# adamjorr/kbbq-py

Hardware: NVIDIA B200
Metric: bases/sec recalibrated (table build + apply) (higher is better)
Workload: dtype u8 in/out, u32->int64 counts, f64 model

## Files before the change

include/kbbq_b200.h:

```cpp
#ifndef KBBQ_B200_H
#define KBBQ_B200_H

#include <stddef.h>
#include <stdint.h>

#ifdef __cplusplus
extern "C" {
#endif

#define KBBQ_NQ 43
#define KBBQ_NDINUC 16

#define KBBQ_OK 0
#define KBBQ_E_ARG (-1)
#define KBBQ_E_CUDA (-2)
#define KBBQ_E_WORKSPACE (-3)
#define KBBQ_E_DATA (-4)
#define KBBQ_E_IO (-5)
#define KBBQ_E_FORMAT (-6)
#define KBBQ_E_RAGGED (-7)
#define KBBQ_E_NAME_FIELD (-8)
#define KBBQ_E_NAME_RG (-9)
#define KBBQ_E_NAME_MISMATCH (-10)
#define KBBQ_E_PEER (-11)
#define KBBQ_E_UNSUPPORTED (-12)

#define KBBQ_FLAG_QUAL_RANGE 1
#define KBBQ_FLAG_BAD_BASE 2
#define KBBQ_FLAG_RG_RANGE 4
#define KBBQ_FLAG_SEGMENTS 8

int kbbq_abi_version(void);
const char *kbbq_strerror(int code);
const char *kbbq_last_cuda_error(void);

int64_t kbbq_pos_table_elems(int L, int R);
int64_t kbbq_din_table_elems(int R);

int kbbq_workspace_bytes(int64_t N, int L, int R, size_t *bytes);

int kbbq_build(const uint8_t *seq_dev, const uint8_t *qual_dev, const uint8_t *corr_dev,
               const uint16_t *rg_dev, const uint8_t *second_dev, int64_t N, int L, int R,
               int minscore, int64_t *pos_errs_dev, int64_t *pos_total_dev, int64_t *din_errs_dev,
               int64_t *din_total_dev, void *workspace_dev, size_t workspace_bytes,
               int *status_dev, int path, void *stream);

int kbbq_marginals(const int64_t *pos_errs_dev, const int64_t *pos_total_dev, int L, int R,
                   int64_t *q_errs_dev, int64_t *q_total_dev, int64_t *rg_errs_dev,
                   int64_t *rg_total_dev, int64_t *meanq_dev, void *stream);

int kbbq_delta_q(const int64_t *prior_q_dev, const int64_t *numerrs_dev,
                 const int64_t *numtotal_dev, int64_t n, int64_t *delta_dev, void *stream);

int kbbq_posterior_q_real(const double *prior_q_dev, const int64_t *numerrs_dev,
                          const int64_t *numtotal_dev, int64_t n, int64_t *posterior_dev, void *stream);

int kbbq_bam_workspace_bytes(int64_t N, int L, int R, size_t *bytes);
int kbbq_build_bam(const uint8_t *seq_dev, const uint8_t *qual_dev, const uint8_t *err_dev,
                   const uint8_t *skip_dev, const uint16_t *rg_dev, const uint8_t *flags_dev,
                   const uint16_t *aln_start_dev, const uint16_t *aln_end_dev, int64_t N, int L, int R,
                   int minscore, int64_t *pos_errs_dev, int64_t *pos_total_dev, int64_t *din_errs_dev,
                   int64_t *din_total_dev, void *workspace_dev, size_t workspace_bytes, int *status_dev,
                   void *stream);
int kbbq_apply_bam(const uint8_t *seq_dev, const uint8_t *qual_dev, const uint16_t *rg_dev,
                   const uint8_t *flags_dev, int64_t N, int L, int R, int minscore,
                   const int64_t *meanq_dev, const int64_t *rgdq_dev, const int64_t *qdq_dev,
                   const int64_t *posdq_dev, const int64_t *dindq_dev, int nq, int ndin1,
                   uint8_t *out_qual_dev, void *workspace_dev, size_t workspace_bytes, int *status_dev,
                   void *stream);

int kbbq_calibration_counts(const uint8_t *qual_dev, const uint8_t *err_dev, const uint8_t *seq_dev,
                            const uint8_t *corr_dev, const uint8_t *skip_dev, int64_t n,
                            int64_t *total_dev, int64_t *errs_dev, void *stream);

int kbbq_get_delta_qs(const int64_t *meanq_dev, const int64_t *rg_errs_dev,
                      const int64_t *rg_total_dev, const int64_t *q_errs_dev,
                      const int64_t *q_total_dev, const int64_t *pos_errs_dev,
                      const int64_t *pos_total_dev, const int64_t *din_errs_dev,
                      const int64_t *din_total_dev, int R, int nq, int ncyc, int ndin,
                      int64_t *rgdq_dev, int64_t *qdq_dev, int64_t *posdq_dev, int64_t *dindq_dev,
                      void *stream);

int kbbq_apply(const uint8_t *seq_dev, const uint8_t *qual_dev, const uint16_t *rg_dev,
               const uint8_t *second_dev, int64_t N, int L, int R, int minscore,
               const int64_t *meanq_dev, const int64_t *rgdq_dev, const int64_t *qdq_dev,
               const int64_t *posdq_dev, const int64_t *dindq_dev, int nq, int ndin1,
               uint8_t *out_qual_dev, void *workspace_dev, size_t workspace_bytes, int *status_dev,
               int path, void *stream);

int64_t kbbq_segment_rows_bound(int64_t N, int R);
int64_t kbbq_segment_table_elems(int R);
int kbbq_segmented_supported(int L, int R, int minscore);
int kbbq_segment_plan(const uint16_t *rg_dev, const uint8_t *second_dev, int64_t N, int R, uint32_t *seg_dev,
                      uint32_t *dest_dev, int *status_dev, void *stream);
int kbbq_segment_rows(const uint8_t *src_dev, const uint32_t *dest_dev, int64_t N, int L, uint8_t *dst_segmented_dev,
                      void *stream);
int kbbq_segment_pad(const uint32_t *seg_dev, int R, int L, uint8_t *seq_dev, uint8_t *qual_dev, uint8_t *corr_dev,
                     void *stream);
int kbbq_unsegment_rows(const uint8_t *src_segmented_dev, const uint32_t *dest_dev, int64_t N, int L,
                        int64_t rows_bound, uint8_t *dst_dev, void *stream);
int kbbq_build_segmented(const uint8_t *seq_dev, const uint8_t *qual_dev, const uint8_t *corr_dev,
                         const uint32_t *seg_dev, int64_t rows_bound, int L, int R, int minscore,
                         int64_t *pos_errs_dev, int64_t *pos_total_dev, int64_t *din_errs_dev,
                         int64_t *din_total_dev, void *workspace_dev, size_t workspace_bytes, int *status_dev,
                         void *stream);
int kbbq_apply_segmented(const uint8_t *seq_dev, const uint8_t *qual_dev, const uint32_t *seg_dev, int64_t rows_bound,
                         int L, int R, int minscore, const int64_t *meanq_dev, const int64_t *rgdq_dev,
                         const int64_t *qdq_dev, const int64_t *posdq_dev, const int64_t *dindq_dev, int nq,
                         int ndin1, uint8_t *out_qual_dev, void *workspace_dev, size_t workspace_bytes,
                         int *status_dev, void *stream);

int kbbq_recalibrate_host(const uint8_t *seq, const uint8_t *qual, const uint8_t *corr,
                          const uint16_t *rg, const uint8_t *second, int64_t N, int L, int R,
                          int minscore, uint8_t *out_qual, int64_t *tables_host,
                          int64_t *deltas_host, int *status_out, int device);
int kbbq_recalibrate_host_multi(const uint8_t *seq, const uint8_t *qual, const uint8_t *corr,
                                const uint16_t *rg, const uint8_t *second, int64_t N, int L, int R,
                                int minscore, uint8_t *out_qual, int64_t *tables_host,
                                int64_t *deltas_host, int *status_out, const int *devices, int n_dev);

int kbbq_recalibrate_fastq(const char *reads_path, const char *corrected_path, int infer_rg, int minscore, int out_fd,
                           int device, int threads, int64_t *n_reads, int *n_rg, int *status_out);

int kbbq_host_release(int device);
int kbbq_host_last_traffic(int device, int64_t *h2d_bytes, int64_t *d2h_bytes);
int kbbq_host_pack_mode(int host_threads);

typedef struct kbbq_session kbbq_session;
int kbbq_session_create(int device, int L, int R, int minscore, int64_t chunk_reads, int64_t resident_reads_cap,
                        int host_threads, kbbq_session **out);
void kbbq_session_destroy(kbbq_session *s);
int64_t kbbq_session_chunk_reads(const kbbq_session *s);
// ... 88 lines not shown
```

kbbq-py_b200/csrc/apply.cuh:

```cuda
#pragma once
#include "build.cuh"
#include "common.cuh"
#include "stage.cuh"

namespace kbbq {

struct ApplyArgs {
    const uint8_t *seq, *qual;
    uint8_t *out;
    long long total_bytes;
    Geom g;
    TableCfg t;
    StageLayout sl;
    int R, nq;
    int nsub, segmode;
    const entry_t *entries;
    const unsigned int *seg;
    const unsigned int *uni;
    const short *fold_cyc;
    const short *fold_din;
    int *status;
};

static_assert((offsetof(ApplyArgs, t) + offsetof(TableCfg, ohe)) % 16 == 0,
              "ApplyArgs: TableCfg::ohe has to be 16-byte aligned in the kernel parameters (build.cuh); pad Geom");

__host__ __device__ inline int apply_table_bytes(const TableCfg &t) { return t.table_bytes; }

template <int KPS, bool UNI>
__device__ __forceinline__ void apply_consume(const ApplyArgs &a, unsigned char *smem_raw, uint32_t lo, uint32_t hi,
                                              uint32_t uni_flo, uint32_t uni_fhi) {
    const Geom &g = a.g;
    const TableCfg &t = a.t;
    const StageLayout &sl = a.sl;
    const int nconsumers = g.threads;
    const uint32_t bar0 = pin(smem_u32(smem_raw + sl.bar_off));
    const ThreadMap m = make_thread_map(g, t, UNI, true);
    const int lane = threadIdx.x & 31;
    const uint32_t pos_base = smem_addr(smem_raw + t.pos_off);
    const uint32_t din_base = pin(smem_addr(smem_raw + t.din_off) + (lane & (t.drep - 1)) * 4);
    uint32_t aeff[4];
#pragma unroll
    for (int b = 0; b < 4; ++b) aeff[b] = pos_base + m.cell[b];
    uint32_t cur_flag = 1;
    const uint32_t selv = pin(m.selv), seln = pin(m.seln);
    const uint32_t rowsel = m.row >= 0 ? (uint32_t)m.row : 0u;
    const uint32_t lanemask = pin(m.row >= 0 ? 0xFFu : 0u);
    const uint32_t rowmask = pin(m.rowmask);
    const bool live = m.row >= 0;
    const uint32_t kgrp = g.ng * g.gbytes;
    const bool half_lo = m.rowmask == 0x0000FFFFu, half_hi = m.rowmask == 0xFFFF0000u;
    const bool st32 = m.rowmask == 0xFFFFFFFFu, st16 = half_lo || half_hi, st8 = !st32 && !st16 && m.rowmask != 0u;
    const uint32_t wshift = pin(half_hi ? 16u : 0u);
    unsigned long long outp = (unsigned long long)(a.out + m.toff + (half_hi ? 2 : 0));
    asm volatile("" : "+l"(outp));
    const uint32_t data0 = pin(smem_u32(smem_raw + sl.data_off) + m.toff + (UNI ? m.grp * g.gbytes : 0));
    const uint32_t hdr0 = pin(smem_u32(smem_raw + sl.hdr_off) + m.grp * 16);
    const uint32_t stage_bytes = pin(sl.narr * sl.abytes), abytes = pin(sl.abytes), hdr_stride = sl.ngs * 16, krec = g.ng * 16;
    const uint32_t nstages = pin(sl.stages), ngs = pin(sl.ngs);
    const uint32_t revoff = t.revoff, addq = t.addq, gbytes = g.gbytes;
    const uint32_t addnq = (uint32_t)(128 - a.nq) * ONE4;
    const uint32_t one = pin(1u);
    uint32_t stage = 0, phase = 0;
    uint32_t qgood = 0xFFFFFFFFu;

    int cur_rg = -1, cur_sub = -1;
    int hs0 = 0, hs1 = 1;
    if (UNI && !a.segmode) {
        hs0 = (int)((uni_flo & 0xFFu) >> 1);
        hs1 = (int)(((uni_flo >> 8) & 0xFFu) >> 1);
    }
    for (int sub = 0; sub < a.nsub; ++sub) {
        uint32_t s_lo = a.seg[sub], s_hi = a.seg[sub + 1];
        if (s_hi <= lo) continue;
        if (s_lo >= hi) break;
        if (s_lo < lo) s_lo = lo;
        if (s_hi > hi) s_hi = hi;
        if (s_lo >= s_hi) continue;
        const int rg = a.segmode ? sub >> 1 : sub;

        if (rg != cur_rg || (a.segmode && sub != cur_sub)) {
            cur_rg = rg;
            cur_sub = sub;
            if (a.segmode) hs0 = hs1 = sub & 1;
            consumer_sync(nconsumers);
            for (int i = threadIdx.x; i < apply_table_bytes(t) / 4; i += nconsumers)
                reinterpret_cast<int *>(smem_raw)[i] = i * 4 < t.din_off && (i * 4) % t.revoff < t.rs ? g.minscore - 1 : 0;
            consumer_sync(nconsumers);
            const int L = g.L, L2 = 2 * g.L;
            const short *fc = a.fold_cyc + (size_t)rg * NQ * L2;
            for (int i = threadIdx.x; i < 2 * (t.nrows - 1) * L; i += nconsumers) {
                const int slot = i >= (t.nrows - 1) * L, j = i - slot * (t.nrows - 1) * L;
                const int r = j / L + 1, c = j - (r - 1) * L;
                const int half = slot ? hs1 : hs0;
                int *p = reinterpret_cast<int *>(smem_raw + t.pos_off + slot * t.revoff + r * t.rs) + ((c & 3) * t.sj + (c >> 2));
                *p = fc[(size_t)(r + g.minscore - 1) * L2 + (half ? L2 - 1 - c : c)];
            }
            const short *fd = a.fold_din + (size_t)rg * NQ * DIN_SLOTS;
            for (int i = threadIdx.x; i < (t.nrows - 1) * DIN_SLOTS * t.drep; i += nconsumers) {
                const int cell = i / t.drep, r = cell / DIN_SLOTS + 1, s = cell & (DIN_SLOTS - 1);
                int *p = reinterpret_cast<int *>(smem_raw + t.din_off + r * t.dq + s * (t.drep * 4)) + (i & (t.drep - 1));
                *p = fd[(r + g.minscore - 1) * DIN_SLOTS + s];
            }
            consumer_sync(nconsumers);
        }

        for (uint32_t first = s_lo; first < s_hi; first += ngs) {
            mbar_wait(bar0 + stage * 8, phase);
            const uint32_t shdr = pin(hdr0 + stage * hdr_stride);
            uint32_t sdata = data0 + stage * stage_bytes;
            uint32_t nlive = sl.ngs;
            if (UNI) {
                sdata += (uint32_t)((unsigned long long)first * g.gbytes) & 15u;
                nlive = s_hi - first;
            }
            sdata = pin(sdata);
            auto apply_word = [&](const uint32_t wa, const uint32_t hgrp) {
                uint32_t sw, qw, pb;
                asm volatile("ld.shared.u32 %0, [%1];" : "=r"(sw) : "r"(wa));
                asm volatile("ld.shared.u32 %0, [%1];" : "=r"(qw) : "r"(wa + abytes));
                asm volatile("ld.shared.u8 %0, [%1];" : "=r"(pb) : "r"(wa - 1));

                const uint32_t nu = ~add_fma(qw, one, addnq);
                const uint32_t w5 = add_fma(qw, one, addq);
                qgood &= nu & ~qw;
                const uint32_t vraw = w5 & nu & ~qw;
                const uint32_t vm8 = prmt(vraw, 0u, selv);
                const uint32_t qrow4 = w5 & vm8 & 0x3F3F3F3Fu;
                const uint32_t pw = prmt(pb, sw, 0x6540u);
                const uint32_t d4 = (pw & 0x06060606u) * 4u + (sw & 0x06060606u);
                const uint32_t nm8 = prmt((sw | pw) * 16u, 0xFFFFFFFFu, seln);
                const uint32_t qd = qrow4 & ~nm8;
                const uint32_t x01 = prmt(d4, qd, 0x5140u), x23 = prmt(d4, qd, 0x7362u);

                uint32_t v[4];
#pragma unroll
                for (int b = 0; b < 4; ++b) {
                    const uint32_t pa = (b & 2) ? __dp2a_hi(t.cyc16[b & 1], qrow4, aeff[b]) : __dp2a_lo(t.cyc16[b & 1], qrow4, aeff[b]);
                    const uint32_t xb = (b & 2) ? x23 : x01;
                    const uint32_t da = (b & 1) ? __dp2a_hi(t.din16, xb, din_base) : __dp2a_lo(t.din16, xb, din_base);
                    uint32_t x, y;
                    asm volatile("ld.shared.u32 %0, [%1];" : "=r"(x) : "r"(pa));
                    asm volatile("ld.shared.u32 %0, [%1];" : "=r"(y) : "r"(da));
                    v[b] = x + y;
                }
                const uint32_t sum4 = __byte_perm(__byte_perm(v[0], v[1], 0x0040), __byte_perm(v[2], v[3], 0x0040), 0x5410);
                const uint32_t res = (sum4 & vm8) | (qw & ~vm8);
                const unsigned long long dst = outp + (unsigned long long)hgrp * gbytes;
                if (UNI) {
                    if (st32) asm volatile("st.global.u32 [%0], %1;" ::"l"(dst), "r"(res) : "memory");
                    return;
                }
                if (st32) asm volatile("st.global.u32 [%0], %1;" ::"l"(dst), "r"(res) : "memory");
                if (st16) asm volatile("st.global.u16 [%0], %1;" ::"l"(dst), "h"((unsigned short)(res >> wshift)) : "memory");
                if (st8) {
#pragma unroll
                    for (int b = 0; b < 4; ++b)
                        if ((rowmask >> (8 * b)) & 1u)
                            asm volatile("st.global.u8 [%0], %1;" ::"l"(dst + b), "r"(res >> (8 * b)) : "memory");
                }
            };
            if (UNI && nlive >= sl.ngs) {
#pragma unroll
                for (int k = 0; k < KPS; ++k) apply_word(sdata + k * kgrp, first + m.grp + k * g.ng);
            } else {
#pragma unroll
                for (int k = 0; k < KPS; ++k) {
                    uint32_t soff, hgrp;
                    if (UNI) {
                        if (!live || (uint32_t)(m.grp + k * g.ng) >= nlive) continue;
                        soff = k * kgrp;
                        hgrp = first + m.grp + k * g.ng;
                    } else {
                        uint32_t flo, fhi;
                        if (g.contig) {
                            const uint32_t e = first + (uint32_t)m.grp + (uint32_t)(k * g.ng);
                            const uint4 rec = e < s_hi ? __ldg(a.entries + e) : make_uint4(0u, 0u, 0u, 0u);
                            soff = rec.x; hgrp = rec.y; flo = rec.z; fhi = rec.w;
                        } else {
                            asm volatile("ld.shared.v4.u32 {%0, %1, %2, %3}, [%4];"
                                         : "=r"(soff), "=r"(hgrp), "=r"(flo), "=r"(fhi)
                                         : "r"(shdr + k * krec));
                        }
                        const uint32_t flag = prmt(flo, fhi, rowsel) & lanemask;
                        if (flag != cur_flag) {
                            if (!flag) continue;
                            const uint32_t delta = ((flag >> 1) - (cur_flag >> 1)) * revoff;
#pragma unroll
                            for (int b = 0; b < 4; ++b) aeff[b] += delta;
                            cur_flag = flag;
                        }
                    }
                    apply_word(sdata + soff, hgrp);
                }
            }
            __syncwarp();
            if (lane == 0) mbar_arrive(bar0 + (nstages + stage) * 8);
            if (++stage == nstages) { stage = 0; phase ^= 1; }
        }
    }
    if (~qgood & rowmask & H4) atomicOr(a.status, KBBQ_FLAG_QUAL_RANGE);
}


template <int KPS>
__global__ void __launch_bounds__(MAX_THREADS, 1) apply_smem_kernel(const __grid_constant__ ApplyArgs a) {
    extern __shared__ __align__(128) unsigned char smem_raw[];
    const Geom &g = a.g;
    const StageLayout &sl = a.sl;
    const int nconsumers = g.threads;

    const unsigned long long E = a.seg[a.nsub];
    const uint32_t lo = (uint32_t)(E * blockIdx.x / gridDim.x), hi = (uint32_t)(E * (blockIdx.x + 1) / gridDim.x);
    const bool contig = a.R == 1 || a.segmode;
    const bool uniform = contig && a.uni[0] == 0u;

    const uint32_t bar0 = smem_u32(smem_raw + sl.bar_off);
    if (threadIdx.x == 0) {
        for (int s = 0; s < sl.stages; ++s) {
            mbar_init(bar0 + s * 8, 1);
            mbar_init(bar0 + (sl.stages + s) * 8, nconsumers / 32);
        }
        mbar_fence_init();
    }
    __syncthreads();

    if ((int)threadIdx.x >= nconsumers) {
        ProducerArgs p;
        p.arr[0] = a.seq; p.arr[1] = a.qual; p.arr[2] = nullptr;
        p.entries = a.entries; p.seg = a.seg; p.nsub = a.nsub; p.contig = contig; p.lo = lo; p.hi = hi;
        p.gbytes = g.gbytes; p.ng = sl.ngs; p.total_bytes = a.total_bytes;
        p.pw = ((int)threadIdx.x - nconsumers) >> 5; p.nprod = g.nprod;
        p.uniform = uniform;
        producer_loop(p, sl, smem_raw);
        return;
    }

    if (uniform) apply_consume<KPS, true>(a, smem_raw, lo, hi, a.uni[1], a.uni[2]);
    else apply_consume<KPS, false>(a, smem_raw, lo, hi, 0u, 0u);
}

struct ApplyGenericArgs {
    const uint8_t *seq, *qual;
    const uint16_t *rg;
    const uint8_t *second;
    uint8_t *out;
    long long N;
    int L, R, minscore, nq;
    const short *fold_cyc, *fold_din;
    int *status;
};

__global__ void apply_generic_kernel(ApplyGenericArgs a) {
    const long long total = a.N * a.L;
    for (long long i = (long long)blockIdx.x * blockDim.x + threadIdx.x; i < total;
         i += (long long)gridDim.x * blockDim.x) {
        const long long r = i / a.L;
        const int c = (int)(i - r * a.L);
        const unsigned int q = a.qual[i];
        if ((int)q < a.minscore) { a.out[i] = (uint8_t)q; continue; }
        if ((int)q >= a.nq) { atomicOr(a.status, KBBQ_FLAG_QUAL_RANGE); a.out[i] = (uint8_t)q; continue; }
        const unsigned int g = a.rg ? a.rg[r] : 0;
        if (g >= (unsigned int)a.R) { atomicOr(a.status, KBBQ_FLAG_RG_RANGE); a.out[i] = (uint8_t)q; continue; }
        const int c2 = (a.second && a.second[r]) ? 2 * a.L - 1 - c : c;
        const size_t gq = (size_t)g * NQ + q;
        int v = a.fold_cyc[gq * (2 * a.L) + c2];
        if (c > 0) {
            const uint8_t s = a.seq[i], ps = a.seq[i - 1];
            if (s != 'N' && ps != 'N') v += a.fold_din[gq * DIN_SLOTS + ((((ps >> 1) & 3) << 2) | ((s >> 1) & 3))];
        }
        a.out[i] = (uint8_t)v;
    }
}

}
```

kbbq-py_b200/csrc/build.cuh:

```cuda
#pragma once
#include <cstddef>
#include "common.cuh"
#include "prepare.cuh"
#include "stage.cuh"

namespace kbbq {

constexpr uint32_t ERR_UNIT = 65025u;
constexpr int DIN_SLOTS = 16;
constexpr int DIN_REP = 32;
constexpr int MAX_WARPS = MAX_THREADS / 32;

struct TableCfg {
    int nrows;
    int rs;
    int sj;
    int revoff;
    int dq;
    int drep;
    int pos_off, din_off;
    int table_bytes;
    int flush_pos;
    int fold_din;
    uint32_t addq;
    uint32_t cyc16[2];
    uint32_t din16;
    uint32_t ohe[4];
    uint32_t val16[2];
};

inline int cycle_table_wavefronts(const Geom &g, int sj, int rs_words, int shift, bool word_owner) {
    const int nwords = g.gbytes >> 2;
    int total = 0;
    for (int warp = 0; warp < g.threads / 32; ++warp)
        for (int b = 0; b < 4; ++b) {
            int cnt[32] = {0}, worst = 0;
            for (int lane = 0; lane < 32; ++lane) {
                const int tid = warp * 32 + lane, grp = tid / g.lps, t = tid - grp * g.lps;
                int cell = (lane + 32 * b) % rs_words;
                if (grp < g.ng && word_owner) {
                    if (t < nwords) {
                        const int j = 4 * t + b, k = j / g.L, c = j - k * g.L;
                        cell = (c & 3) * sj + (c >> 2) + (k & 1) * shift;
                    }
                } else if (grp < g.ng) {
                    for (int k = 0; k < g.G; ++k)
                        if (t >= g.wstart[k] && t < g.wstart[k + 1]) {
                            const int c = 4 * (t - g.wstart[k]) + b - ((k * g.L) & 3);
                            cell = c >= 0 && c < g.L ? (c & 3) * sj + (c >> 2) + (k & 1) * shift : 0;
                        }
                }
                worst = std::max(worst, ++cnt[cell & 31]);
            }
            total += worst;
        }
    return total;
}

inline bool make_table_cfg(const Geom &g, int kps, int drep, bool word_owner, TableCfg *t) {
    if (g.minscore < 1) return false;
    if (drep != 32 && drep != 16 && drep != 8) return false;
    t->nrows = NQ + 1 - g.minscore;
    t->sj = (g.L + 3) / 4;
    t->rs = (16 * t->sj + 127) / 128 * 128;
    if (t->rs > 1152) return false;
    int shift = 0;
    if (const char *e = getenv("KBBQ_SLOT_SHIFT")) shift = std::max(0, std::min(31, atoi(e)));
    else {
        int best = cycle_table_wavefronts(g, t->sj, t->rs / 4, 0, word_owner);
        for (int d = 1; d < 32; ++d) {
            const int w = cycle_table_wavefronts(g, t->sj, t->rs / 4, d, word_owner);
            if (w < best) { best = w; shift = d; }
        }
    }
    t->revoff = t->nrows * t->rs + 4 * shift;
    t->drep = drep;
    t->dq = DIN_SLOTS * drep * 4;
    t->pos_off = 0;
    t->din_off = (t->revoff + t->nrows * t->rs + 127) / 128 * 128;
    t->table_bytes = t->din_off + t->nrows * t->dq;
    t->flush_pos = std::max(1, (int)((ERR_UNIT - 1) / (uint32_t)(kps * g.ng * g.G)));
    t->fold_din = std::max(1, (int)((ERR_UNIT - 1) / (uint32_t)(kps * 4 * ((g.threads + drep - 1) / drep))));
    t->addq = (uint32_t)(0x81 - g.minscore) * ONE4;
    t->cyc16[0] = (uint32_t)t->rs;
    t->cyc16[1] = (uint32_t)t->rs << 16;
    t->din16 = (uint32_t)(drep * 2) | ((uint32_t)t->dq << 16);
    for (int b = 0; b < 4; ++b) t->ohe[b] = 255u << (8 * b);
    t->val16[0] = 1u | (16u << 16);
    t->val16[1] = 256u | (4096u << 16);
    return true;
}

struct BuildArgs {
    const uint8_t *seq, *qual, *corr;
    long long total_bytes;
    Geom g;
    TableCfg t;
    StageLayout sl;
    int R;
    int nsub;
    int segmode;
    const entry_t *entries;
    const unsigned int *seg;
    const unsigned int *uni;
    unsigned long long *pos_errs, *pos_total, *din_errs, *din_total;
    int *status;
};

static_assert((offsetof(BuildArgs, t) + offsetof(TableCfg, ohe)) % 16 == 0,
              "BuildArgs: TableCfg::ohe has to be 16-byte aligned in the kernel parameters; pad Geom");

__device__ __forceinline__ void red_shared_add(uint32_t saddr, uint32_t v) {
    asm volatile("red.shared.add.u32 [%0], %1;" ::"r"(saddr), "r"(v) : "memory");
}
__device__ __forceinline__ uint32_t smem_addr(const void *p) {
    return (uint32_t)__cvta_generic_to_shared(p);
}
__device__ __forceinline__ uint32_t prmt(uint32_t a, uint32_t b, uint32_t sel) {
    uint32_t d;
    asm("prmt.b32 %0, %1, %2, %3;" : "=r"(d) : "r"(a), "r"(b), "r"(sel));
    return d;
}
__device__ __forceinline__ uint32_t pin(uint32_t v) {
    asm volatile("" : "+r"(v));
    return v;
}

__device__ __forceinline__ uint32_t add_fma(uint32_t a, uint32_t one, uint32_t c) {
    uint32_t d;
    asm("mad.lo.u32 %0, %1, %2, %3;" : "=r"(d) : "r"(a), "r"(one), "r"(c));
    return d;
}

struct ThreadMap {
    int grp;
    int row;
    int toff;
    uint32_t rowmask;
    uint32_t selv;
    uint32_t seln;
    uint32_t cell[4];
    int cyc[4];
};

__device__ __forceinline__ ThreadMap make_thread_map(const Geom &g, const TableCfg &tc, bool by_parity, bool word_owner) {
    ThreadMap m;
    const int tid = threadIdx.x;
    m.grp = tid / g.lps;
    const int t = tid - m.grp * g.lps;
    m.row = -1;
    int w = 0;
#pragma unroll
    for (int k = 0; k < MAX_G; ++k)
        if (k < g.G && t >= g.wstart[k] && t < g.wstart[k + 1]) { m.row = k; w = t - g.wstart[k]; }
    if (m.grp >= g.ng) m.row = -1;
    m.rowmask = 0; m.toff = 0; m.selv = 0x4444u; m.seln = 0x4444u;
#pragma unroll
    for (int b = 0; b < 4; ++b) { m.cell[b] = 0; m.cyc[b] = -1; }
    if (by_parity && word_owner) {
        const int nwords = g.gbytes >> 2;
        m.row = (t < nwords && m.grp < g.ng) ? (4 * t) / g.L : -1;
        if (m.row >= 0) {
            m.toff = 4 * t;
            m.rowmask = 0xFFFFFFFFu;
            m.selv = 0xBA98u;
            m.seln = 0xBA98u;
#pragma unroll
            for (int b = 0; b < 4; ++b) {
                const int j = 4 * t + b, k = j / g.L, c = j - k * g.L;
                m.cyc[b] = c;
                if (c == 0) m.seln = (m.seln & ~(0xFu << (4 * b))) | (0x4u << (4 * b));
                m.cell[b] = 4u * (uint32_t)((c & 3) * tc.sj + (c >> 2)) + (uint32_t)((k & 1) * tc.revoff);
            }
        }
    } else if (m.row >= 0) {
        const int a = (m.row * g.L) & 3;
        m.toff = m.row * g.L - a + 4 * w;
#pragma unroll
        for (int b = 0; b < 4; ++b) {
            const int c = 4 * w + b - a;
            if (c >= 0 && c < g.L) {
                m.cyc[b] = c;
                m.rowmask |= 0xFFu << (8 * b);
                m.selv = (m.selv & ~(0xFu << (4 * b))) | ((8u | b) << (4 * b));
                if (c != 0) m.seln = (m.seln & ~(0xFu << (4 * b))) | ((8u | b) << (4 * b));
                m.cell[b] = 4u * (uint32_t)((c & 3) * tc.sj + (c >> 2)) + (by_parity ? (uint32_t)((m.row & 1) * tc.revoff) : 0u);
            }
// ... 12 lines not shown
    const int lane = threadIdx.x & 31, warp = threadIdx.x >> 5, nwarps = nconsumers >> 5;
    unsigned long long *gde = a.din_errs + (size_t)rg * NQ * 16, *gdt = a.din_total + (size_t)rg * NQ * 16;
    for (int cell = DIN_SLOTS + warp; cell < t.nrows * DIN_SLOTS; cell += nwarps) {
        const int r = cell / DIN_SLOTS, dn = cell - r * DIN_SLOTS;
        unsigned int *p = reinterpret_cast<unsigned int *>(smem_raw + t.din_off + r * t.dq + dn * (t.drep * 4)) + lane;
        const unsigned int v = lane < t.drep ? *p : 0u;
        if (__any_sync(0xFFFFFFFFu, v != 0)) {
            if (lane < t.drep) *p = 0;
            unsigned int tot = v % ERR_UNIT, er = v / ERR_UNIT;
#pragma unroll
            for (int o = 16; o; o >>= 1) {
                tot += __shfl_xor_sync(0xFFFFFFFFu, tot, o);
                er += __shfl_xor_sync(0xFFFFFFFFu, er, o);
            }
            if (lane == 0) {
                const int dref = nat_to_ref(dn >> 2) * 4 + nat_to_ref(dn & 3);
                const size_t o = (size_t)(r + a.g.minscore - 1) * 16 + dref;
                atomicAdd(gdt + o, (unsigned long long)tot);
                if (er) atomicAdd(gde + o, (unsigned long long)er);
            }
        }
    }
}

__device__ __forceinline__ void flush_pos_table(const BuildArgs &a, unsigned char *smem_raw, int rg, int nconsumers, int hs0, int hs1) {
    const Geom &g = a.g;
    const TableCfg &t = a.t;
    const int L = g.L, L2 = 2 * g.L;
    unsigned long long *gpe = a.pos_errs + (size_t)rg * NQ * L2, *gpt = a.pos_total + (size_t)rg * NQ * L2;
    const int per_slot = (t.nrows - 1) * L;
    for (int i = threadIdx.x; i < 2 * per_slot; i += nconsumers) {
        const int slot = i >= per_slot, j = i - slot * per_slot;
        const int r = j / L + 1, c = j - (r - 1) * L;
        unsigned int *p = reinterpret_cast<unsigned int *>(smem_raw + t.pos_off + slot * t.revoff + r * t.rs) +
                          ((c & 3) * t.sj + (c >> 2));
        const unsigned int v = *p;
        if (v) {
            *p = 0;
            const unsigned int tot = v % ERR_UNIT, er = v / ERR_UNIT;
            const int half = slot ? hs1 : hs0;
            const size_t o = (size_t)(r + g.minscore - 1) * L2 + (half ? L2 - 1 - c : c);
            atomicAdd(gpt + o, (unsigned long long)tot);
            if (er) atomicAdd(gpe + o, (unsigned long long)er);
        }
    }
}

template <int KPS, bool VALIDATE, bool UNI>
__device__ __forceinline__ void build_consume(const BuildArgs &a, unsigned char *smem_raw, uint32_t lo, uint32_t hi,
                                              uint32_t uni_flo, uint32_t uni_fhi) {
    const Geom &g = a.g;
    const TableCfg &t = a.t;
    const StageLayout &sl = a.sl;
    const int nconsumers = g.threads;
    const uint32_t bar0 = pin(smem_u32(smem_raw + sl.bar_off));
    const ThreadMap m = make_thread_map(g, t, UNI, false);
    const int lane = threadIdx.x & 31;
    const uint32_t pos_base = smem_addr(smem_raw + t.pos_off);
    const uint32_t din_base = pin(smem_addr(smem_raw + t.din_off) + (lane & (t.drep - 1)) * 4);
    uint32_t aeff[4];
#pragma unroll
    for (int b = 0; b < 4; ++b) aeff[b] = pos_base + m.cell[b];
    uint32_t cur_flag = 1;
    const uint32_t selv = pin(m.selv), seln = pin(m.seln);
    const uint32_t rowsel = m.row >= 0 ? (uint32_t)m.row : 0u;
    const uint32_t lanemask = pin(m.row >= 0 ? 0xFFu : 0u);
    const uint32_t rowmask = pin(m.rowmask);
    const bool live = m.row >= 0;
    const uint32_t data0 = pin(smem_u32(smem_raw + sl.data_off) + m.toff + (UNI ? m.grp * g.gbytes : 0));
    const uint32_t hdr0 = pin(smem_u32(smem_raw + sl.hdr_off) + m.grp * 16);
    const uint32_t kgrp = g.ng * g.gbytes;
    const uint32_t stage_bytes = pin(sl.narr * sl.abytes), abytes = pin(sl.abytes), abytes2 = pin(2 * sl.abytes), hdr_stride = sl.ngs * 16, krec = g.ng * 16;
    const uint32_t nstages = pin(sl.stages), ngs = pin(sl.ngs);
    const uint32_t revoff = t.revoff, addq = t.addq;
    const uint32_t one = pin(1u), minus1 = pin(0xFFFFFFFFu), lut_lo = pin(0x43014101u), lut_hi = pin(0x474E0154u);
    uint32_t stage = 0, phase = 0;
    uint32_t qgood = 0xFFFFFFFFu, bbad = 0;

    for (int i = threadIdx.x; i < t.table_bytes / 4; i += nconsumers) reinterpret_cast<unsigned int *>(smem_raw)[i] = 0;
    consumer_sync(nconsumers);
    int cur_rg = -1, cur_sub = -1;
    int hs0 = 0, hs1 = 1;
    uint32_t since_pos = 0, since_din = 0;
    auto flush_all = [&](int rg) {
        consumer_sync(nconsumers);
        flush_pos_table(a, smem_raw, rg, nconsumers, hs0, hs1);
        fold_din_replicas(a, smem_raw, rg, nconsumers);
        consumer_sync(nconsumers);
        since_pos = since_din = 0;
    };
    if (UNI && !a.segmode) {
        hs0 = (int)((uni_flo & 0xFFu) >> 1);
        hs1 = (int)(((uni_flo >> 8) & 0xFFu) >> 1);
    }

    for (int sub = 0; sub < a.nsub; ++sub) {
        uint32_t s_lo = a.seg[sub], s_hi = a.seg[sub + 1];
        if (s_hi <= lo) continue;
        if (s_lo >= hi) break;
        if (s_lo < lo) s_lo = lo;
        if (s_hi > hi) s_hi = hi;
        if (s_lo >= s_hi) continue;
        const int rg = a.segmode ? sub >> 1 : sub;
        if (cur_rg >= 0 && (rg != cur_rg || (a.segmode && sub != cur_sub))) flush_all(cur_rg);
        cur_rg = rg;
        cur_sub = sub;
        if (a.segmode) hs0 = hs1 = sub & 1;

        for (uint32_t first = s_lo; first < s_hi;) {
            if (since_pos >= (uint32_t)t.flush_pos || since_din >= (uint32_t)t.fold_din) {
                consumer_sync(nconsumers);
                if (since_pos >= (uint32_t)t.flush_pos) { flush_pos_table(a, smem_raw, rg, nconsumers, hs0, hs1); since_pos = 0; }
                if (since_din >= (uint32_t)t.fold_din) { fold_din_replicas(a, smem_raw, rg, nconsumers); since_din = 0; }
                consumer_sync(nconsumers);
            }
            const uint32_t room = min((uint32_t)t.flush_pos - since_pos, (uint32_t)t.fold_din - since_din);
            const uint32_t chunk_end = (uint32_t)min((unsigned long long)s_hi, (unsigned long long)first + (unsigned long long)room * sl.ngs);
            const uint32_t iters = (chunk_end - first + ngs - 1) / ngs;
            since_pos += iters;
            since_din += iters;
            for (; first < chunk_end; first += ngs) {
                mbar_wait(bar0 + stage * 8, phase);
                const uint32_t shdr = pin(hdr0 + stage * hdr_stride);
                uint32_t sdata = data0 + stage * stage_bytes;
                uint32_t nlive = sl.ngs;
                if (UNI) {
                    sdata += (uint32_t)((unsigned long long)first * g.gbytes) & 15u;
                    nlive = s_hi - first;
                }
                sdata = pin(sdata);
                auto tally_word = [&](const uint32_t wa) {
                    uint32_t sw, qw, cw, pb;
                    asm volatile("ld.shared.u32 %0, [%1];" : "=r"(sw) : "r"(wa));
                    asm volatile("ld.shared.u32 %0, [%1];" : "=r"(qw) : "r"(wa + abytes));
                    asm volatile("ld.shared.u32 %0, [%1];" : "=r"(cw) : "r"(wa + abytes2));
                    asm volatile("ld.shared.u8 %0, [%1];" : "=r"(pb) : "r"(wa - 1));

                    const uint32_t nu = add_fma(qw, minus1, 0xAAAAAAAAu);
                    const uint32_t w5 = qw + addq;
                    qgood &= nu & ~qw;
                    const uint32_t vraw = w5 & nu & ~qw;
                    const uint32_t vm8 = prmt(vraw, 0u, selv);
                    const uint32_t qrow4 = w5 & vm8 & 0x3F3F3F3Fu;

                    const uint32_t pw = prmt(pb, sw, 0x6540u);
                    const uint32_t d4 = (pw & 0x06060606u) * 4u + (sw & 0x06060606u);
                    const uint32_t nm8 = prmt((sw | pw) * 16u, 0xFFFFFFFFu, seln);
                    const uint32_t qd = qrow4 & ~nm8;
                    const uint32_t x01 = prmt(d4, qd, 0x5140u), x23 = prmt(d4, qd, 0x7362u);

                    const uint32_t e8 = prmt(add_fma(sw ^ cw, one, 0x7F7F7F7Fu), 0u, 0xBA98u);

                    if (VALIDATE) {
                        const uint32_t code3 = sw & 0x07070707u;
                        const uint32_t sel = __dp2a_hi(t.val16[1], code3, __dp2a_lo(t.val16[0], code3, 0u));
                        const uint32_t recon = prmt(lut_lo, lut_hi, sel);
                        bbad |= recon ^ sw;
                    }

#pragma unroll
                    for (int b = 0; b < 4; ++b) {
                        const uint32_t inc = __dp4a(e8, t.ohe[b], one);
                        const uint32_t pa = (b & 2) ? __dp2a_hi(t.cyc16[b & 1], qrow4, aeff[b]) : __dp2a_lo(t.cyc16[b & 1], qrow4, aeff[b]);
                        const uint32_t xb = (b & 2) ? x23 : x01;
                        const uint32_t da = (b & 1) ? __dp2a_hi(t.din16, xb, din_base) : __dp2a_lo(t.din16, xb, din_base);
                        red_shared_add(pa, inc);
                        red_shared_add(da, inc);
                    }
                };
                if (UNI && nlive >= sl.ngs) {
#pragma unroll
                    for (int k = 0; k < KPS; ++k) tally_word(sdata + k * kgrp);
                } else {
#pragma unroll
                    for (int k = 0; k < KPS; ++k) {
                        uint32_t soff;
                        if (UNI) {
                            if (!live || (uint32_t)(m.grp + k * g.ng) >= nlive) continue;
                            soff = k * kgrp;
                        } else {
                            uint32_t hgrp, flo, fhi;
                            if (g.contig) {
                                const uint32_t e = first + (uint32_t)m.grp + (uint32_t)(k * g.ng);
                                const uint4 rec = e < s_hi ? __ldg(a.entries + e) : make_uint4(0u, 0u, 0u, 0u);
                                soff = rec.x; hgrp = rec.y; flo = rec.z; fhi = rec.w;
                            } else {
                                asm volatile("ld.shared.v4.u32 {%0, %1, %2, %3}, [%4];"
                                             : "=r"(soff), "=r"(hgrp), "=r"(flo), "=r"(fhi)
                                             : "r"(shdr + k * krec));
                            }
                            const uint32_t flag = prmt(flo, fhi, rowsel) & lanemask;
                            if (flag != cur_flag) {
                                if (!flag) continue;
                                const uint32_t delta = ((flag >> 1) - (cur_flag >> 1)) * revoff;
#pragma unroll
                                for (int b = 0; b < 4; ++b) aeff[b] += delta;
                                cur_flag = flag;
                            }
                        }
                        tally_word(sdata + soff);
                    }
                }
                __syncwarp();
                if (lane == 0) mbar_arrive(bar0 + (nstages + stage) * 8);
                if (++stage == nstages) { stage = 0; phase ^= 1; }
            }
        }
    }
    if (cur_rg >= 0) flush_all(cur_rg);
    if (~qgood & rowmask & H4) atomicOr(a.status, KBBQ_FLAG_QUAL_RANGE);
    if (VALIDATE && (bbad & rowmask)) atomicOr(a.status, KBBQ_FLAG_BAD_BASE);
}


template <int KPS, bool VALIDATE>
__global__ void __launch_bounds__(MAX_THREADS, 1) build_smem_kernel(const __grid_constant__ BuildArgs a) {
    extern __shared__ __align__(128) unsigned char smem_raw[];
    const Geom &g = a.g;
    const StageLayout &sl = a.sl;
    const int nconsumers = g.threads;

    const unsigned long long E = a.seg[a.nsub];
    const uint32_t lo = (uint32_t)(E * blockIdx.x / gridDim.x), hi = (uint32_t)(E * (blockIdx.x + 1) / gridDim.x);
    const bool contig = a.R == 1 || a.segmode;
    const bool uniform = contig && a.uni[0] == 0u;

    const uint32_t bar0 = smem_u32(smem_raw + sl.bar_off);
    if (threadIdx.x == 0) {
        for (int s = 0; s < sl.stages; ++s) {
            mbar_init(bar0 + s * 8, 1);
            mbar_init(bar0 + (sl.stages + s) * 8, nconsumers / 32);
        }
        mbar_fence_init();
    }
    __syncthreads();

    if ((int)threadIdx.x >= nconsumers) {
        ProducerArgs p;
        p.arr[0] = a.seq; p.arr[1] = a.qual; p.arr[2] = a.corr;
        p.entries = a.entries; p.seg = a.seg; p.nsub = a.nsub; p.contig = contig; p.lo = lo; p.hi = hi;
        p.gbytes = g.gbytes; p.ng = sl.ngs; p.total_bytes = a.total_bytes;
        p.pw = ((int)threadIdx.x - nconsumers) >> 5; p.nprod = g.nprod;
        p.uniform = uniform;
        producer_loop(p, sl, smem_raw);
        return;
    }

    if (uniform) build_consume<KPS, VALIDATE, true>(a, smem_raw, lo, hi, a.uni[1], a.uni[2]);
    else build_consume<KPS, VALIDATE, false>(a, smem_raw, lo, hi, 0u, 0u);
}

struct BuildGenericArgs {
    const uint8_t *seq, *qual, *corr;
    const uint16_t *rg;
    const uint8_t *second;
    long long N;
    int L, R, minscore;
    unsigned long long *pos_errs, *pos_total, *din_errs, *din_total;
    int *status;
};

__device__ __forceinline__ int base_code_ref(uint8_t b) {
    return b == 'A' ? 0 : b == 'T' ? 1 : b == 'G' ? 2 : b == 'C' ? 3 : b == 'N' ? 4 : 5;
}

__global__ void build_generic_kernel(BuildGenericArgs a) {
    const long long total = a.N * a.L;
    for (long long i = (long long)blockIdx.x * blockDim.x + threadIdx.x; i < total;
         i += (long long)gridDim.x * blockDim.x) {
        const long long r = i / a.L;
        const int c = (int)(i - r * a.L);
        const unsigned int q = a.qual[i];
        const uint8_t s = a.seq[i];
        const int code = base_code_ref(s);
        if (code == 5) atomicOr(a.status, KBBQ_FLAG_BAD_BASE);
        if (q > NQ - 1) { atomicOr(a.status, KBBQ_FLAG_QUAL_RANGE); continue; }
        const unsigned int g = a.rg ? a.rg[r] : 0;
        if (g >= (unsigned int)a.R) { atomicOr(a.status, KBBQ_FLAG_RG_RANGE); continue; }
        if ((int)q < a.minscore) continue;
        const bool err = s != a.corr[i];
        const int c2 = (a.second && a.second[r]) ? 2 * a.L - 1 - c : c;
        const size_t po = ((size_t)g * NQ + q) * (2 * a.L) + c2;
        atomicAdd(a.pos_total + po, 1ull);
        if (err) atomicAdd(a.pos_errs + po, 1ull);
        if (c > 0) {
            const int pcode = base_code_ref(a.seq[i - 1]);
            if (code < 4 && pcode < 4) {
                const size_t d = ((size_t)g * NQ + q) * 16 + pcode * 4 + code;
                atomicAdd(a.din_total + d, 1ull);
                if (err) atomicAdd(a.din_errs + d, 1ull);
            }
        }
    }
}

}
```

kbbq-py_b200/csrc/host_api.cu:

```cuda
#include <algorithm>
#include <atomic>
#include <chrono>
#include <condition_variable>
#include <memory>
#include <mutex>
#include <sched.h>
#include <stdlib.h>
#include <string.h>
#include <sys/mman.h>
#include <sys/stat.h>
#include <fcntl.h>
#include <thread>
#include <unistd.h>
#include <vector>

#include "common.cuh"

using namespace kbbq;

namespace {

#define KBBQ_TRY(x) do { int rc_ = (x); if (rc_) return rc_; } while (0)

constexpr int MAX_DEVICES = 16;
// ... 258 lines not shown
    return p;
}

bool chunk_args_ok(const kbbq_session *S, int64_t k, int64_t n, bool keep) {
    return n > 0 && n <= S->C && (!keep || k < (int64_t)S->res.size());
}

int build_chunk_upload(kbbq_session *S, int64_t k, const uint8_t *seq, const uint8_t *qual, const uint16_t *rg,
                       const uint8_t *second, int64_t n, bool keep) {
    if (!chunk_args_ok(S, k, n, keep) || !seq || !qual) return KBBQ_E_ARG;
    const ChunkPlace p = chunk_place(S, k, keep, rg != nullptr, second != nullptr);
    KBBQ_CUDA(cudaStreamWaitEvent(S->s_up, p.u->consumed, 0));
    return upload_reads(S, S->pack == PACK_NIBBLES ? nullptr : seq, qual, rg, second, n, p.d_seq, p.d_qual, p.d_rg, p.d_sec);
}

int build_chunk_finish(kbbq_session *S, int64_t k, const uint8_t *seq, const uint8_t *corr, bool has_rg, bool has_second,
                       int64_t n, bool keep) {
    if (!chunk_args_ok(S, k, n, keep) || !seq || !corr) return KBBQ_E_ARG;
    const ChunkPlace p = chunk_place(S, k, keep, has_rg, has_second);
    UpSlot &u = *p.u;
    Resident *r = p.r;
    const int L = S->L, R = S->R;
    const size_t nb = (size_t)n * L;
    if (r) r->n = n;
    if (S->pack) {
        KBBQ_CUDA(cudaEventSynchronize(u.uploaded));
        size_t bb;
        if (S->pack == PACK_NIBBLES) {
            int bad = 0;
            KBBQ_TRY(kbbq_host_pack_nibbles(seq, corr, (int64_t)nb, (uint8_t *)u.h_bits, S->host_threads, &bad));
            if (bad) S->host_status |= KBBQ_FLAG_BAD_BASE;
            bb = (nb + 1) / 2;
        } else {
            KBBQ_TRY(kbbq_host_mismatch_bits(seq, corr, (int64_t)nb, u.h_bits, S->host_threads));
            bb = ((nb + 31) / 32) * 4;
        }
        KBBQ_CUDA(cudaMemcpyAsync(u.bits, u.h_bits, bb, cudaMemcpyHostToDevice, S->s_up));
        S->h2d_bytes += (int64_t)bb;
    } else {
        KBBQ_CUDA(cudaMemcpyAsync(u.corr, corr, nb, cudaMemcpyHostToDevice, S->s_up));
        S->h2d_bytes += (int64_t)nb;
    }
    KBBQ_CUDA(cudaEventRecord(u.uploaded, S->s_up));
    KBBQ_CUDA(cudaStreamWaitEvent(S->s_comp, u.uploaded, 0));
    if (S->pack == PACK_NIBBLES) KBBQ_TRY(kbbq_expand_nibbles((const uint8_t *)u.bits, (int64_t)nb, p.d_seq, u.corr, S->s_comp));
    else if (S->pack == PACK_BITS) KBBQ_TRY(kbbq_expand_mismatch_bits(p.d_seq, u.bits, (int64_t)nb, u.corr, S->s_comp));
    const size_t npos = (size_t)R * NQ * 2 * L, ndin = (size_t)R * NQ * 16;
    int64_t *pe = S->d_tab, *pt = pe + npos, *de = pt + npos, *dt = de + ndin;
    if (S->segmode) {
        uint32_t *seg = keep ? r->seg : u.seg, *dest = keep ? r->dest : u.dest;
        uint8_t *sseq = keep ? r->seq : u.sseq, *squal = keep ? r->qual : u.squal;
        KBBQ_TRY(kbbq_segment_plan(p.d_rg, p.d_sec, n, R, seg, dest, S->d_status, S->s_comp));
        KBBQ_TRY(kbbq_segment_rows(p.d_seq, dest, n, L, sseq, S->s_comp));
        KBBQ_TRY(kbbq_segment_rows(p.d_qual, dest, n, L, squal, S->s_comp));
        KBBQ_TRY(kbbq_segment_rows(u.corr, dest, n, L, u.scorr, S->s_comp));
        KBBQ_TRY(kbbq_segment_pad(seg, R, L, sseq, squal, u.scorr, S->s_comp));
        KBBQ_TRY(kbbq_build_segmented(sseq, squal, u.scorr, seg, S->rowsC, L, R, S->minscore, pe, pt, de, dt, S->d_ws,
                                      S->ws_bytes, S->d_status, S->s_comp));
    } else {
        KBBQ_TRY(kbbq_build(p.d_seq, p.d_qual, u.corr, p.d_rg, p.d_sec, n, L, R, S->minscore, pe, pt, de, dt, S->d_ws, S->ws_bytes,
                            S->d_status, 0, S->s_comp));
    }
    KBBQ_CUDA(cudaEventRecord(u.consumed, S->s_comp));
    return KBBQ_OK;
}

int build_chunk_async(kbbq_session *S, const uint8_t *seq, const uint8_t *qual, const uint8_t *corr, const uint16_t *rg,
                      const uint8_t *second, int64_t n, bool keep) {
    if (n < 0 || n > S->C) return KBBQ_E_ARG;
    if (n == 0) return KBBQ_OK;
    if (!seq || !qual || !corr) return KBBQ_E_ARG;
    const int64_t k = S->built;
    if (keep && k >= (int64_t)S->res.size()) return KBBQ_E_ARG;
    S->built++;
    KBBQ_TRY(build_chunk_upload(S, k, seq, qual, rg, second, n, keep));
    return build_chunk_finish(S, k, seq, corr, rg != nullptr, second != nullptr, n, keep);
}

int model_async(kbbq_session *S) {
    const int L = S->L, R = S->R;
    const size_t npos = (size_t)R * NQ * 2 * L, ndin = (size_t)R * NQ * 16;
    int64_t *pe = S->summed ? S->d_sum : S->d_tab, *pt = pe + npos, *de = pt + npos, *dt = de + ndin;
    const ModelPtrs &mp = S->mp;
    KBBQ_TRY(kbbq_marginals(pe, pt, L, R, mp.q_errs, mp.q_total, mp.rg_errs, mp.rg_total, mp.meanq, S->s_comp));
    KBBQ_TRY(kbbq_get_delta_qs(mp.meanq, mp.rg_errs, mp.rg_total, mp.q_errs, mp.q_total, pe, pt, de, dt, R, NQ, 2 * L, 16,
                               mp.rgdq, mp.qdq, mp.posdq, mp.dindq, S->s_comp));
    return KBBQ_OK;
}

int apply_and_download(kbbq_session *S, const uint8_t *d_seq, const uint8_t *d_qual, const uint16_t *d_rg,
                       const uint8_t *d_sec, const uint32_t *seg, const uint32_t *dest, int64_t n, uint8_t *out_host) {
    const int L = S->L, R = S->R;
    OutSlot &o = S->down[S->applied++ & 1];
    const ModelPtrs &mp = S->mp;
    KBBQ_CUDA(cudaStreamWaitEvent(S->s_comp, o.drained, 0));
    if (S->segmode) {
        KBBQ_TRY(kbbq_apply_segmented(d_seq, d_qual, seg, S->rowsC, L, R, S->minscore, mp.meanq, mp.rgdq, mp.qdq, mp.posdq,
                                      mp.dindq, NQ, 17, o.out_seg, S->d_ws, S->ws_bytes, S->d_status, S->s_comp));
        KBBQ_TRY(kbbq_unsegment_rows(o.out_seg, dest, n, L, S->rowsC, o.out, S->s_comp));
    } else {
        KBBQ_TRY(kbbq_apply(d_seq, d_qual, d_rg, d_sec, n, L, R, S->minscore, mp.meanq, mp.rgdq, mp.qdq, mp.posdq, mp.dindq,
                            NQ, 17, o.out, S->d_ws, S->ws_bytes, S->d_status, 0, S->s_comp));
    }
    KBBQ_CUDA(cudaEventRecord(o.applied, S->s_comp));
    KBBQ_CUDA(cudaStreamWaitEvent(S->s_down, o.applied, 0));
    KBBQ_CUDA(cudaMemcpyAsync(out_host, o.out, (size_t)n * L, cudaMemcpyDeviceToHost, S->s_down));
    S->d2h_bytes += n * L;
    KBBQ_CUDA(cudaEventRecord(o.drained, S->s_down));
    return KBBQ_OK;
}

int apply_resident_async(kbbq_session *S, int64_t k, uint8_t *out_host) {
    if (k < 0 || k >= (int64_t)S->res.size() || !out_host) return KBBQ_E_ARG;
    const Resident &r = S->res[(size_t)k];
    if (r.n == 0) return KBBQ_OK;
    return apply_and_download(S, r.seq, r.qual, r.rg, r.sec, r.seg, r.dest, r.n, out_host);
}

int apply_chunk_async(kbbq_session *S, const uint8_t *seq, const uint8_t *qual, const uint16_t *rg, const uint8_t *second,
                      int64_t n, uint8_t *out_host) {
    if (n < 0 || n > S->C || !S->up[0].seq) return KBBQ_E_ARG;
    if (n == 0) return KBBQ_OK;
    if (!seq || !qual || !out_host) return KBBQ_E_ARG;
    UpSlot &u = S->up[S->applied & 1];
    const int L = S->L, R = S->R;
    uint16_t *d_rg = rg ? u.rg : nullptr;
    uint8_t *d_sec = second ? u.sec : nullptr;
    KBBQ_CUDA(cudaStreamWaitEvent(S->s_up, u.consumed, 0));
    KBBQ_TRY(upload_reads(S, seq, qual, rg, second, n, u.seq, u.qual, d_rg, d_sec));
    KBBQ_CUDA(cudaEventRecord(u.uploaded, S->s_up));
    KBBQ_CUDA(cudaStreamWaitEvent(S->s_comp, u.uploaded, 0));
    const uint8_t *a_seq = u.seq, *a_qual = u.qual;
    if (S->segmode) {
        uint8_t *sseq = u.sseq ? u.sseq : nullptr, *squal = u.squal;
        if (!sseq) return KBBQ_E_ARG;
        KBBQ_TRY(kbbq_segment_plan(d_rg, d_sec, n, R, u.seg, u.dest, S->d_status, S->s_comp));
        KBBQ_TRY(kbbq_segment_rows(u.seq, u.dest, n, L, sseq, S->s_comp));
        KBBQ_TRY(kbbq_segment_rows(u.qual, u.dest, n, L, squal, S->s_comp));
        KBBQ_TRY(kbbq_segment_pad(u.seg, R, L, sseq, squal, nullptr, S->s_comp));
        a_seq = sseq; a_qual = squal;
    }
    KBBQ_TRY(apply_and_download(S, a_seq, a_qual, d_rg, d_sec, u.seg, u.dest, n, out_host));
    KBBQ_CUDA(cudaEventRecord(u.consumed, S->s_comp));
    return KBBQ_OK;
}

int session_sync(kbbq_session *S, int *status_out) {
    int st = 0;
    KBBQ_CUDA(cudaStreamSynchronize(S->s_up));
    KBBQ_CUDA(cudaStreamSynchronize(S->s_comp));
    KBBQ_CUDA(cudaStreamSynchronize(S->s_down));
    KBBQ_CUDA(cudaMemcpy(&st, S->d_status, sizeof(int), cudaMemcpyDeviceToHost));
    st |= S->host_status;
    if (status_out) *status_out = st;
    return st ? KBBQ_E_DATA : KBBQ_OK;
}

struct CacheSlot {
    std::mutex mu;
    std::unique_ptr<kbbq_session> s;
};
CacheSlot g_cache[MAX_DEVICES];

int cached_session(int slot, int device, int L, int R, int minscore, int64_t C, int64_t M, int host_threads, int pack,
                   kbbq_session **out) {
    CacheSlot &c = g_cache[slot];
    kbbq_session *s = c.s.get();
    const int64_t C16 = (C + 15) / 16 * 16;
    const int64_t nres = M ? (M + C16 - 1) / C16 : 0;
    if (s && s->device == device && s->L == L && s->R == R && s->minscore == minscore && s->C == C16 &&
// ... 597 lines not shown
```

kbbq-py_b200/csrc/kbbq_b200.cu:

```cuda
#include <algorithm>
#include <mutex>
#include <stdlib.h>
#include <string.h>
#include <vector>

#include "apply.cuh"
#include "bam.cuh"
#include "build.cuh"
#include "calib.cuh"
#include "common.cuh"
#include "model.cuh"
#include "prepare.cuh"
#include "segment.cuh"
#include "synth.cuh"

namespace kbbq {

std::atomic<long long> g_launches{0};
char g_last_cuda_error[256] = "";

static std::mutex g_const_mu;
static bool g_const_done[64];

static int upload_constants(int device) {
// ... 133 lines not shown
    case KBBQ_E_DATA: return "input data error (see status flags)";
    case KBBQ_E_IO: return "FASTQ file could not be opened, read or written";
    case KBBQ_E_FORMAT: return "malformed FASTQ (4-line records expected)";
    case KBBQ_E_RAGGED: return "reads of unequal length";
    case KBBQ_E_NAME_FIELD: return "read name has no read-group field";
    case KBBQ_E_NAME_RG: return "read-group field does not start with RG";
    case KBBQ_E_NAME_MISMATCH: return "corrected read name does not start with the read name";
    case KBBQ_E_PEER: return "multi-GPU: peer access between the devices is not available";
    case KBBQ_E_UNSUPPORTED: return "not handled by this entry point (use the chunked driver)";
    default: return "unknown error";
    }
}

const char *kbbq_last_cuda_error(void) { return g_last_cuda_error; }

int64_t kbbq_pos_table_elems(int L, int R) { return (int64_t)R * NQ * 2 * L; }
int64_t kbbq_din_table_elems(int R) { return (int64_t)R * NQ * 16; }
int64_t kbbq_launch_count(void) { return g_launches.load(); }

int kbbq_plan_info(int L, int R, int minscore, int arrays, int max_smem, int *out) {
    if (!out || L < 1 || R < 1 || (arrays != 2 && arrays != 3)) return KBBQ_E_ARG;
    Geom g;
    TableCfg tc;
    StageLayout sl;
    if (!plan_kernel(L, R, minscore, arrays, max_smem > 0 ? max_smem : 232448, &g, &tc, &sl))
        return KBBQ_E_ARG;
    const int v[10] = {g.G, g.lanes, g.ng, g.threads, g.nprod, sl.kps, sl.stages, tc.drep, sl.total, tc.table_bytes};
    for (int i = 0; i < 10; ++i) out[i] = v[i];
    return KBBQ_OK;
}

int kbbq_workspace_bytes(int64_t N, int L, int R, size_t *bytes) {
    if (N < 0 || L < 1 || R < 1 || R > 65535 || !bytes) return KBBQ_E_ARG;
    *bytes = carve_workspace(nullptr, N, L, R).bytes;
    return KBBQ_OK;
}

static int build_impl(const uint8_t *seq, const uint8_t *qual, const uint8_t *corr, const uint16_t *rg,
                      const uint8_t *second, int64_t N, int L, int R, int minscore, int64_t *pos_errs,
                      int64_t *pos_total, int64_t *din_errs, int64_t *din_total, void *workspace,
                      size_t workspace_bytes, int *status, int path, void *stream, const unsigned int *seg_rows) {
    if (N < 0 || L < 1 || R < 1 || R > 65535 || minscore < 0 || minscore >= NQ) return KBBQ_E_ARG;
    if (!pos_errs || !pos_total || !din_errs || !din_total || !status) return KBBQ_E_ARG;
    if (N == 0) return KBBQ_OK;
    if (!seq || !qual || !corr) return KBBQ_E_ARG;
    const bool segmode = seg_rows != nullptr;
    cudaStream_t st = (cudaStream_t)stream;
    int device, sms, max_smem;
    int rc = current_device_info(&device, &sms, &max_smem);
    if (rc) return rc;

    Geom g;
    TableCfg tc;
    StageLayout sl;
    const bool smem_ok = path != 2 && !misaligned(seq, 16) && !misaligned(qual, 16) && !misaligned(corr, 16) &&
                         plan_kernel(L, R, minscore, 3, max_smem, &g, &tc, &sl, segmode) &&
                         (uint64_t)((N + g.G - 1) / g.G) < 0xFFFFFFFFull;
    if (!smem_ok) {
        if (path == 1 || segmode) return KBBQ_E_ARG;
        BuildGenericArgs a = {seq, qual, corr, rg, second, N, L, R, minscore,
                              (unsigned long long *)pos_errs, (unsigned long long *)pos_total,
                              (unsigned long long *)din_errs, (unsigned long long *)din_total, status};
        build_generic_kernel<<<sms * 8, 256, 0, st>>>(a);
        KBBQ_LAUNCHED();
        return KBBQ_OK;
    }
    Workspace w = carve_workspace(workspace, N, L, R);
    if (!workspace || workspace_bytes < w.bytes) return KBBQ_E_WORKSPACE;
    if (segmode) {
        seg_prepare_kernel<<<1, 256, 0, st>>>(seg_rows, 2 * R, g.G, (unsigned long long)N, w.seg, w.uni, status);
        KBBQ_LAUNCHED();
    } else {
        const int64_t tail = (R == 1 && N > g.G) ? N % g.G : 0;
        if (tail) {
            const int64_t n0 = N - tail;
            BuildGenericArgs ga = {seq + n0 * L, qual + n0 * L, corr + n0 * L, rg ? rg + n0 : nullptr,
                                   second ? second + n0 : nullptr, tail, L, R, minscore,
                                   (unsigned long long *)pos_errs, (unsigned long long *)pos_total,
                                   (unsigned long long *)din_errs, (unsigned long long *)din_total, status};
            build_generic_kernel<<<1, 256, 0, st>>>(ga);
            KBBQ_LAUNCHED();
            N = n0;
        }
        rc = run_prepare(rg, second, N, g.G, R, w, status, sms, sl.ngs, g.gbytes, sl.slot, st);
        if (rc) return rc;
    }

    BuildArgs a;
    a.seq = seq; a.qual = qual; a.corr = corr; a.total_bytes = N * L; a.g = g; a.t = tc; a.R = R;
    a.nsub = segmode ? 2 * R : R; a.segmode = segmode ? 1 : 0;
    a.sl = sl;
    a.entries = w.entries; a.seg = w.seg; a.uni = w.uni;
    a.pos_errs = (unsigned long long *)pos_errs; a.pos_total = (unsigned long long *)pos_total;
    a.din_errs = (unsigned long long *)din_errs; a.din_total = (unsigned long long *)din_total;
    a.status = status;
    return launch_build_smem(a, sms, a.sl.total, st);
}

int kbbq_build(const uint8_t *seq, const uint8_t *qual, const uint8_t *corr, const uint16_t *rg,
               const uint8_t *second, int64_t N, int L, int R, int minscore, int64_t *pos_errs,
               int64_t *pos_total, int64_t *din_errs, int64_t *din_total, void *workspace,
               size_t workspace_bytes, int *status, int path, void *stream) {
    return build_impl(seq, qual, corr, rg, second, N, L, R, minscore, pos_errs, pos_total, din_errs, din_total,
                      workspace, workspace_bytes, status, path, stream, nullptr);
}

int kbbq_build_segmented(const uint8_t *seq, const uint8_t *qual, const uint8_t *corr, const uint32_t *seg,
                         int64_t rows_bound, int L, int R, int minscore, int64_t *pos_errs, int64_t *pos_total,
                         int64_t *din_errs, int64_t *din_total, void *workspace, size_t workspace_bytes, int *status,
                         void *stream) {
    if (!seg || rows_bound % SEG_ALIGN) return KBBQ_E_ARG;
    return build_impl(seq, qual, corr, nullptr, nullptr, rows_bound, L, R, minscore, pos_errs, pos_total, din_errs,
                      din_total, workspace, workspace_bytes, status, 1, stream, seg);
}

int kbbq_marginals(const int64_t *pos_errs, const int64_t *pos_total, int L, int R, int64_t *q_errs,
                   int64_t *q_total, int64_t *rg_errs, int64_t *rg_total, int64_t *meanq, void *stream) {
    if (L < 1 || R < 1 || !pos_errs || !pos_total || !q_errs || !q_total || !rg_errs || !rg_total || !meanq)
        return KBBQ_E_ARG;
    cudaStream_t st = (cudaStream_t)stream;
    int device;
    KBBQ_CUDA(cudaGetDevice(&device));
    int rc = upload_constants(device);
    if (rc) return rc;
    marginals_q_kernel<<<dim3(NQ, R), 128, 0, st>>>((const long long *)pos_errs, (const long long *)pos_total,
                                                   2 * L, (long long *)q_errs, (long long *)q_total);
    KBBQ_LAUNCHED();
    marginals_rg_kernel<<<R, 64, 0, st>>>((const long long *)q_errs, (const long long *)q_total, R,
                                                      (long long *)rg_errs, (long long *)rg_total, (long long *)meanq);
    KBBQ_LAUNCHED();
    return KBBQ_OK;
}

int kbbq_delta_q(const int64_t *prior_q, const int64_t *numerrs, const int64_t *numtotal, int64_t n,
                 int64_t *delta, void *stream) {
    if (n < 0 || (n > 0 && (!prior_q || !numerrs || !numtotal || !delta))) return KBBQ_E_ARG;
    if (n == 0) return KBBQ_OK;
    int device;
    KBBQ_CUDA(cudaGetDevice(&device));
    int rc = upload_constants(device);
    if (rc) return rc;
    delta_q_kernel<<<(unsigned)((n + 127) / 128), 128, 0, (cudaStream_t)stream>>>(
        (const long long *)prior_q, (const long long *)numerrs, (const long long *)numtotal, n, (long long *)delta);
    KBBQ_LAUNCHED();
    return KBBQ_OK;
}

int kbbq_posterior_q_real(const double *prior_q, const int64_t *numerrs, const int64_t *numtotal, int64_t n,
                          int64_t *posterior, void *stream) {
    if (n < 0 || (n > 0 && (!prior_q || !numerrs || !numtotal || !posterior))) return KBBQ_E_ARG;
    if (n == 0) return KBBQ_OK;
    int device;
    KBBQ_CUDA(cudaGetDevice(&device));
    int rc = upload_constants(device);
    if (rc) return rc;
    posterior_q_real_kernel<<<(unsigned)((n + 127) / 128), 128, 0, (cudaStream_t)stream>>>(
        prior_q, (const long long *)numerrs, (const long long *)numtotal, n, (long long *)posterior);
    KBBQ_LAUNCHED();
    return KBBQ_OK;
}

struct BamWorkspace {
    uint8_t *cseq, *cqual, *cthird, *csecond;
    void *inner;
    size_t inner_bytes, bytes;
};
static BamWorkspace carve_bam_workspace(void *base, long long N, int L, int R) {
    BamWorkspace w = {};
    char *p = (char *)base;
    size_t off = 0;
    const size_t nb = align_up((size_t)N * L + 16, 256);
    w.cseq = (uint8_t *)(p + off); off += nb;
    w.cqual = (uint8_t *)(p + off); off += nb;
    w.cthird = (uint8_t *)(p + off); off += nb;
    w.csecond = (uint8_t *)(p + off); off += align_up((size_t)N + 16, 256);
    w.inner = p + off;
    w.inner_bytes = carve_workspace(nullptr, N, L, R).bytes;
    w.bytes = off + w.inner_bytes;
    return w;
}

static int launch_bam_canon(const BamCanonArgs &c, cudaStream_t st) {
    const unsigned int wmax = (unsigned int)((3 + c.L + 3) >> 2);
    const long long per = std::max<long long>(1, (long long)(0x7FFFFFFFu / wmax) / 256 * 256);
    for (long long r0 = 0; r0 < c.N; r0 += per) {
        const long long n = std::min<long long>(per, c.N - r0);
        bam_canon_kernel<<<(unsigned)((n * wmax + BAM_WARPS * 32 - 1) / (BAM_WARPS * 32)), BAM_WARPS * 32, 0, st>>>(c, r0, wmax);
        KBBQ_LAUNCHED();
    }
    return KBBQ_OK;
}

int kbbq_bam_workspace_bytes(int64_t N, int L, int R, size_t *bytes) {
    if (N < 0 || L < 1 || R < 1 || R > 65535 || !bytes) return KBBQ_E_ARG;
    *bytes = carve_bam_workspace(nullptr, N, L, R).bytes;
    return KBBQ_OK;
}

int kbbq_build_bam(const uint8_t *seq, const uint8_t *qual, const uint8_t *err, const uint8_t *skip, const uint16_t *rg,
                   const uint8_t *flags, const uint16_t *aln_start, const uint16_t *aln_end, int64_t N, int L, int R,
                   int minscore, int64_t *pos_errs, int64_t *pos_total, int64_t *din_errs, int64_t *din_total,
                   void *workspace, size_t workspace_bytes, int *status, void *stream) {
    if (N < 0 || L < 1 || L > 32767 || R < 1 || R > 65535 || minscore < 0 || minscore > NQ) return KBBQ_E_ARG;
    if (!pos_errs || !pos_total || !din_errs || !din_total || !status) return KBBQ_E_ARG;
    if (N == 0) return KBBQ_OK;
    if (!seq || !qual || !err) return KBBQ_E_ARG;
    int device, sms = KBBQ_SM_COUNT_FALLBACK;
    KBBQ_CUDA(cudaGetDevice(&device));
    cudaDeviceGetAttribute(&sms, cudaDevAttrMultiProcessorCount, device);
    cudaStream_t st = (cudaStream_t)stream;
    const long long blocks = std::min<long long>(((long long)N * L + 255) / 256, (long long)sms * 16);
    if (workspace && minscore >= 1) {
        BamWorkspace w = carve_bam_workspace(workspace, N, L, R);
        if (workspace_bytes < w.bytes) return KBBQ_E_WORKSPACE;
        BamCanonArgs c = {seq, qual, err, skip, rg, flags, aln_start, aln_end, N, L, R, minscore, true,
                          w.cseq, w.cqual, w.cthird, w.csecond,
                          (unsigned long long *)pos_errs, (unsigned long long *)pos_total,
                          (unsigned long long *)din_errs, (unsigned long long *)din_total, status};
        { const int rc_ = launch_bam_canon(c, st); if (rc_) return rc_; }
        return kbbq_build(w.cseq, w.cqual, w.cthird, rg, w.csecond, N, L, R, minscore, pos_errs, pos_total, din_errs,
                          din_total, w.inner, w.inner_bytes, status, 0, stream);
    }
    BuildBamArgs a = {seq, qual, err, skip, rg, flags, aln_start, aln_end, N, L, R, minscore,
                      (unsigned long long *)pos_errs, (unsigned long long *)pos_total,
                      (unsigned long long *)din_errs, (unsigned long long *)din_total, status};
    build_bam_kernel<<<(unsigned)blocks, 256, 0, st>>>(a);
    KBBQ_LAUNCHED();
    return KBBQ_OK;
}

int kbbq_apply_bam(const uint8_t *seq, const uint8_t *qual, const uint16_t *rg, const uint8_t *flags, int64_t N, int L,
                   int R, int minscore, const int64_t *meanq, const int64_t *rgdq, const int64_t *qdq,
                   const int64_t *posdq, const int64_t *dindq, int nq, int ndin1, uint8_t *out_qual, void *workspace,
                   size_t workspace_bytes, int *status, void *stream) {
    if (N < 0 || L < 1 || L > 32767 || R < 1 || R > 65535 || nq < 1 || nq > 256 || ndin1 != 17) return KBBQ_E_ARG;
    if (!meanq || !rgdq || !qdq || !posdq || !dindq || !status) return KBBQ_E_ARG;
    if (N == 0) return KBBQ_OK;
    if (!seq || !qual || !out_qual) return KBBQ_E_ARG;
    int device, sms = KBBQ_SM_COUNT_FALLBACK;
    KBBQ_CUDA(cudaGetDevice(&device));
    cudaDeviceGetAttribute(&sms, cudaDevAttrMultiProcessorCount, device);
    cudaStream_t st = (cudaStream_t)stream;
    const long long blocks = std::min<long long>(((long long)N * L + 255) / 256, (long long)sms * 16);
    if (workspace && minscore >= 1 && nq <= NQ) {
        BamWorkspace w = carve_bam_workspace(workspace, N, L, R);
        if (workspace_bytes < w.bytes) return KBBQ_E_WORKSPACE;
        BamCanonArgs c = {seq, qual, nullptr, nullptr, rg, flags, nullptr, nullptr, N, L, R, minscore, false,
                          w.cseq, w.cqual, nullptr, w.csecond, nullptr, nullptr, nullptr, nullptr, status};
        { const int rc_ = launch_bam_canon(c, st); if (rc_) return rc_; }
        int rc = kbbq_apply(w.cseq, w.cqual, rg, w.csecond, N, L, R, minscore, meanq, rgdq, qdq, posdq, dindq, nq, ndin1,
                            w.cthird, w.inner, w.inner_bytes, status, 0, stream);
        if (rc) return rc;
        {
            const unsigned int wmax = (unsigned int)((3 + L + 3) >> 2);
            const long long per = std::max<long long>(1, (long long)(0x7FFFFFFFu / wmax) / 256 * 256);
            for (long long r0 = 0; r0 < N; r0 += per) {
                const long long n = std::min<long long>(per, N - r0);
                bam_uncanon_kernel<<<(unsigned)((n * wmax + BAM_WARPS * 32 - 1) / (BAM_WARPS * 32)), BAM_WARPS * 32, 0, st>>>(
                    w.cthird, flags, N, L, out_qual, r0, wmax);
                KBBQ_LAUNCHED();
            }
        }
        return KBBQ_OK;
    }
    ApplyBamArgs a = {seq, qual, rg, flags, out_qual, N, L, R, minscore, nq, ndin1, (const long long *)meanq,
                      (const long long *)rgdq, (const long long *)qdq, (const long long *)posdq,
                      (const long long *)dindq, status};
    apply_bam_kernel<<<(unsigned)blocks, 256, 0, st>>>(a);
    KBBQ_LAUNCHED();
    return KBBQ_OK;
}

int kbbq_calibration_counts(const uint8_t *qual, const uint8_t *err, const uint8_t *seq, const uint8_t *corr,
                            const uint8_t *skip, int64_t n, int64_t *total, int64_t *errs, void *stream) {
    if (n < 0 || !total || !errs) return KBBQ_E_ARG;
    if (n == 0) return KBBQ_OK;
    if (!qual || (!err && (!seq || !corr))) return KBBQ_E_ARG;
    cudaStream_t st = (cudaStream_t)stream;
    int device, sms = KBBQ_SM_COUNT_FALLBACK;
    KBBQ_CUDA(cudaGetDevice(&device));
    cudaDeviceGetAttribute(&sms, cudaDevAttrMultiProcessorCount, device);
    auto misaligned = [](const void *p) { return p && ((uintptr_t)p & 15u); };
    CalibArgs a = {qual, err, seq, corr, skip, n, (unsigned long long *)total, (unsigned long long *)errs};
    if (misaligned(qual) || misaligned(err) || misaligned(skip) || (!err && (misaligned(seq) || misaligned(corr)))) {
        const long long chunk = 1ll << 31;
        for (long long o = 0; o < n; o += chunk) {
            CalibArgs c = a;
            c.qual += o; if (err) c.err += o; else { c.seq += o; c.corr += o; } if (skip) c.skip += o;
            c.n = std::min<long long>(chunk, n - o);
            calibration_scalar_kernel<<<sms * 8, CAL_THREADS, 0, st>>>(c);
            KBBQ_LAUNCHED();
        }
        return KBBQ_OK;
    }
    const int grid = sms * 3;
    const long long chunk = (long long)grid * CAL_THREADS * CAL_MAX_ITERS * 32;
    auto kern = err ? (skip ? calibration_kernel<true, true> : calibration_kernel<true, false>)
                    : (skip ? calibration_kernel<false, true> : calibration_kernel<false, false>);
    KBBQ_CUDA(cudaFuncSetAttribute(kern, cudaFuncAttributeMaxDynamicSharedMemorySize, CAL_SMEM));
    for (long long o = 0; o < n; o += chunk) {
        CalibArgs c = a;
        c.qual += o; if (err) c.err += o; else { c.seq += o; c.corr += o; } if (skip) c.skip += o;
        c.n = std::min<long long>(chunk, n - o);
        kern<<<grid, CAL_THREADS, CAL_SMEM, st>>>(c);
        KBBQ_LAUNCHED();
    }
    return KBBQ_OK;
}

int kbbq_get_delta_qs(const int64_t *meanq, const int64_t *rg_errs, const int64_t *rg_total,
                      const int64_t *q_errs, const int64_t *q_total, const int64_t *pos_errs,
                      const int64_t *pos_total, const int64_t *din_errs, const int64_t *din_total, int R,
                      int nq, int ncyc, int ndin, int64_t *rgdq, int64_t *qdq, int64_t *posdq,
                      int64_t *dindq, void *stream) {
    if (R < 1 || nq < 1 || ncyc < 0 || ndin < 0) return KBBQ_E_ARG;
    if (!meanq || !rg_errs || !rg_total || !q_errs || !q_total || !rgdq || !qdq) return KBBQ_E_ARG;
    if ((ncyc && (!pos_errs || !pos_total || !posdq)) || !dindq || (ndin && (!din_errs || !din_total)))
        return KBBQ_E_ARG;
    int device;
    KBBQ_CUDA(cudaGetDevice(&device));
    int rc = upload_constants(device);
    if (rc) return rc;
    cudaStream_t st = (cudaStream_t)stream;
    DeltaArgs a = {(const long long *)meanq, (const long long *)rg_errs, (const long long *)rg_total,
                   (const long long *)q_errs, (const long long *)q_total, (const long long *)pos_errs,
                   (const long long *)pos_total, (const long long *)din_errs, (const long long *)din_total,
                   R, nq, ncyc, ndin, (long long *)rgdq, (long long *)qdq, (long long *)posdq, (long long *)dindq};
    delta_levels12_kernel<<<R, 64, 0, st>>>(a);
    KBBQ_LAUNCHED();
    const long long cells = (long long)R * nq * (ncyc + ndin + 1);
    delta_level3_kernel<<<(unsigned)((cells + 127) / 128), 128, 0, st>>>(a);
    KBBQ_LAUNCHED();
    return KBBQ_OK;
}

static int apply_impl(const uint8_t *seq, const uint8_t *qual, const uint16_t *rg, const uint8_t *second, int64_t N,
                      int L, int R, int minscore, const int64_t *meanq, const int64_t *rgdq, const int64_t *qdq,
                      const int64_t *posdq, const int64_t *dindq, int nq, int ndin1, uint8_t *out_qual,
                      void *workspace, size_t workspace_bytes, int *status, int path, void *stream,
                      const unsigned int *seg_rows) {
    const bool segmode = seg_rows != nullptr;
    if (N < 0 || L < 1 || R < 1 || R > 65535 || minscore < 0 || minscore >= NQ) return KBBQ_E_ARG;
    if (nq < 1 || nq > NQ || ndin1 < 16 || ndin1 > 64) return KBBQ_E_ARG;
    if (!meanq || !rgdq || !qdq || !posdq || !dindq || !status) return KBBQ_E_ARG;
    if (N == 0) return KBBQ_OK;
    if (!seq || !qual || !out_qual) return KBBQ_E_ARG;
    cudaStream_t st = (cudaStream_t)stream;
    int device, sms, max_smem;
    int rc = current_device_info(&device, &sms, &max_smem);
    if (rc) return rc;
    Workspace w = carve_workspace(workspace, N, L, R);
    if (!workspace || workspace_bytes < w.bytes) return KBBQ_E_WORKSPACE;

    const long long fold_cells = (long long)R * NQ * (2 * L + 16);
    fold_kernel<<<(unsigned)((fold_cells + 255) / 256), 256, 0, st>>>(
        (const long long *)meanq, (const long long *)rgdq, (const long long *)qdq, (const long long *)posdq,
        (const long long *)dindq, R, nq, 2 * L, ndin1, w.fold_cyc, w.fold_din);
    KBBQ_LAUNCHED();

    Geom g;
    TableCfg tc;
    StageLayout sl;
    const bool smem_ok = path != 2 && !misaligned(seq, 16) && !misaligned(qual, 16) && !misaligned(out_qual, 4) &&
                         plan_kernel(L, R, minscore, 2, max_smem, &g, &tc, &sl, segmode) &&
                         (uint64_t)((N + g.G - 1) / g.G) < 0xFFFFFFFFull;
    if (!smem_ok) {
        if (path == 1 || segmode) return KBBQ_E_ARG;
        ApplyGenericArgs a = {seq, qual, rg, second, out_qual, N, L, R, minscore, nq, w.fold_cyc, w.fold_din, status};
        apply_generic_kernel<<<sms * 8, 256, 0, st>>>(a);
        KBBQ_LAUNCHED();
        return KBBQ_OK;
    }
    const int64_t tail = (!segmode && R == 1 && N > g.G) ? N % g.G : 0;
    if (tail) {
        const int64_t n0 = N - tail;
        ApplyGenericArgs ga = {seq + n0 * L, qual + n0 * L, rg ? rg + n0 : nullptr, second ? second + n0 : nullptr,
                               out_qual + n0 * L, tail, L, R, minscore, nq, w.fold_cyc, w.fold_din, status};
        apply_generic_kernel<<<1, 256, 0, st>>>(ga);
        KBBQ_LAUNCHED();
        N = n0;
    }
    if (segmode) {
        seg_prepare_kernel<<<1, 256, 0, st>>>(seg_rows, 2 * R, g.G, (unsigned long long)N, w.seg, w.uni, status);
        KBBQ_LAUNCHED();
    } else {
        rc = run_prepare(rg, second, N, g.G, R, w, status, sms, sl.ngs, g.gbytes, sl.slot, st);
        if (rc) return rc;
    }
    ApplyArgs a;
    a.nsub = segmode ? 2 * R : R; a.segmode = segmode ? 1 : 0;
    a.seq = seq; a.qual = qual; a.out = out_qual; a.total_bytes = N * L; a.g = g; a.t = tc; a.R = R; a.nq = nq;
    a.sl = sl;
    a.entries = w.entries; a.seg = w.seg; a.uni = w.uni; a.fold_cyc = w.fold_cyc; a.fold_din = w.fold_din; a.status = status;
    return launch_apply_smem(a, sms, a.sl.total, st);
}

int kbbq_apply(const uint8_t *seq, const uint8_t *qual, const uint16_t *rg, const uint8_t *second, int64_t N,
               int L, int R, int minscore, const int64_t *meanq, const int64_t *rgdq, const int64_t *qdq,
               const int64_t *posdq, const int64_t *dindq, int nq, int ndin1, uint8_t *out_qual,
               void *workspace, size_t workspace_bytes, int *status, int path, void *stream) {
    return apply_impl(seq, qual, rg, second, N, L, R, minscore, meanq, rgdq, qdq, posdq, dindq, nq, ndin1, out_qual,
                      workspace, workspace_bytes, status, path, stream, nullptr);
}

int kbbq_apply_segmented(const uint8_t *seq, const uint8_t *qual, const uint32_t *seg, int64_t rows_bound, int L, int R,
                         int minscore, const int64_t *meanq, const int64_t *rgdq, const int64_t *qdq,
                         const int64_t *posdq, const int64_t *dindq, int nq, int ndin1, uint8_t *out_qual,
                         void *workspace, size_t workspace_bytes, int *status, void *stream) {
    if (!seg || rows_bound % SEG_ALIGN) return KBBQ_E_ARG;
    return apply_impl(seq, qual, nullptr, nullptr, rows_bound, L, R, minscore, meanq, rgdq, qdq, posdq, dindq, nq, ndin1,
                      out_qual, workspace, workspace_bytes, status, 1, stream, seg);
}


int64_t kbbq_segment_rows_bound(int64_t N, int R) {
    if (N < 0 || R < 1) return -1;
    return (N + SEG_ALIGN - 1) / SEG_ALIGN * SEG_ALIGN + (int64_t)2 * R * SEG_ALIGN;
}

int64_t kbbq_segment_table_elems(int R) { return R < 1 ? -1 : (int64_t)6 * R + 1; }

int kbbq_segmented_supported(int L, int R, int minscore) {
    if (L < 1 || R < 1 || R > 65535) return 0;
    Geom g;
    TableCfg tc;
    StageLayout sl;
    return plan_kernel(L, R, minscore, 3, 232448, &g, &tc, &sl, true) && plan_kernel(L, R, minscore, 2, 232448, &g, &tc, &sl, true);
}

int kbbq_segment_plan(const uint16_t *rg, const uint8_t *second, int64_t N, int R, uint32_t *seg, uint32_t *dest,
                      int *status, void *stream) {
    if (N < 0 || R < 1 || R > 65535 || !seg || !status || (N > 0 && !dest)) return KBBQ_E_ARG;
    if (kbbq_segment_rows_bound(N, R) >= 0xFFFFFFFFll) return KBBQ_E_ARG;
    cudaStream_t st = (cudaStream_t)stream;
    const int nkeys = 2 * R;
    SegPlanArgs a = {rg, second, N, R, seg, seg + 2 * nkeys + 1, dest, status};
    KBBQ_CUDA(cudaMemsetAsync(a.cursor, 0, sizeof(unsigned int) * nkeys, st));
    const int per_thread = 8;
    const long long per_block = (long long)SEG_THREADS * per_thread;
    const unsigned int blocks = (unsigned int)((N + per_block - 1) / per_block);
    const size_t smem = nkeys <= SEG_SMEM_KEYS ? sizeof(unsigned int) * nkeys : 0;
    if (blocks) {
        seg_bucket_kernel<0><<<blocks, SEG_THREADS, smem, st>>>(a, per_thread);
        KBBQ_LAUNCHED();
    }
    seg_scan_kernel<<<1, 1024, 0, st>>>(a);
    KBBQ_LAUNCHED();
    if (blocks) {
        seg_bucket_kernel<1><<<blocks, SEG_THREADS, smem, st>>>(a, per_thread);
        KBBQ_LAUNCHED();
    }
    return KBBQ_OK;
}

static int move_rows(const uint8_t *src, const uint32_t *dest, int64_t N, int L, uint8_t *dst, int64_t src_rows, bool scatter,
                     cudaStream_t st) {
    if (N < 0 || L < 1 || src_rows < 0) return KBBQ_E_ARG;
    if (N == 0) return KBBQ_OK;
    if (!src || !dest || !dst) return KBBQ_E_ARG;
    int device, sms, max_smem;
    int rc = current_device_info(&device, &sms, &max_smem);
    if (rc) return rc;
    const long long warps_per_block = SEG_THREADS / 32;
    const unsigned int blocks = (unsigned int)std::min<long long>((N + warps_per_block - 1) / warps_per_block, (long long)sms * 32);
    if (scatter) seg_move_rows_kernel<true><<<blocks, SEG_THREADS, 0, st>>>(src, dst, dest, N, L, src_rows);
    else seg_move_rows_kernel<false><<<blocks, SEG_THREADS, 0, st>>>(src, dst, dest, N, L, src_rows);
    KBBQ_LAUNCHED();
    return KBBQ_OK;
}

int kbbq_segment_rows(const uint8_t *src, const uint32_t *dest, int64_t N, int L, uint8_t *dst_segmented, void *stream) {
    return move_rows(src, dest, N, L, dst_segmented, N, true, (cudaStream_t)stream);
}

int kbbq_unsegment_rows(const uint8_t *src_segmented, const uint32_t *dest, int64_t N, int L, int64_t rows_bound,
                        uint8_t *dst, void *stream) {
// ... 403 lines not shown
```

kbbq-py_b200/csrc/model.cuh:

```cuda
#pragma once
#include "common.cuh"

namespace kbbq {

__constant__ double c_lnp[NQ];
__constant__ double c_ln1mp[NQ];
__constant__ double c_prior[NQ];
__constant__ double c_p[NQ];
__constant__ double c_bound_hi[NQ];
__constant__ double c_bound_lo[NQ];

struct dd { double hi, lo; };
__device__ __forceinline__ dd two_sum(double a, double b) {
    double s = __dadd_rn(a, b), bb = __dsub_rn(s, a);
    double e = __dadd_rn(__dsub_rn(a, __dsub_rn(s, bb)), __dsub_rn(b, bb));
    return {s, e};
}
__device__ __forceinline__ dd two_prod(double a, double b) {
    double p = __dmul_rn(a, b);
    return {p, __fma_rn(a, b, -p)};
}
__device__ __forceinline__ dd dd_add(dd a, dd b) {
    dd s = two_sum(a.hi, b.hi);
    double lo = __dadd_rn(s.lo, __dadd_rn(a.lo, b.lo));
    return two_sum(s.hi, lo);
}
__device__ __forceinline__ dd dd_div_d(dd a, double b) {
    double q1 = __ddiv_rn(a.hi, b);
    dd p = two_prod(q1, b);
    double r = __dadd_rn(__dsub_rn(__dsub_rn(a.hi, p.hi), p.lo), a.lo);
    double q2 = __ddiv_rn(r, b);
    return two_sum(q1, q2);
}
__device__ __forceinline__ bool dd_le(dd a, double bh, double bl) {
    return a.hi < bh || (a.hi == bh && a.lo <= bl);
}

__global__ void marginals_q_kernel(const long long *pos_errs, const long long *pos_total, int L2,
                                   long long *q_errs, long long *q_total) {
    const int q = blockIdx.x, rg = blockIdx.y;
    const size_t base = ((size_t)rg * NQ + q) * L2;
    long long e = 0, t = 0;
    for (int c = threadIdx.x; c < L2; c += blockDim.x) { e += pos_errs[base + c]; t += pos_total[base + c]; }
    __shared__ long long se[32], st[32];
    for (int o = 16; o; o >>= 1) { e += __shfl_down_sync(0xFFFFFFFFu, e, o); t += __shfl_down_sync(0xFFFFFFFFu, t, o); }
    if ((threadIdx.x & 31) == 0) { se[threadIdx.x >> 5] = e; st[threadIdx.x >> 5] = t; }
    __syncthreads();
    if (threadIdx.x == 0) {
        e = 0; t = 0;
        for (int w = 0; w < (blockDim.x + 31) / 32; ++w) { e += se[w]; t += st[w]; }
        q_errs[rg * NQ + q] = e;
        q_total[rg * NQ + q] = t;
    }
}

__global__ void marginals_rg_kernel(const long long *q_errs, const long long *q_total, int R,
                                    long long *rg_errs, long long *rg_total, long long *meanq) {
    const int rg = blockIdx.x;
    __shared__ long long s_e[NQ], s_t[NQ];
    if (threadIdx.x < NQ) {
        s_e[threadIdx.x] = q_errs[rg * NQ + threadIdx.x];
        s_t[threadIdx.x] = q_total[rg * NQ + threadIdx.x];
    }
    __syncthreads();
    if (threadIdx.x != 0) return;
    long long e = 0, t = 0;
    dd acc = {0.0, 0.0};
    for (int q = 0; q < NQ; ++q) {
        const long long tq = s_t[q];
        e += s_e[q];
        t += tq;
        if (tq) acc = dd_add(acc, two_prod((double)tq, c_p[q]));
    }
    rg_errs[rg] = e;
    rg_total[rg] = t;
    long long mq = 0;
    if (t > 0) {
        if (acc.hi == 0.0) mq = NQ - 1;
        else {
            const dd p = dd_div_d(acc, (double)t);
            for (int m = 1; m < NQ; ++m) mq += dd_le(p, c_bound_hi[m], c_bound_lo[m]) ? 1 : 0;
        }
    }
    meanq[rg] = mq;
}

__device__ __forceinline__ dd round_to_x87(dd s) {
    if (s.lo == 0.0 || isinf(s.hi) || isnan(s.hi)) return s;
    int e;
    frexp(s.hi, &e);
    int eh = e - 1;
    if (fabs(s.hi) == ldexp(1.0, eh) && ((s.hi > 0.0) != (s.lo > 0.0))) eh -= 1;
    const int qe = eh - 63;
    const double lo_r = ldexp(rint(ldexp(s.lo, -qe)), qe);
    const double h = __dadd_rn(s.hi, lo_r);
    return {h, __dadd_rn(__dsub_rn(s.hi, h), lo_r)};
}

template <typename PRIOR>
__device__ __forceinline__ int posterior_q_cell(PRIOR prior, long long errs, long long tot) {
    const double k = (double)(errs + 1), mm = (double)((tot + 2) - (errs + 1));
    int best = 0;
    double bh = 0.0, bl = 0.0;
    bool have = false;
    for (int c = 0; c < NQ; ++c) {
        int d = (int)((PRIOR)c - prior);
        d = d < 0 ? -d : d;
        const double pr = d < NQ ? c_prior[d] : -KBBQ_INF;
        const double a = __dmul_rn(k, c_lnp[c]);
        const double b = (mm == 0.0) ? 0.0 : __dmul_rn(mm, c_ln1mp[c]);
        const double ll = __dadd_rn(a, b);
        double h, l;
        if (isinf(pr) || isinf(ll)) { h = -KBBQ_INF; l = 0.0; }
        else { dd s = round_to_x87(two_sum(pr, ll)); h = s.hi; l = s.lo; }
        if (!have || h > bh || (h == bh && l > bl)) { best = c; bh = h; bl = l; have = true; }
    }
    return best;
}
__device__ __forceinline__ int delta_q_cell(int prior, long long errs, long long tot) {
    return posterior_q_cell<int>(prior, errs, tot) - prior;
}

__global__ void delta_q_kernel(const long long *prior, const long long *errs, const long long *tot,
                               long long n, long long *out) {
    long long i = (long long)blockIdx.x * blockDim.x + threadIdx.x;
    if (i < n) out[i] = delta_q_cell((int)prior[i], errs[i], tot[i]);
}

__global__ void posterior_q_real_kernel(const double *prior, const long long *errs, const long long *tot,
                                        long long n, long long *out) {
    long long i = (long long)blockIdx.x * blockDim.x + threadIdx.x;
    if (i < n) out[i] = posterior_q_cell<double>(prior[i], errs[i], tot[i]);
}

struct DeltaArgs {
    const long long *meanq, *rg_errs, *rg_total, *q_errs, *q_total, *pos_errs, *pos_total, *din_errs, *din_total;
    int R, nq, ncyc, ndin;
    long long *rgdq, *qdq, *posdq, *dindq;
};

__global__ void delta_levels12_kernel(DeltaArgs a) {
    const int rg = blockIdx.x;
    __shared__ int s_prior1;
    if (threadIdx.x == 0) {
        const int mq = (int)a.meanq[rg];
        const int d = delta_q_cell(mq, a.rg_errs[rg], a.rg_total[rg]);
        a.rgdq[rg] = d;
        s_prior1 = mq + d;
    }
    __syncthreads();
    for (int q = threadIdx.x; q < a.nq; q += blockDim.x)
        a.qdq[rg * a.nq + q] = delta_q_cell(s_prior1, a.q_errs[rg * a.nq + q], a.q_total[rg * a.nq + q]);
}

__global__ void delta_level3_kernel(DeltaArgs a) {
    const long long ncell_pos = (long long)a.R * a.nq * a.ncyc;
    const long long ncell_din = (long long)a.R * a.nq * (a.ndin + 1);
    long long i = (long long)blockIdx.x * blockDim.x + threadIdx.x;
    if (i < ncell_pos) {
        const long long gq = i / a.ncyc;
        const int rg = (int)(gq / a.nq);
        const int prior2 = (int)(a.meanq[rg] + a.rgdq[rg] + a.qdq[gq]);
        a.posdq[i] = delta_q_cell(prior2, a.pos_errs[i], a.pos_total[i]);
    } else if (i < ncell_pos + ncell_din) {
        i -= ncell_pos;
        const long long gq = i / (a.ndin + 1);
        const int d = (int)(i - gq * (a.ndin + 1));
        if (d == a.ndin) { a.dindq[i] = 0; return; }
        const int rg = (int)(gq / a.nq);
        const int prior2 = (int)(a.meanq[rg] + a.rgdq[rg] + a.qdq[gq]);
        a.dindq[i] = delta_q_cell(prior2, a.din_errs[gq * a.ndin + d], a.din_total[gq * a.ndin + d]);
    }
}

__global__ void fold_kernel(const long long *meanq, const long long *rgdq, const long long *qdq,
                            const long long *posdq, const long long *dindq, int R, int nq, int L2,
                            int ndin1, short *fold_cyc, short *fold_din) {
    const long long ncyc = (long long)R * NQ * L2, ndin = (long long)R * NQ * 16;
    long long i = (long long)blockIdx.x * blockDim.x + threadIdx.x;
    if (i < ncyc) {
        const long long gq = i / L2;
        const int c2 = (int)(i - gq * L2);
        const int rg = (int)(gq / NQ), q = (int)(gq - (long long)rg * NQ);
        long long v = 0;
        if (q < nq)
            v = meanq[rg] + rgdq[rg] + qdq[rg * nq + q] + posdq[((size_t)rg * nq + q) * L2 + c2] +
                dindq[((size_t)rg * nq + q) * ndin1 + ndin1 - 1];
        fold_cyc[i] = (short)v;
    } else if (i < ncyc + ndin) {
        i -= ncyc;
        const long long gq = i >> 4;
        const int n = (int)(i & 15);
        const int rg = (int)(gq / NQ), q = (int)(gq - (long long)rg * NQ);
        long long v = 0;
        if (q < nq) {
            const size_t row = ((size_t)rg * nq + q) * ndin1;
            v = dindq[row + nat_to_ref(n >> 2) * 4 + nat_to_ref(n & 3)] - dindq[row + ndin1 - 1];
        }
        fold_din[i] = (short)v;
    }
}

}
```

kbbq-py_b200/csrc/prepare.cuh:

```cuda
#pragma once
#include "common.cuh"

namespace kbbq {

constexpr int PREP_THREADS = 256;
constexpr int PREP_SMEM_RG = 8192;

struct PrepArgs {
    const uint16_t *rg;
    const uint8_t *second;
    long long N;
    long long ngroups;
    int G;
    int R;
    unsigned int *seg;
    unsigned int *cursor;
    entry_t *entries;
    unsigned int *uni;
    int *status;
    int grid;
    int ng;
    unsigned int gbytes;
    unsigned int slot;
};

__device__ __forceinline__ entry_t make_entry(unsigned int soff, long long grp, unsigned int match, unsigned int sec) {
    unsigned int f[2] = {0u, 0u};
#pragma unroll
    for (int k = 0; k < MAX_G; ++k) {
        const unsigned int live = (match >> k) & 1u, s2 = (sec >> k) & 1u;
        f[k >> 2] |= (live | ((live & s2) << 1)) << (8 * (k & 3));
    }
    return make_uint4(soff, (unsigned int)grp, f[0], f[1]);
}

__device__ __forceinline__ unsigned long long slice_lo(unsigned long long E, unsigned long long b, int grid) {
    return E * b / (unsigned long long)grid;
}
__device__ __forceinline__ unsigned long long slice_of(unsigned long long E, unsigned long long i, int grid) {
    return ((i + 1) * (unsigned long long)grid + E - 1) / E - 1;
}

__device__ __forceinline__ void load_rows(const PrepArgs &a, long long grp, unsigned int rgv[MAX_G],
                                          unsigned int &sec, unsigned int &exist) {
    sec = 0;
    exist = 0;
#pragma unroll
    for (int k = 0; k < MAX_G; ++k) {
        rgv[k] = 0xFFFFFFFFu;
        if (k < a.G) {
            const long long r = grp * a.G + k;
            if (r < a.N) {
                rgv[k] = a.rg ? a.rg[r] : 0u;
                exist |= 1u << k;
                if (a.second && a.second[r]) sec |= 1u << k;
            }
        }
    }
}

__device__ __forceinline__ void identity_rows(const PrepArgs &a, long long grp, unsigned int &exist, unsigned int &sec,
                                              bool report) {
    unsigned int rgv[MAX_G];
    load_rows(a, grp, rgv, sec, exist);
    if (a.rg) {
        unsigned int ok = 0;
#pragma unroll
        for (int k = 0; k < MAX_G; ++k)
            if ((exist >> k) & 1) {
                if (rgv[k] == 0) ok |= 1u << k;
                else if (report) atomicOr(a.status, KBBQ_FLAG_RG_RANGE);
            }
        exist = ok;
    }
}

__global__ void prep_uniform_kernel(PrepArgs a) {
    const long long t0 = (long long)blockIdx.x * blockDim.x + threadIdx.x;
    const long long stride = (long long)gridDim.x * blockDim.x;
    if (t0 == 0) {
        a.seg[0] = 0;
        a.seg[1] = (unsigned int)a.ngroups;
    }
    unsigned int exist0, sec0;
    identity_rows(a, 0, exist0, sec0, false);
    bool differs = exist0 != (1u << a.G) - 1u;
    for (int k = 2; k < a.G; ++k) differs |= ((sec0 >> k) & 1u) != ((sec0 >> (k & 1)) & 1u);
    const bool wide = (a.G & (a.G - 1)) == 0 && a.G <= 16 && (!a.second || ((uintptr_t)a.second & 15u) == 0) &&
                      (!a.rg || ((uintptr_t)a.rg & 15u) == 0);
    long long done_groups = 0;
    if (wide) {
        const long long chunks = a.N / 16;
        uint4 pat;
        {
            unsigned int v[4];
            for (int j = 0; j < 4; ++j) {
                v[j] = 0;
                for (int k = 0; k < 4; ++k) v[j] |= ((sec0 >> ((4 * j + k) % a.G)) & 1u) << (8 * k);
            }
            pat = make_uint4(v[0], v[1], v[2], v[3]);
        }
        for (long long c = t0; c < chunks; c += stride) {
            if (a.second) {
                const uint4 s = reinterpret_cast<const uint4 *>(a.second)[c];
                auto norm = [](unsigned int x) { return ((x | ((x | 0x80808080u) - 0x01010101u)) >> 7) & 0x01010101u; };
                differs |= norm(s.x) != pat.x || norm(s.y) != pat.y || norm(s.z) != pat.z || norm(s.w) != pat.w;
            } else {
                differs |= sec0 != 0;
            }
            if (a.rg) {
                const uint4 r0 = reinterpret_cast<const uint4 *>(a.rg)[2 * c], r1 = reinterpret_cast<const uint4 *>(a.rg)[2 * c + 1];
                if (r0.x | r0.y | r0.z | r0.w | r1.x | r1.y | r1.z | r1.w) { differs = true; atomicOr(a.status, KBBQ_FLAG_RG_RANGE); }
            }
        }
        done_groups = chunks * 16 / a.G;
    }
    for (long long grp = done_groups + t0; grp < a.ngroups; grp += stride) {
        unsigned int exist, sec;
        identity_rows(a, grp, exist, sec, true);
        differs |= exist != exist0 || sec != sec0;
    }
    if (differs) a.uni[0] = 1u;
    if (t0 == 0) {
        const entry_t p0 = make_entry(0u, 0, exist0, sec0);
        a.uni[1] = p0.z;
        a.uni[2] = p0.w;
    }
}

__global__ void prep_identity_kernel(PrepArgs a) {
    if (a.uni[0] == 0u) return;
    const unsigned long long E = (unsigned long long)a.ngroups;
    for (long long grp = (long long)blockIdx.x * blockDim.x + threadIdx.x; grp < a.ngroups;
         grp += (long long)gridDim.x * blockDim.x) {
        unsigned int exist, sec;
        identity_rows(a, grp, exist, sec, false);
        const unsigned long long lo = slice_lo(E, slice_of(E, (unsigned long long)grp, a.grid), a.grid);
        const unsigned int j = (unsigned int)(((unsigned long long)grp - lo) % (unsigned int)a.ng);
        const unsigned int mis0 = (unsigned int)((((unsigned long long)grp - j) * a.gbytes) & 15ull);
        a.entries[grp] = make_entry(mis0 + j * a.gbytes, grp, exist, sec);
    }
}

template <int MODE>
__global__ void __launch_bounds__(PREP_THREADS) prep_bucket_kernel(PrepArgs a) {
    extern __shared__ unsigned int s_cnt[];
    const bool use_smem = a.R <= PREP_SMEM_RG;
    if (use_smem) {
        for (int i = threadIdx.x; i < a.R; i += blockDim.x) s_cnt[i] = 0;
        __syncthreads();
    }
    const long long grp = (long long)blockIdx.x * blockDim.x + threadIdx.x;
    unsigned int rgv[MAX_G], exist = 0, sec = 0;
    unsigned int slot[MAX_G], mask[MAX_G];
    if (grp < a.ngroups) load_rows(a, grp, rgv, sec, exist);
#pragma unroll
    for (int k = 0; k < MAX_G; ++k) {
        mask[k] = 0;
        slot[k] = 0;
        if (!((exist >> k) & 1)) continue;
        const unsigned int v = rgv[k];
        if (v >= (unsigned int)a.R) {
            atomicOr(a.status, KBBQ_FLAG_RG_RANGE);
            continue;
        }
        bool first = true;
        unsigned int m = 0;
#pragma unroll
        for (int k2 = 0; k2 < MAX_G; ++k2) {
            if (((exist >> k2) & 1) && rgv[k2] == v) {
                if (k2 < k) first = false;
                m |= 1u << k2;
            }
        }
        if (!first) continue;
        mask[k] = m;
        if (use_smem) slot[k] = atomicAdd(&s_cnt[v], 1u);
        else slot[k] = atomicAdd(&a.cursor[v], 1u);
    }
    if (use_smem) {
        __syncthreads();
        for (int i = threadIdx.x; i < a.R; i += blockDim.x) {
            const unsigned int c = s_cnt[i];
            if (c) s_cnt[i] = atomicAdd(&a.cursor[i], c);
        }
        if (MODE == 0) return;
        __syncthreads();
    }
    if (MODE == 1) {
        const unsigned long long E = a.seg[a.R];
#pragma unroll
        for (int k = 0; k < MAX_G; ++k) {
            if (!mask[k]) continue;
            const unsigned int pos = slot[k] + (use_smem ? s_cnt[rgv[k]] : 0u);
            const unsigned long long lo = slice_lo(E, slice_of(E, pos, a.grid), a.grid);
            const unsigned long long start = max((unsigned long long)a.seg[rgv[k]], lo);
            const unsigned int j = (unsigned int)((pos - start) % (unsigned int)a.ng);
            const unsigned int mis = (unsigned int)(((unsigned long long)grp * a.gbytes) & 15ull);
            a.entries[pos] = make_entry(j * a.slot + mis, grp, mask[k], sec);
        }
    }
}

__global__ void prep_scan_kernel(PrepArgs a) {
    __shared__ unsigned int s_part[1024];
    const int T = blockDim.x;
    const int per = (a.R + T - 1) / T;
    const int lo = threadIdx.x * per, hi = min(a.R, lo + per);
    unsigned int sum = 0;
    for (int i = lo; i < hi; ++i) sum += a.cursor[i];
    s_part[threadIdx.x] = sum;
    __syncthreads();
    if (threadIdx.x == 0) {
        unsigned int run = 0;
        for (int t = 0; t < T; ++t) {
            const unsigned int v = s_part[t];
            s_part[t] = run;
            run += v;
        }
        a.seg[a.R] = run;
    }
    __syncthreads();
    unsigned int run = s_part[threadIdx.x];
    for (int i = lo; i < hi; ++i) {
        const unsigned int v = a.cursor[i];
        a.seg[i] = run;
        a.cursor[i] = run;
        run += v;
    }
}

struct Workspace {
    unsigned int *seg;
    unsigned int *cursor;
    unsigned int *uni;
    entry_t *entries;
    short *fold_cyc;
    short *fold_din;
    size_t bytes;
};

inline size_t align_up(size_t v, size_t a) { return (v + a - 1) / a * a; }

inline Workspace carve_workspace(void *base, long long N, int L, int R) {
    Workspace w = {};
    size_t off = 0;
    char *p = (char *)base;
    const size_t max_entries = (size_t)N + MAX_G;
    w.seg = (unsigned int *)(p + off);      off = align_up(off + sizeof(unsigned int) * (2 * (size_t)R + 2), 256);
    w.cursor = (unsigned int *)(p + off);   off = align_up(off + sizeof(unsigned int) * (size_t)R, 256);
    w.uni = (unsigned int *)(p + off);      off = align_up(off + sizeof(unsigned int) * 4, 256);
    w.entries = (entry_t *)(p + off);       off = align_up(off + sizeof(entry_t) * max_entries, 256);
    w.fold_cyc = (short *)(p + off);        off = align_up(off + sizeof(short) * (size_t)R * NQ * 2 * L, 256);
    w.fold_din = (short *)(p + off);        off = align_up(off + sizeof(short) * (size_t)R * NQ * 16, 256);
    w.bytes = off;
    return w;
}

inline int run_prepare(const uint16_t *rg, const uint8_t *second, long long N, int G, int R,
                       const Workspace &w, int *status, int grid, int ng, unsigned int gbytes,
                       unsigned int slot, cudaStream_t st) {
    PrepArgs a;
    a.rg = rg; a.second = second; a.N = N; a.G = G;
    a.ngroups = (N + G - 1) / G; a.R = R;
    a.seg = w.seg; a.cursor = w.cursor; a.entries = w.entries; a.uni = w.uni; a.status = status;
    a.grid = grid; a.ng = ng; a.gbytes = gbytes; a.slot = slot;
    KBBQ_CUDA(cudaMemsetAsync(w.uni, (R == 1 && a.ngroups > 0) ? 0 : 0xFF, sizeof(unsigned int) * 4, st));
    if (a.ngroups == 0) {
        KBBQ_CUDA(cudaMemsetAsync(w.seg, 0, sizeof(unsigned int) * ((size_t)R + 1), st));
        return KBBQ_OK;
    }
    const unsigned int blocks = (unsigned int)((a.ngroups + PREP_THREADS - 1) / PREP_THREADS);
    if (R == 1) {
        const unsigned int few = std::min<unsigned int>(blocks, (unsigned int)std::max(grid, 1) * 8u);
        prep_uniform_kernel<<<few, PREP_THREADS, 0, st>>>(a);
        KBBQ_LAUNCHED();
        prep_identity_kernel<<<few, PREP_THREADS, 0, st>>>(a);
        KBBQ_LAUNCHED();
        return KBBQ_OK;
    }
    const size_t smem = R <= PREP_SMEM_RG ? sizeof(unsigned int) * (size_t)R : 0;
    KBBQ_CUDA(cudaMemsetAsync(w.cursor, 0, sizeof(unsigned int) * (size_t)R, st));
    prep_bucket_kernel<0><<<blocks, PREP_THREADS, smem, st>>>(a);
    KBBQ_LAUNCHED();
    prep_scan_kernel<<<1, 1024, 0, st>>>(a);
    KBBQ_LAUNCHED();
    prep_bucket_kernel<1><<<blocks, PREP_THREADS, smem, st>>>(a);
    KBBQ_LAUNCHED();
    return KBBQ_OK;
}

}
```

kbbq-py_b200/csrc/stage.cuh:

```cuda
#pragma once
#include "common.cuh"
#include "prepare.cuh"

namespace kbbq {

constexpr int MAX_STAGES = 8;

struct StageLayout {
    int stages;
    int kps;
    int ngs;
    int narr;
    int abytes;
    int slot;
    int data_off;
    int hdr_off;
    int bar_off;
    int total;
};

inline StageLayout make_stage_layout(const Geom &g, int narr, int stages, int kps, size_t table_bytes) {
    StageLayout s;
    s.stages = stages;
    s.kps = kps;
    s.ngs = g.ng * kps;
    s.narr = narr;
    s.slot = (g.gbytes + 15 + 15) / 16 * 16;
    s.abytes = g.contig ? (s.ngs * g.gbytes + 32 + 15) / 16 * 16 : (s.ngs * s.slot + 127) / 128 * 128;
    s.data_off = (int)((table_bytes + 127) / 128 * 128);
    s.hdr_off = s.data_off + stages * narr * s.abytes;
    s.bar_off = (s.hdr_off + (g.contig ? 0 : stages * s.ngs * 16) + 15) / 16 * 16;
    s.total = s.bar_off + 2 * stages * 8;
    return s;
}

__device__ __forceinline__ uint32_t smem_u32(const void *p) { return (uint32_t)__cvta_generic_to_shared(p); }

__device__ __forceinline__ void mbar_init(uint32_t bar, uint32_t count) {
    asm volatile("mbarrier.init.shared::cta.b64 [%0], %1;" ::"r"(bar), "r"(count) : "memory");
}
__device__ __forceinline__ void mbar_fence_init() { asm volatile("fence.mbarrier_init.release.cluster;" ::: "memory"); }
__device__ __forceinline__ void mbar_arrive(uint32_t bar) {
    asm volatile("mbarrier.arrive.shared::cta.b64 _, [%0];" ::"r"(bar) : "memory");
}
__device__ __forceinline__ void mbar_arrive_expect_tx(uint32_t bar, uint32_t bytes) {
    asm volatile("mbarrier.arrive.expect_tx.shared::cta.b64 _, [%0], %1;" ::"r"(bar), "r"(bytes) : "memory");
}
__device__ __forceinline__ void mbar_wait(uint32_t bar, uint32_t parity) {
    uint32_t ok;
    do {
        asm volatile(
            "{\n .reg .pred p;\n mbarrier.try_wait.parity.shared::cta.b64 p, [%1], %2;\n selp.u32 %0, 1, 0, p;\n}"
            : "=r"(ok)
            : "r"(bar), "r"(parity)
            : "memory");
    } while (!ok);
}
__device__ __forceinline__ void bulk_g2s(uint32_t dst, const void *src, uint32_t bytes, uint32_t bar) {
    asm volatile("cp.async.bulk.shared::cluster.global.mbarrier::complete_tx::bytes [%0], [%1], %2, [%3];" ::"r"(dst),
                 "l"(src), "r"(bytes), "r"(bar)
                 : "memory");
}
__device__ __forceinline__ void consumer_sync(int nthreads) {
    asm volatile("bar.sync 1, %0;" ::"r"(nthreads) : "memory");
}

struct ProducerArgs {
    const uint8_t *arr[3];
    const entry_t *entries;
    const unsigned int *seg;
    int nsub;
    bool contig;
    uint32_t lo, hi;
    uint32_t gbytes;
    int ng;
    long long total_bytes;
    int pw, nprod;
    bool uniform;
};

__device__ __forceinline__ void mbar_expect_tx(uint32_t bar, uint32_t bytes) {
    asm volatile("mbarrier.expect_tx.relaxed.cta.shared::cta.b64 [%0], %1;" ::"r"(bar), "r"(bytes) : "memory");
}

__device__ __forceinline__ void producer_loop(const ProducerArgs &p, const StageLayout &sl, unsigned char *smem_base) {
    const int lane = threadIdx.x & 31;
    const uint32_t data0 = smem_u32(smem_base + sl.data_off);
    const uint32_t hdr0 = smem_u32(smem_base + sl.hdr_off);
    const uint32_t bar0 = smem_u32(smem_base + sl.bar_off);
    uint32_t stage = 0, phase = 0;
    const unsigned long long end16 = ((unsigned long long)p.total_bytes + 15ull) & ~15ull;

    if (p.contig) {
        if (lane != 0 || p.pw != 0) return;
        for (int sub = 0; sub < p.nsub; ++sub) {
            uint32_t s_lo = p.seg[sub], s_hi = p.seg[sub + 1];
            if (s_hi <= p.lo) continue;
            if (s_lo >= p.hi) break;
            if (s_lo < p.lo) s_lo = p.lo;
            if (s_hi > p.hi) s_hi = p.hi;
            for (uint32_t first = s_lo; first < s_hi; first += p.ng) {
                const uint32_t n = min((uint32_t)p.ng, s_hi - first);
                const uint32_t full = bar0 + stage * 8, empty = bar0 + (sl.stages + stage) * 8;
                const unsigned long long start = (unsigned long long)first * p.gbytes;
                const uint32_t mis = (uint32_t)start & 15u;
                const unsigned long long src = start - mis;
                uint32_t bytes = (mis + n * p.gbytes + 15u) & ~15u;
                bytes = src >= end16 ? 0u : (uint32_t)min((unsigned long long)bytes, end16 - src);
                mbar_wait(empty, phase ^ 1);
                mbar_arrive_expect_tx(full, bytes * sl.narr);
                const uint32_t dst = data0 + stage * sl.narr * sl.abytes;
                if (bytes) {
#pragma unroll
                    for (int k = 0; k < 3; ++k)
                        if (k < sl.narr) bulk_g2s(dst + k * sl.abytes, p.arr[k] + src, bytes, full);
                }
                if (++stage == (uint32_t)sl.stages) { stage = 0; phase ^= 1; }
            }
        }
        return;
    }

    uint32_t it = 0;
    for (int rg = 0; rg < p.nsub; ++rg) {
        uint32_t s_lo = p.seg[rg], s_hi = p.seg[rg + 1];
        if (s_hi <= p.lo) continue;
        if (s_lo >= p.hi) break;
        if (s_lo < p.lo) s_lo = p.lo;
        if (s_hi > p.hi) s_hi = p.hi;
        const uint32_t iters = (s_hi - s_lo + p.ng - 1) / p.ng;
        uint32_t i = (uint32_t)((p.pw + p.nprod - (int)(it % p.nprod)) % p.nprod);
        auto fetch = [&](uint32_t iter) -> uint32_t {
            const unsigned long long e = (unsigned long long)s_lo + (unsigned long long)iter * p.ng + lane;
            return (iter < iters && lane < p.ng && e < s_hi) ? __ldg(&p.entries[e].y) : 0u;
        };
        uint32_t nxt = fetch(i);
        for (; i < iters; i += p.nprod) {
            const uint32_t first = s_lo + i * p.ng;
            const uint32_t grp = nxt;
            nxt = fetch(i + p.nprod);
            const uint32_t g_it = it + i;
            stage = g_it % (uint32_t)sl.stages;
            phase = (g_it / (uint32_t)sl.stages) & 1u;
            const uint32_t n = min((uint32_t)p.ng, s_hi - first);
            const uint32_t full = bar0 + stage * 8, empty = bar0 + (sl.stages + stage) * 8;
            const unsigned long long start = (unsigned long long)grp * p.gbytes;
            const uint32_t mis = (uint32_t)start & 15u;
            const unsigned long long src = start - mis;
            uint32_t bytes = 0;
            if ((uint32_t)lane < n) {
                bytes = (mis + p.gbytes + 15u) & ~15u;
                bytes = src >= end16 ? 0u : (uint32_t)min((unsigned long long)bytes, end16 - src);
            }
            if (lane == 0) mbar_wait(empty, phase ^ 1);
            __syncwarp();
            if (bytes) {
                mbar_expect_tx(full, bytes * sl.narr);
                const uint32_t dst = data0 + stage * sl.narr * sl.abytes + lane * sl.slot;
#pragma unroll
                for (int k = 0; k < 3; ++k)
                    if (k < sl.narr) bulk_g2s(dst + k * sl.abytes, p.arr[k] + src, bytes, full);
            }
            if ((uint32_t)lane >= n && lane < p.ng)
                asm volatile("st.shared.v4.u32 [%0], {%1, %1, %1, %1};" ::"r"(hdr0 + (stage * p.ng + lane) * 16u), "r"(0u) : "memory");
            if (lane == 0) {
                mbar_expect_tx(full, n * 16u);
                bulk_g2s(hdr0 + stage * p.ng * 16u, p.entries + first, n * 16u, full);
            }
            __syncwarp();
            if (lane == 0) mbar_arrive(full);
        }
        it += iters;
    }
}

}
```

kbbq-py_b200/kbbq/_native.py:

```python
import ctypes as C
import os

import numpy as np

HERE = os.path.dirname(os.path.abspath(__file__))
LIB_PATH = os.path.join(HERE, "libkbbq_b200.so")

NQ = 43
FLAG_QUAL_RANGE, FLAG_BAD_BASE, FLAG_RG_RANGE, FLAG_SEGMENTS = 1, 2, 4, 8
E_DATA = -4
E_UNSUPPORTED = -12

_lib = None

_vp, _i, _i64, _sz = C.c_void_p, C.c_int, C.c_int64, C.c_size_t
SIGNATURES = {
    "kbbq_abi_version": (_i, []),
    "kbbq_strerror": (C.c_char_p, [_i]),
    "kbbq_last_cuda_error": (C.c_char_p, []),
    "kbbq_pos_table_elems": (_i64, [_i, _i]),
    "kbbq_din_table_elems": (_i64, [_i]),
    "kbbq_workspace_bytes": (_i, [_i64, _i, _i, C.POINTER(_sz)]),
    "kbbq_build": (_i, [_vp] * 5 + [_i64, _i, _i, _i] + [_vp] * 4 + [_vp, _sz, _vp, _i, _vp]),
    "kbbq_marginals": (_i, [_vp, _vp, _i, _i] + [_vp] * 5 + [_vp]),
    "kbbq_delta_q": (_i, [_vp, _vp, _vp, _i64, _vp, _vp]),
    "kbbq_get_delta_qs": (_i, [_vp] * 9 + [_i, _i, _i, _i] + [_vp] * 4 + [_vp]),
    "kbbq_apply": (_i, [_vp] * 4 + [_i64, _i, _i, _i] + [_vp] * 5 + [_i, _i, _vp, _vp, _sz, _vp, _i, _vp]),
    "kbbq_recalibrate_host": (_i, [_vp] * 5 + [_i64, _i, _i, _i] + [_vp] * 3 + [C.POINTER(_i), _i]),
    "kbbq_recalibrate_host_multi": (_i, [_vp] * 5 + [_i64, _i, _i, _i] + [_vp] * 3 + [C.POINTER(_i), C.POINTER(_i), _i]),
    "kbbq_recalibrate_fastq": (_i, [C.c_char_p, C.c_char_p, _i, _i, _i, _i, _i, C.POINTER(_i64), C.POINTER(_i), C.POINTER(_i)]),
    "kbbq_host_release": (_i, [_i]),
    "kbbq_session_create": (_i, [_i, _i, _i, _i, _i64, _i64, _i, C.POINTER(_vp)]),
    "kbbq_session_destroy": (None, [_vp]),
    "kbbq_session_chunk_reads": (_i64, [_vp]),
    "kbbq_session_reset": (_i, [_vp]),
    "kbbq_session_build_chunk": (_i, [_vp] * 6 + [_i64, _i]),
    "kbbq_session_build_range": (_i, [_vp] * 6 + [_i64]),
    "kbbq_session_tables": (_i, [_vp, _vp]),
    "kbbq_session_set_tables": (_i, [_vp, _vp]),
    "kbbq_session_tables_dev": (_i, [_vp, C.POINTER(_vp), C.POINTER(_i64), C.POINTER(_vp)]),
    "kbbq_session_model": (_i, [_vp, _vp]),
    "kbbq_session_apply_resident": (_i, [_vp, _i64, _vp]),
    "kbbq_session_apply_chunk": (_i, [_vp] * 5 + [_i64, _vp]),
    "kbbq_session_flush": (_i, [_vp]),
    "kbbq_session_sync": (_i, [_vp, C.POINTER(_i)]),
    "kbbq_session_traffic": (_i, [_vp, C.POINTER(_i64), C.POINTER(_i64)]),
    "kbbq_build_host": (_i, [_vp] * 5 + [_i64, _i, _i, _i] + [_vp] * 4 + [C.POINTER(_i), _i]),
    "kbbq_apply_host": (_i, [_vp] * 4 + [_i64, _i, _i, _i] + [_vp] * 5 + [_i, _i, _vp, C.POINTER(_i), _i]),
    "kbbq_get_delta_qs_host": (_i, [_vp] * 9 + [_i, _i, _i, _i] + [_vp] * 4 + [_i]),
    "kbbq_delta_q_host": (_i, [_vp, _vp, _vp, _i64, _vp, _i]),
    "kbbq_posterior_q_real": (_i, [_vp, _vp, _vp, _i64, _vp, _vp]),
    "kbbq_posterior_q_real_host": (_i, [_vp, _vp, _vp, _i64, _vp, _i]),
    "kbbq_calibration_counts": (_i, [_vp] * 5 + [_i64, _vp, _vp, _vp]),
    "kbbq_calibration_counts_host": (_i, [_vp] * 5 + [_i64, _vp, _vp, _i]),
    "kbbq_bam_workspace_bytes": (_i, [_i64, _i, _i, C.POINTER(_sz)]),
    "kbbq_build_bam": (_i, [_vp] * 8 + [_i64, _i, _i, _i] + [_vp] * 4 + [_vp, _sz, _vp, _vp]),
    "kbbq_apply_bam": (_i, [_vp] * 4 + [_i64, _i, _i, _i] + [_vp] * 5 + [_i, _i, _vp, _vp, _sz, _vp, _vp]),
    "kbbq_build_bam_host": (_i, [_vp] * 8 + [_i64, _i, _i, _i] + [_vp] * 4 + [_vp, _i]),
    "kbbq_apply_bam_host": (_i, [_vp] * 4 + [_i64, _i, _i, _i] + [_vp] * 5 + [_i, _i, _vp, _vp, _i]),
    "kbbq_marginals_host": (_i, [_vp, _vp, _i, _i] + [_vp] * 5 + [_i]),
    "kbbq_synth_reads": (_i, [C.c_uint64, _i64, _i64, _i, _i] + [_vp] * 5 + [_vp]),
    "kbbq_launch_count": (_i64, []),
    "kbbq_fastq_open": (_i, [C.c_char_p, _i, C.POINTER(_vp)]),
    "kbbq_fastq_open_mem": (_i, [_vp, _sz, _i, C.POINTER(_vp)]),
    "kbbq_fastq_close": (None, [_vp]),
    "kbbq_fastq_num_reads": (_i64, [_vp]),
    "kbbq_fastq_read_len": (_i, [_vp]),
    "kbbq_fastq_pack": (_i, [_vp, _i64, _i64, _vp, _vp, _i]),
    "kbbq_fastq_name": (_i, [_vp, _i64, C.POINTER(C.c_char_p), C.POINTER(_i)]),
    "kbbq_fastq_infer": (_i, [_vp, _i, _vp, _vp, C.POINTER(_i), _i]),
    "kbbq_fastq_rg_key": (_i, [_vp, _i, C.POINTER(C.c_char_p), C.POINTER(_i)]),
    "kbbq_fastq_check_names": (_i, [_vp, _vp, _i64, _i, C.POINTER(_i64)]),
    "kbbq_fastq_write": (_i, [_i, _vp, _i64, _i64, _vp, _i]),
    "kbbq_fastq_format_size": (_i, [_vp, _i64, _i64, _i, C.POINTER(_i64)]),
    "kbbq_fastq_format": (_i, [_vp, _i64, _i64, _vp, _vp, _i64, _i]),
    "kbbq_host_mismatch_bits": (_i, [_vp, _vp, _i64, _vp, _i]),
    "kbbq_expand_mismatch_bits": (_i, [_vp, _vp, _i64, _vp, _vp]),
    "kbbq_host_last_traffic": (_i, [_i, C.POINTER(_i64), C.POINTER(_i64)]),
    "kbbq_host_pack_mode": (_i, [_i]),
    "kbbq_host_pack_nibbles": (_i, [_vp, _vp, _i64, _vp, _i, _vp]),
    "kbbq_expand_nibbles": (_i, [_vp, _i64, _vp, _vp, _vp]),
    "kbbq_plan_info": (_i, [_i, _i, _i, _i, _i, C.POINTER(_i)]),
    "kbbq_segment_rows_bound": (_i64, [_i64, _i]),
    "kbbq_segment_table_elems": (_i64, [_i]),
    "kbbq_segmented_supported": (_i, [_i, _i, _i]),
    "kbbq_segment_plan": (_i, [_vp, _vp, _i64, _i, _vp, _vp, _vp, _vp]),
    "kbbq_segment_rows": (_i, [_vp, _vp, _i64, _i, _vp, _vp]),
    "kbbq_segment_pad": (_i, [_vp, _i, _i, _vp, _vp, _vp, _vp]),
    "kbbq_unsegment_rows": (_i, [_vp, _vp, _i64, _i, _i64, _vp, _vp]),
    "kbbq_build_segmented": (_i, [_vp] * 4 + [_i64, _i, _i, _i] + [_vp] * 4 + [_vp, _sz, _vp, _vp]),
    "kbbq_apply_segmented": (_i, [_vp] * 3 + [_i64, _i, _i, _i] + [_vp] * 5 + [_i, _i, _vp, _vp, _sz, _vp, _vp]),
}


class KbbqNativeError(RuntimeError):
    """The CUDA library is missing, or a CUDA / argument error came back from it."""


def lib():
    global _lib
    if _lib is None:
        if not os.path.exists(LIB_PATH):
            raise KbbqNativeError(
                "%s not found: build it with `python -c 'import __graft_entry__ as g; g.build()'` "
                "(or make -C kbbq-py_b200/csrc). kbbq_b200 has no CPU fallback." % LIB_PATH)
        handle = C.CDLL(LIB_PATH)
        for name, (res, args) in SIGNATURES.items():
# ... 326 lines not shown
```

kbbq-py_b200/kbbq/device.py:

```python
import ctypes as C

import torch

from . import _native
from . import parallel

NQ = _native.NQ


def _p(t):
    return None if t is None else C.c_void_p(t.data_ptr())


def _on_device(fn):
    import functools

    @functools.wraps(fn)
    def wrapper(self, *args, **kwargs):
        with torch.cuda.device(self.device):
            return fn(self, *args, **kwargs)
    return wrapper


class SegmentedBatch:
# ... 33 lines not shown
        self.ws_reads = -1
        self._ensure_workspace(max_reads)

    @_on_device
    def _ensure_workspace(self, n_reads):
        if n_reads <= self.ws_reads:
            return
        nbytes = C.c_size_t(0)
        _native.check(self.lib.kbbq_workspace_bytes(n_reads, self.L, self.R, C.byref(nbytes)))
        self.workspace = torch.empty(max(nbytes.value, 256), dtype=torch.uint8, device=self.device)
        self.ws_bytes = nbytes.value
        self.ws_reads = n_reads

    def _stream(self):
        return C.c_void_p(torch.cuda.current_stream(self.device).cuda_stream)

    def reset(self):
        self.tables.zero_()
        self.status.zero_()

    @_on_device
    def build(self, seq, qual, corr, rg=None, second=None, path=0):
        N = seq.numel() // self.L
        self._ensure_workspace(N)
        rc = self.lib.kbbq_build(_p(seq), _p(qual), _p(corr), _p(rg), _p(second), N, self.L, self.R, self.minscore,
                                 _p(self.pos_errs), _p(self.pos_total), _p(self.din_errs), _p(self.din_total),
                                 _p(self.workspace), self.ws_bytes, _p(self.status), path, self._stream())
        _native.check(rc)

    @_on_device
    def build_from_bits(self, seq, qual, bits, corr_scratch, rg=None, second=None):
        _native.check(self.lib.kbbq_expand_mismatch_bits(_p(seq), _p(bits), seq.numel(), _p(corr_scratch), self._stream()))
        self.build(seq, qual, corr_scratch, rg, second)

    @_on_device
    def segment(self, seq, qual, corr=None, rg=None, second=None):
        N, L, R = seq.numel() // self.L, self.L, self.R
        if not self.lib.kbbq_segmented_supported(L, R, self.minscore):
            raise _native.KbbqNativeError("no shared-memory plan for L=%d, R=%d: use build() / apply()" % (L, R))
        rows = int(self.lib.kbbq_segment_rows_bound(N, R))
        dev, st = self.device, self._stream()
        seg = torch.empty(int(self.lib.kbbq_segment_table_elems(R)), dtype=torch.int32, device=dev)
        dest = torch.empty(max(N, 1), dtype=torch.int32, device=dev)
        _native.check(self.lib.kbbq_segment_plan(_p(rg), _p(second), N, R, _p(seg), _p(dest), _p(self.status), st))
        outs = []
        for src in (seq, qual, corr):
            if src is None:
                outs.append(None)
                continue
            dst = torch.empty(rows * L + 16, dtype=torch.uint8, device=dev)
            _native.check(self.lib.kbbq_segment_rows(_p(src), _p(dest), N, L, _p(dst), st))
            outs.append(dst)
        _native.check(self.lib.kbbq_segment_pad(_p(seg), R, L, _p(outs[0]), _p(outs[1]), _p(outs[2]), st))
        return SegmentedBatch(outs[0], outs[1], outs[2], seg, dest, N, rows)

    @_on_device
    def build_segmented(self, sb):
        self._ensure_workspace(sb.rows_bound)
        rc = self.lib.kbbq_build_segmented(_p(sb.seq), _p(sb.qual), _p(sb.corr), _p(sb.seg), sb.rows_bound, self.L, self.R,
                                           self.minscore, _p(self.pos_errs), _p(self.pos_total), _p(self.din_errs),
                                           _p(self.din_total), _p(self.workspace), self.ws_bytes, _p(self.status),
                                           self._stream())
        _native.check(rc)

    @_on_device
    def apply_segmented(self, sb, out_seg):
        self._ensure_workspace(sb.rows_bound)
        rc = self.lib.kbbq_apply_segmented(_p(sb.seq), _p(sb.qual), _p(sb.seg), sb.rows_bound, self.L, self.R, self.minscore,
                                           _p(self.meanq), _p(self.rgdq), _p(self.qdq), _p(self.posdq), _p(self.dindq),
                                           NQ, 17, _p(out_seg), _p(self.workspace), self.ws_bytes, _p(self.status),
                                           self._stream())
        _native.check(rc)

    @_on_device
    def unsegment(self, sb, out_seg, out):
        _native.check(self.lib.kbbq_unsegment_rows(_p(out_seg), _p(sb.dest), sb.N, self.L, sb.rows_bound, _p(out),
                                                   self._stream()))

    def allreduce(self):
        parallel.allreduce_tables(self.tables, self.pg)

    @_on_device
    def model(self):
        L, R = self.L, self.R
        _native.check(self.lib.kbbq_marginals(_p(self.pos_errs), _p(self.pos_total), L, R, _p(self.q_errs),
                                              _p(self.q_total), _p(self.rg_errs), _p(self.rg_total),
                                              _p(self.meanq), self._stream()))
        _native.check(self.lib.kbbq_get_delta_qs(_p(self.meanq), _p(self.rg_errs), _p(self.rg_total),
                                                 _p(self.q_errs), _p(self.q_total), _p(self.pos_errs),
                                                 _p(self.pos_total), _p(self.din_errs), _p(self.din_total),
                                                 R, NQ, 2 * L, 16, _p(self.rgdq), _p(self.qdq), _p(self.posdq),
                                                 _p(self.dindq), self._stream()))

    @_on_device
    def apply(self, seq, qual, out, rg=None, second=None, path=0):
        N = seq.numel() // self.L
        self._ensure_workspace(N)
        rc = self.lib.kbbq_apply(_p(seq), _p(qual), _p(rg), _p(second), N, self.L, self.R, self.minscore,
                                 _p(self.meanq), _p(self.rgdq), _p(self.qdq), _p(self.posdq), _p(self.dindq),
                                 NQ, 17, _p(out), _p(self.workspace), self.ws_bytes, _p(self.status), path,
                                 self._stream())
        _native.check(rc)

    @_on_device
    def build_bam(self, seq, qual, err, skip=None, rg=None, flags=None, aln_start=None, aln_end=None, fast=True):
        N = seq.numel() // self.L
        ws = self._bam_workspace(N) if fast else None
        rc = self.lib.kbbq_build_bam(_p(seq), _p(qual), _p(err), _p(skip), _p(rg), _p(flags), _p(aln_start),
                                     _p(aln_end), N, self.L, self.R, self.minscore, _p(self.pos_errs),
                                     _p(self.pos_total), _p(self.din_errs), _p(self.din_total), _p(ws),
                                     0 if ws is None else ws.numel(), _p(self.status), self._stream())
        _native.check(rc)

    @_on_device
    def _bam_workspace(self, n_reads):
        if n_reads > getattr(self, "bam_ws_reads", -1):
            nbytes = C.c_size_t(0)
            _native.check(self.lib.kbbq_bam_workspace_bytes(n_reads, self.L, self.R, C.byref(nbytes)))
            self.bam_ws = torch.empty(max(nbytes.value, 256), dtype=torch.uint8, device=self.device)
            self.bam_ws_reads = n_reads
        return self.bam_ws

    @_on_device
    def apply_bam(self, seq, qual, out, rg=None, flags=None, fast=True):
        N = seq.numel() // self.L
        ws = self._bam_workspace(N) if fast else None
        rc = self.lib.kbbq_apply_bam(_p(seq), _p(qual), _p(rg), _p(flags), N, self.L, self.R, self.minscore,
                                     _p(self.meanq), _p(self.rgdq), _p(self.qdq), _p(self.posdq), _p(self.dindq),
                                     NQ, 17, _p(out), _p(ws), 0 if ws is None else ws.numel(), _p(self.status),
                                     self._stream())
        _native.check(rc)

    @_on_device
    def check_status(self):
        st = int(self.status.item())
        if st:
            _native.raise_for_status(st)

    def covariate_arrays(self):
        self.model()
        return tuple(t.cpu().numpy().copy() for t in (self.meanq, self.rg_errs, self.rg_total, self.q_errs,
                                                      self.q_total, self.pos_errs, self.pos_total,
                                                      self.din_errs, self.din_total))

    def delta_qs(self):
        return tuple(t.cpu().numpy().copy() for t in (self.rgdq, self.qdq, self.posdq, self.dindq))


def calibration_counts(qual, err=None, seq=None, corr=None, skip=None, total=None, errs=None):
    lib = _native.lib()
    dev = qual.device
    torch.cuda.set_device(dev)
    if total is None:
        total = torch.zeros(256, dtype=torch.int64, device=dev)
    if errs is None:
        errs = torch.zeros(256, dtype=torch.int64, device=dev)
    rc = lib.kbbq_calibration_counts(_p(qual), _p(err), _p(seq), _p(corr), _p(skip), qual.numel(), _p(total),
                                     _p(errs), C.c_void_p(torch.cuda.current_stream(dev).cuda_stream))
    _native.check(rc)
    return total, errs


def synth_reads(seed, first_read, n, L, R, device=None, want_corr=True):
    lib = _native.lib()
    dev = torch.device("cuda", torch.cuda.current_device()) if device is None else torch.device(device)
    torch.cuda.set_device(dev)
    seq = torch.empty(n, L, dtype=torch.uint8, device=dev)
    qual = torch.empty(n, L, dtype=torch.uint8, device=dev)
    corr = torch.empty(n, L, dtype=torch.uint8, device=dev)
    rg = torch.empty(n, dtype=torch.int16, device=dev)
    second = torch.empty(n, dtype=torch.uint8, device=dev)
    rc = lib.kbbq_synth_reads(seed, first_read, n, L, R, _p(seq), _p(qual), _p(corr), _p(rg), _p(second),
                              C.c_void_p(torch.cuda.current_stream(dev).cuda_stream))
    _native.check(rc)
    return seq, qual, corr, rg, second
# ... 1 lines not shown
```

Baseline: 870.7 billion.

## Fuse model into one kernel and drop R==1 prep and fold tables

Combines the marginals and delta-q steps into a single model kernel with several CTAs per read group. For the single-read-group case it skips the prepare kernels: entry records are computed inline from rg/second, and uniformity is checked per slice inside the main kernels. The apply path now reads delta tables directly instead of going through materialised fold_cyc/fold_din buffers. Uniform slices also get a separate, less frequent position-flush interval. The goal is fewer launches and less global traffic, at the cost of extra per-block scanning and more complex index math.

```diff
diff --git a/include/kbbq_b200.h b/include/kbbq_b200.h
--- a/include/kbbq_b200.h
+++ b/include/kbbq_b200.h
@@ -48,6 +48,11 @@
 int kbbq_marginals(const int64_t *pos_errs_dev, const int64_t *pos_total_dev, int L, int R,
                    int64_t *q_errs_dev, int64_t *q_total_dev, int64_t *rg_errs_dev,
                    int64_t *rg_total_dev, int64_t *meanq_dev, void *stream);
+
+int kbbq_model(const int64_t *pos_errs_dev, const int64_t *pos_total_dev, const int64_t *din_errs_dev,
+               const int64_t *din_total_dev, int L, int R, int64_t *q_errs_dev, int64_t *q_total_dev,
+               int64_t *rg_errs_dev, int64_t *rg_total_dev, int64_t *meanq_dev, int64_t *rgdq_dev,
+               int64_t *qdq_dev, int64_t *posdq_dev, int64_t *dindq_dev, void *stream);
 
 int kbbq_delta_q(const int64_t *prior_q_dev, const int64_t *numerrs_dev,
                  const int64_t *numtotal_dev, int64_t n, int64_t *delta_dev, void *stream);
diff --git a/kbbq-py_b200/csrc/apply.cuh b/kbbq-py_b200/csrc/apply.cuh
--- a/kbbq-py_b200/csrc/apply.cuh
+++ b/kbbq-py_b200/csrc/apply.cuh
@@ -17,10 +17,25 @@
     const entry_t *entries;
     const unsigned int *seg;
     const unsigned int *uni;
-    const short *fold_cyc;
-    const short *fold_din;
+    uint32_t E1;
+    const uint16_t *rg;
+    const uint8_t *second;
+    long long nrows;
+    int ndin1;
+    const long long *meanq, *rgdq, *qdq, *posdq, *dindq;
     int *status;
 };
+
+__device__ __forceinline__ int fold_cyc_cell(const long long *meanq, const long long *rgdq, const long long *qdq,
+                                             const long long *posdq, const long long *dindq, int rg, int nq, int q,
+                                             int L2, int ndin1, int c2) {
+    const size_t gq = (size_t)rg * nq + q;
+    return (short)(meanq[rg] + rgdq[rg] + qdq[gq] + posdq[gq * L2 + c2] + dindq[gq * ndin1 + ndin1 - 1]);
+}
+__device__ __forceinline__ int fold_din_cell(const long long *dindq, int rg, int nq, int q, int ndin1, int n) {
+    const long long *row = dindq + ((size_t)rg * nq + q) * ndin1;
+    return (short)(row[nat_to_ref(n >> 2) * 4 + nat_to_ref(n & 3)] - row[ndin1 - 1]);
+}
 
 static_assert((offsetof(ApplyArgs, t) + offsetof(TableCfg, ohe)) % 16 == 0,
               "ApplyArgs: TableCfg::ohe has to be 16-byte aligned in the kernel parameters (build.cuh); pad Geom");
@@ -71,7 +86,7 @@
         hs1 = (int)(((uni_flo >> 8) & 0xFFu) >> 1);
     }
     for (int sub = 0; sub < a.nsub; ++sub) {
-        uint32_t s_lo = a.seg[sub], s_hi = a.seg[sub + 1];
+        uint32_t s_lo = a.seg ? a.seg[sub] : 0u, s_hi = a.seg ? a.seg[sub + 1] : a.E1;
         if (s_hi <= lo) continue;
         if (s_lo >= hi) break;
         if (s_lo < lo) s_lo = lo;
@@ -88,19 +103,19 @@
                 reinterpret_cast<int *>(smem_raw)[i] = i * 4 < t.din_off && (i * 4) % t.revoff < t.rs ? g.minscore - 1 : 0;
             consumer_sync(nconsumers);
             const int L = g.L, L2 = 2 * g.L;
-            const short *fc = a.fold_cyc + (size_t)rg * NQ * L2;
             for (int i = threadIdx.x; i < 2 * (t.nrows - 1) * L; i += nconsumers) {
                 const int slot = i >= (t.nrows - 1) * L, j = i - slot * (t.nrows - 1) * L;
-                const int r = j / L + 1, c = j - (r - 1) * L;
+                const int r = j / L + 1, c = j - (r - 1) * L, q = r + g.minscore - 1;
                 const int half = slot ? hs1 : hs0;
                 int *p = reinterpret_cast<int *>(smem_raw + t.pos_off + slot * t.revoff + r * t.rs) + ((c & 3) * t.sj + (c >> 2));
-                *p = fc[(size_t)(r + g.minscore - 1) * L2 + (half ? L2 - 1 - c : c)];
-            }
-            const short *fd = a.fold_din + (size_t)rg * NQ * DIN_SLOTS;
+                *p = q < a.nq ? fold_cyc_cell(a.meanq, a.rgdq, a.qdq, a.posdq, a.dindq, rg, a.nq, q, L2, a.ndin1,
+                                              half ? L2 - 1 - c : c)
+                              : 0;
+            }
             for (int i = threadIdx.x; i < (t.nrows - 1) * DIN_SLOTS * t.drep; i += nconsumers) {
-                const int cell = i / t.drep, r = cell / DIN_SLOTS + 1, s = cell & (DIN_SLOTS - 1);
+                const int cell = i / t.drep, r = cell / DIN_SLOTS + 1, s = cell & (DIN_SLOTS - 1), q = r + g.minscore - 1;
                 int *p = reinterpret_cast<int *>(smem_raw + t.din_off + r * t.dq + s * (t.drep * 4)) + (i & (t.drep - 1));
-                *p = fd[(r + g.minscore - 1) * DIN_SLOTS + s];
+                *p = q < a.nq ? fold_din_cell(a.dindq, rg, a.nq, q, a.ndin1, s) : 0;
             }
             consumer_sync(nconsumers);
         }
@@ -175,7 +190,8 @@
                         uint32_t flo, fhi;
                         if (g.contig) {
                             const uint32_t e = first + (uint32_t)m.grp + (uint32_t)(k * g.ng);
-                            const uint4 rec = e < s_hi ? __ldg(a.entries + e) : make_uint4(0u, 0u, 0u, 0u);
+                            const uint4 rec = e < s_hi ? identity_record(a.rg, a.second, a.nrows, g.G, g.gbytes, first, e)
+                                                       : make_uint4(0u, 0u, 0u, 0u);
                             soff = rec.x; hgrp = rec.y; flo = rec.z; fhi = rec.w;
                         } else {
                             asm volatile("ld.shared.v4.u32 {%0, %1, %2, %3}, [%4];"
@@ -210,10 +226,9 @@
     const StageLayout &sl = a.sl;
     const int nconsumers = g.threads;
 
-    const unsigned long long E = a.seg[a.nsub];
+    const unsigned long long E = a.seg ? a.seg[a.nsub] : a.E1;
     const uint32_t lo = (uint32_t)(E * blockIdx.x / gridDim.x), hi = (uint32_t)(E * (blockIdx.x + 1) / gridDim.x);
     const bool contig = a.R == 1 || a.segmode;
-    const bool uniform = contig && a.uni[0] == 0u;
 
     const uint32_t bar0 = smem_u32(smem_raw + sl.bar_off);
     if (threadIdx.x == 0) {
@@ -231,12 +246,13 @@
         p.entries = a.entries; p.seg = a.seg; p.nsub = a.nsub; p.contig = contig; p.lo = lo; p.hi = hi;
         p.gbytes = g.gbytes; p.ng = sl.ngs; p.total_bytes = a.total_bytes;
         p.pw = ((int)threadIdx.x - nconsumers) >> 5; p.nprod = g.nprod;
-        p.uniform = uniform;
+        p.E1 = a.E1;
         producer_loop(p, sl, smem_raw);
         return;
     }
 
-    if (uniform) apply_consume<KPS, true>(a, smem_raw, lo, hi, a.uni[1], a.uni[2]);
+    uint32_t flo = 0, fhi = 0;
+    if (uniform_walk(a, lo, hi, nconsumers, flo, fhi)) apply_consume<KPS, true>(a, smem_raw, lo, hi, flo, fhi);
     else apply_consume<KPS, false>(a, smem_raw, lo, hi, 0u, 0u);
 }
 
@@ -246,8 +262,8 @@
     const uint8_t *second;
     uint8_t *out;
     long long N;
-    int L, R, minscore, nq;
-    const short *fold_cyc, *fold_din;
+    int L, R, minscore, nq, ndin1;
+    const long long *meanq, *rgdq, *qdq, *posdq, *dindq;
     int *status;
 };
 
@@ -263,11 +279,10 @@
         const unsigned int g = a.rg ? a.rg[r] : 0;
         if (g >= (unsigned int)a.R) { atomicOr(a.status, KBBQ_FLAG_RG_RANGE); a.out[i] = (uint8_t)q; continue; }
         const int c2 = (a.second && a.second[r]) ? 2 * a.L - 1 - c : c;
-        const size_t gq = (size_t)g * NQ + q;
-        int v = a.fold_cyc[gq * (2 * a.L) + c2];
+        int v = fold_cyc_cell(a.meanq, a.rgdq, a.qdq, a.posdq, a.dindq, (int)g, a.nq, (int)q, 2 * a.L, a.ndin1, c2);
         if (c > 0) {
             const uint8_t s = a.seq[i], ps = a.seq[i - 1];
-            if (s != 'N' && ps != 'N') v += a.fold_din[gq * DIN_SLOTS + ((((ps >> 1) & 3) << 2) | ((s >> 1) & 3))];
+            if (s != 'N' && ps != 'N') v += fold_din_cell(a.dindq, (int)g, a.nq, (int)q, a.ndin1, (((ps >> 1) & 3) << 2) | ((s >> 1) & 3));
         }
         a.out[i] = (uint8_t)v;
     }
diff --git a/kbbq-py_b200/csrc/build.cuh b/kbbq-py_b200/csrc/build.cuh
--- a/kbbq-py_b200/csrc/build.cuh
+++ b/kbbq-py_b200/csrc/build.cuh
@@ -27,6 +27,7 @@
     uint32_t din16;
     uint32_t ohe[4];
     uint32_t val16[2];
+    int flush_pos_par;
 };
 
 inline int cycle_table_wavefronts(const Geom &g, int sj, int rs_words, int shift, bool word_owner) {
@@ -80,6 +81,7 @@
     t->din_off = (t->revoff + t->nrows * t->rs + 127) / 128 * 128;
     t->table_bytes = t->din_off + t->nrows * t->dq;
     t->flush_pos = std::max(1, (int)((ERR_UNIT - 1) / (uint32_t)(kps * g.ng * g.G)));
+    t->flush_pos_par = std::max(1, (int)((ERR_UNIT - 1) / (uint32_t)(kps * g.ng * ((g.G + 1) / 2))));
     t->fold_din = std::max(1, (int)((ERR_UNIT - 1) / (uint32_t)(kps * 4 * ((g.threads + drep - 1) / drep))));
     t->addq = (uint32_t)(0x81 - g.minscore) * ONE4;
     t->cyc16[0] = (uint32_t)t->rs;
@@ -103,6 +105,10 @@
     const entry_t *entries;
     const unsigned int *seg;
     const unsigned int *uni;
+    uint32_t E1;
+    const uint16_t *rg;
+    const uint8_t *second;
+    long long nrows;
     unsigned long long *pos_errs, *pos_total, *din_errs, *din_total;
     int *status;
 };
@@ -281,6 +287,7 @@
     int cur_rg = -1, cur_sub = -1;
     int hs0 = 0, hs1 = 1;
     uint32_t since_pos = 0, since_din = 0;
+    const uint32_t flush_every = (uint32_t)(UNI ? t.flush_pos_par : t.flush_pos);
     auto flush_all = [&](int rg) {
         consumer_sync(nconsumers);
         flush_pos_table(a, smem_raw, rg, nconsumers, hs0, hs1);
@@ -294,7 +301,7 @@
     }
 
     for (int sub = 0; sub < a.nsub; ++sub) {
-        uint32_t s_lo = a.seg[sub], s_hi = a.seg[sub + 1];
+        uint32_t s_lo = a.seg ? a.seg[sub] : 0u, s_hi = a.seg ? a.seg[sub + 1] : a.E1;
         if (s_hi <= lo) continue;
         if (s_lo >= hi) break;
         if (s_lo < lo) s_lo = lo;
@@ -307,13 +314,13 @@
         if (a.segmode) hs0 = hs1 = sub & 1;
 
         for (uint32_t first = s_lo; first < s_hi;) {
-            if (since_pos >= (uint32_t)t.flush_pos || since_din >= (uint32_t)t.fold_din) {
+            if (since_pos >= flush_every || since_din >= (uint32_t)t.fold_din) {
                 consumer_sync(nconsumers);
-                if (since_pos >= (uint32_t)t.flush_pos) { flush_pos_table(a, smem_raw, rg, nconsumers, hs0, hs1); since_pos = 0; }
+                if (since_pos >= flush_every) { flush_pos_table(a, smem_raw, rg, nconsumers, hs0, hs1); since_pos = 0; }
                 if (since_din >= (uint32_t)t.fold_din) { fold_din_replicas(a, smem_raw, rg, nconsumers); since_din = 0; }
                 consumer_sync(nconsumers);
             }
-            const uint32_t room = min((uint32_t)t.flush_pos - since_pos, (uint32_t)t.fold_din - since_din);
+            const uint32_t room = min(flush_every - since_pos, (uint32_t)t.fold_din - since_din);
             const uint32_t chunk_end = (uint32_t)min((unsigned long long)s_hi, (unsigned long long)first + (unsigned long long)room * sl.ngs);
             const uint32_t iters = (chunk_end - first + ngs - 1) / ngs;
             since_pos += iters;
@@ -381,7 +388,8 @@
                             uint32_t hgrp, flo, fhi;
                             if (g.contig) {
                                 const uint32_t e = first + (uint32_t)m.grp + (uint32_t)(k * g.ng);
-                                const uint4 rec = e < s_hi ? __ldg(a.entries + e) : make_uint4(0u, 0u, 0u, 0u);
+                                const uint4 rec = e < s_hi ? identity_record(a.rg, a.second, a.nrows, g.G, g.gbytes, first, e)
+                                                           : make_uint4(0u, 0u, 0u, 0u);
                                 soff = rec.x; hgrp = rec.y; flo = rec.z; fhi = rec.w;
                             } else {
                                 asm volatile("ld.shared.v4.u32 {%0, %1, %2, %3}, [%4];"
@@ -412,6 +420,18 @@
 }
 
 
+template <class ARGS>
+__device__ __forceinline__ bool uniform_walk(const ARGS &a, uint32_t lo, uint32_t hi, int nconsumers, uint32_t &flo,
+                                             uint32_t &fhi) {
+    if (a.segmode) {
+        flo = a.uni[1];
+        fhi = a.uni[2];
+        return a.uni[0] == 0u;
+    }
+    if (a.R != 1) return false;
+    return slice_uniform(a.rg, a.second, a.nrows, a.g.G, lo, hi, nconsumers, a.status, flo, fhi);
+}
+
 template <int KPS, bool VALIDATE>
 __global__ void __launch_bounds__(MAX_THREADS, 1) build_smem_kernel(const __grid_constant__ BuildArgs a) {
     extern __shared__ __align__(128) unsigned char smem_raw[];
@@ -419,10 +439,9 @@
     const StageLayout &sl = a.sl;
     const int nconsumers = g.threads;
 
-    const unsigned long long E = a.seg[a.nsub];
+    const unsigned long long E = a.seg ? a.seg[a.nsub] : a.E1;
     const uint32_t lo = (uint32_t)(E * blockIdx.x / gridDim.x), hi = (uint32_t)(E * (blockIdx.x + 1) / gridDim.x);
     const bool contig = a.R == 1 || a.segmode;
-    const bool uniform = contig && a.uni[0] == 0u;
 
     const uint32_t bar0 = smem_u32(smem_raw + sl.bar_off);
     if (threadIdx.x == 0) {
@@ -440,12 +459,13 @@
         p.entries = a.entries; p.seg = a.seg; p.nsub = a.nsub; p.contig = contig; p.lo = lo; p.hi = hi;
         p.gbytes = g.gbytes; p.ng = sl.ngs; p.total_bytes = a.total_bytes;
         p.pw = ((int)threadIdx.x - nconsumers) >> 5; p.nprod = g.nprod;
-        p.uniform = uniform;
+        p.E1 = a.E1;
         producer_loop(p, sl, smem_raw);
         return;
     }
 
-    if (uniform) build_consume<KPS, VALIDATE, true>(a, smem_raw, lo, hi, a.uni[1], a.uni[2]);
+    uint32_t flo = 0, fhi = 0;
+    if (uniform_walk(a, lo, hi, nconsumers, flo, fhi)) build_consume<KPS, VALIDATE, true>(a, smem_raw, lo, hi, flo, fhi);
     else build_consume<KPS, VALIDATE, false>(a, smem_raw, lo, hi, 0u, 0u);
 }
 
diff --git a/kbbq-py_b200/csrc/host_api.cu b/kbbq-py_b200/csrc/host_api.cu
--- a/kbbq-py_b200/csrc/host_api.cu
+++ b/kbbq-py_b200/csrc/host_api.cu
@@ -364,10 +364,8 @@
     const size_t npos = (size_t)R * NQ * 2 * L, ndin = (size_t)R * NQ * 16;
     int64_t *pe = S->summed ? S->d_sum : S->d_tab, *pt = pe + npos, *de = pt + npos, *dt = de + ndin;
     const ModelPtrs &mp = S->mp;
-    KBBQ_TRY(kbbq_marginals(pe, pt, L, R, mp.q_errs, mp.q_total, mp.rg_errs, mp.rg_total, mp.meanq, S->s_comp));
-    KBBQ_TRY(kbbq_get_delta_qs(mp.meanq, mp.rg_errs, mp.rg_total, mp.q_errs, mp.q_total, pe, pt, de, dt, R, NQ, 2 * L, 16,
-                               mp.rgdq, mp.qdq, mp.posdq, mp.dindq, S->s_comp));
-    return KBBQ_OK;
+    return kbbq_model(pe, pt, de, dt, L, R, mp.q_errs, mp.q_total, mp.rg_errs, mp.rg_total, mp.meanq, mp.rgdq, mp.qdq,
+                      mp.posdq, mp.dindq, S->s_comp);
 }
 
 int apply_and_download(kbbq_session *S, const uint8_t *d_seq, const uint8_t *d_qual, const uint16_t *d_rg,
diff --git a/kbbq-py_b200/csrc/kbbq_b200.cu b/kbbq-py_b200/csrc/kbbq_b200.cu
--- a/kbbq-py_b200/csrc/kbbq_b200.cu
+++ b/kbbq-py_b200/csrc/kbbq_b200.cu
@@ -239,15 +239,18 @@
             KBBQ_LAUNCHED();
             N = n0;
         }
-        rc = run_prepare(rg, second, N, g.G, R, w, status, sms, sl.ngs, g.gbytes, sl.slot, st);
-        if (rc) return rc;
+        if (R > 1) {
+            rc = run_prepare(rg, second, N, g.G, R, w, status, sms, sl.ngs, g.gbytes, sl.slot, st);
+            if (rc) return rc;
+        }
     }
 
     BuildArgs a;
     a.seq = seq; a.qual = qual; a.corr = corr; a.total_bytes = N * L; a.g = g; a.t = tc; a.R = R;
     a.nsub = segmode ? 2 * R : R; a.segmode = segmode ? 1 : 0;
     a.sl = sl;
-    a.entries = w.entries; a.seg = w.seg; a.uni = w.uni;
+    a.entries = w.entries; a.seg = (R == 1 && !segmode) ? nullptr : w.seg; a.uni = w.uni;
+    a.E1 = (uint32_t)((N + g.G - 1) / g.G); a.rg = rg; a.second = second; a.nrows = N;
     a.pos_errs = (unsigned long long *)pos_errs; a.pos_total = (unsigned long long *)pos_total;
     a.din_errs = (unsigned long long *)din_errs; a.din_total = (unsigned long long *)din_total;
     a.status = status;
@@ -271,50 +274,85 @@
                       din_total, workspace, workspace_bytes, status, 1, stream, seg);
 }
 
+static int model_ctas_per_rg(long long ncell, int R, int sms) {
+    const long long want = std::max(1LL, (ncell + 127) / 128);
+    const long long cap = std::max(1LL, 4LL * sms / R);
+    return (int)std::min(want, cap);
+}
+
+static int launch_model(const ModelArgs &a0, bool from_pos, cudaStream_t st) {
+    int device, sms, max_smem;
+    int rc = current_device_info(&device, &sms, &max_smem);
+    if (rc) return rc;
+    rc = upload_constants(device);
+    if (rc) return rc;
+    ModelArgs a = a0;
+    const long long ncell = (long long)a.nq * (a.ncyc + a.ndin + 1);
+    a.nx = a.deltas ? model_ctas_per_rg(ncell, a.R, sms) : 1;
+    const size_t smem = sizeof(int) * (size_t)a.nq;
+    const unsigned int grid = (unsigned int)((long long)a.nx * a.R);
+    if (from_pos) model_kernel<true><<<grid, MODEL_THREADS, smem, st>>>(a);
+    else model_kernel<false><<<grid, MODEL_THREADS, smem, st>>>(a);
+    KBBQ_LAUNCHED();
+    return KBBQ_OK;
+}
+
 int kbbq_marginals(const int64_t *pos_errs, const int64_t *pos_total, int L, int R, int64_t *q_errs,
                    int64_t *q_total, int64_t *rg_errs, int64_t *rg_total, int64_t *meanq, void *stream) {
-    if (L < 1 || R < 1 || !pos_errs || !pos_total || !q_errs || !q_total || !rg_errs || !rg_total || !meanq)
+    if (L < 1 || R < 1 || R > 65535 || !pos_errs || !pos_total || !q_errs || !q_total || !rg_errs || !rg_total ||
+        !meanq)
         return KBBQ_E_ARG;
-    cudaStream_t st = (cudaStream_t)stream;
-    int device;
-    KBBQ_CUDA(cudaGetDevice(&device));
-    int rc = upload_constants(device);
+    ModelArgs a = {};
+    a.pos_errs = (const long long *)pos_errs; a.pos_total = (const long long *)pos_total;
+    a.q_errs = (long long *)q_errs; a.q_total = (long long *)q_total; a.rg_errs = (long long *)rg_errs;
+    a.rg_total = (long long *)rg_total; a.meanq = (long long *)meanq;
+    a.R = R; a.nq = NQ; a.ncyc = 2 * L; a.ndin = 16; a.deltas = 0;
+    return launch_model(a, true, (cudaStream_t)stream);
+}
+
+int kbbq_model(const int64_t *pos_errs, const int64_t *pos_total, const int64_t *din_errs, const int64_t *din_total,
+               int L, int R, int64_t *q_errs, int64_t *q_total, int64_t *rg_errs, int64_t *rg_total, int64_t *meanq,
+               int64_t *rgdq, int64_t *qdq, int64_t *posdq, int64_t *dindq, void *stream) {
+    if (L < 1 || R < 1 || R > 65535 || !pos_errs || !pos_total || !din_errs || !din_total || !q_errs || !q_total ||
+        !rg_errs || !rg_total || !meanq || !rgdq || !qdq || !posdq || !dindq)
+        return KBBQ_E_ARG;
+    ModelArgs a = {(const long long *)pos_errs, (const long long *)pos_total, (const long long *)din_errs,
+                   (const long long *)din_total, (long long *)q_errs, (long long *)q_total, (long long *)rg_errs,
+                   (long long *)rg_total, (long long *)meanq, R, NQ, 2 * L, 16, 0, 1,
+                   (long long *)rgdq, (long long *)qdq, (long long *)posdq, (long long *)dindq};
+    return launch_model(a, true, (cudaStream_t)stream);
+}
+
+}
+
+template <typename IN, typename PRIOR, bool DELTA>
+static int launch_cells(const IN *prior, const int64_t *numerrs, const int64_t *numtotal, int64_t n, int64_t *out,
+                        void *stream) {
+    if (n < 0 || (n > 0 && (!prior || !numerrs || !numtotal || !out))) return KBBQ_E_ARG;
+    if (n == 0) return KBBQ_OK;
+    int device, sms, max_smem;
+    int rc = current_device_info(&device, &sms, &max_smem);
     if (rc) return rc;
-    marginals_q_kernel<<<dim3(NQ, R), 128, 0, st>>>((const long long *)pos_errs, (const long long *)pos_total,
-                                                   2 * L, (long long *)q_errs, (long long *)q_total);
-    KBBQ_LAUNCHED();
-    marginals_rg_kernel<<<R, 64, 0, st>>>((const long long *)q_errs, (const long long *)q_total, R,
-                                                      (long long *)rg_errs, (long long *)rg_total, (long long *)meanq);
-    KBBQ_LAUNCHED();
-    return KBBQ_OK;
-}
+    rc = upload_constants(device);
+    if (rc) return rc;
+    const long long cells_per_cta = 2 * (MODEL_THREADS / 32);
+    const unsigned int grid = (unsigned int)std::min<long long>((n + cells_per_cta - 1) / cells_per_cta, (long long)sms * 32);
+    posterior_cells_kernel<IN, PRIOR, DELTA><<<grid, MODEL_THREADS, 0, (cudaStream_t)stream>>>(
+        prior, (const long long *)numerrs, (const long long *)numtotal, n, (long long *)out);
+    KBBQ_LAUNCHED();
+    return KBBQ_OK;
+}
+
+extern "C" {
 
 int kbbq_delta_q(const int64_t *prior_q, const int64_t *numerrs, const int64_t *numtotal, int64_t n,
                  int64_t *delta, void *stream) {
-    if (n < 0 || (n > 0 && (!prior_q || !numerrs || !numtotal || !delta))) return KBBQ_E_ARG;
-    if (n == 0) return KBBQ_OK;
-    int device;
-    KBBQ_CUDA(cudaGetDevice(&device));
-    int rc = upload_constants(device);
-    if (rc) return rc;
-    delta_q_kernel<<<(unsigned)((n + 127) / 128), 128, 0, (cudaStream_t)stream>>>(
-        (const long long *)prior_q, (const long long *)numerrs, (const long long *)numtotal, n, (long long *)delta);
-    KBBQ_LAUNCHED();
-    return KBBQ_OK;
+    return launch_cells<long long, int, true>((const long long *)prior_q, numerrs, numtotal, n, delta, stream);
 }
 
 int kbbq_posterior_q_real(const double *prior_q, const int64_t *numerrs, const int64_t *numtotal, int64_t n,
                           int64_t *posterior, void *stream) {
-    if (n < 0 || (n > 0 && (!prior_q || !numerrs || !numtotal || !posterior))) return KBBQ_E_ARG;
-    if (n == 0) return KBBQ_OK;
-    int device;
-    KBBQ_CUDA(cudaGetDevice(&device));
-    int rc = upload_constants(device);
-    if (rc) return rc;
-    posterior_q_real_kernel<<<(unsigned)((n + 127) / 128), 128, 0, (cudaStream_t)stream>>>(
-        prior_q, (const long long *)numerrs, (const long long *)numtotal, n, (long long *)posterior);
-    KBBQ_LAUNCHED();
-    return KBBQ_OK;
+    return launch_cells<double, double, false>(prior_q, numerrs, numtotal, n, posterior, stream);
 }
 
 struct BamWorkspace {
@@ -474,21 +512,12 @@
     if (!meanq || !rg_errs || !rg_total || !q_errs || !q_total || !rgdq || !qdq) return KBBQ_E_ARG;
     if ((ncyc && (!pos_errs || !pos_total || !posdq)) || !dindq || (ndin && (!din_errs || !din_total)))
         return KBBQ_E_ARG;
-    int device;
-    KBBQ_CUDA(cudaGetDevice(&device));
-    int rc = upload_constants(device);
-    if (rc) return rc;
-    cudaStream_t st = (cudaStream_t)stream;
-    DeltaArgs a = {(const long long *)meanq, (const long long *)rg_errs, (const long long *)rg_total,
-                   (const long long *)q_errs, (const long long *)q_total, (const long long *)pos_errs,
-                   (const long long *)pos_total, (const long long *)din_errs, (const long long *)din_total,
-                   R, nq, ncyc, ndin, (long long *)rgdq, (long long *)qdq, (long long *)posdq, (long long *)dindq};
-    delta_levels12_kernel<<<R, 64, 0, st>>>(a);
-    KBBQ_LAUNCHED();
-    const long long cells = (long long)R * nq * (ncyc + ndin + 1);
-    delta_level3_kernel<<<(unsigned)((cells + 127) / 128), 128, 0, st>>>(a);
-    KBBQ_LAUNCHED();
-    return KBBQ_OK;
+    if (nq > 12288) return KBBQ_E_ARG;
+    ModelArgs a = {(const long long *)pos_errs, (const long long *)pos_total, (const long long *)din_errs,
+                   (const long long *)din_total, (long long *)q_errs, (long long *)q_total, (long long *)rg_errs,
+                   (long long *)rg_total, (long long *)meanq, R, nq, ncyc, ndin, 0, 1,
+                   (long long *)rgdq, (long long *)qdq, (long long *)posdq, (long long *)dindq};
+    return launch_model(a, false, (cudaStream_t)stream);
 }
 
 static int apply_impl(const uint8_t *seq, const uint8_t *qual, const uint16_t *rg, const uint8_t *second, int64_t N,
@@ -508,12 +537,8 @@
     if (rc) return rc;
     Workspace w = carve_workspace(workspace, N, L, R);
     if (!workspace || workspace_bytes < w.bytes) return KBBQ_E_WORKSPACE;
-
-    const long long fold_cells = (long long)R * NQ * (2 * L + 16);
-    fold_kernel<<<(unsigned)((fold_cells + 255) / 256), 256, 0, st>>>(
-        (const long long *)meanq, (const long long *)rgdq, (const long long *)qdq, (const long long *)posdq,
-        (const long long *)dindq, R, nq, 2 * L, ndin1, w.fold_cyc, w.fold_din);
-    KBBQ_LAUNCHED();
+    const long long *dm = (const long long *)meanq, *dr = (const long long *)rgdq, *dqq = (const long long *)qdq,
+                    *dp = (const long long *)posdq, *dd_ = (const long long *)dindq;
 
     Geom g;
     TableCfg tc;
@@ -523,7 +548,7 @@
                          (uint64_t)((N + g.G - 1) / g.G) < 0xFFFFFFFFull;
     if (!smem_ok) {
         if (path == 1 || segmode) return KBBQ_E_ARG;
-        ApplyGenericArgs a = {seq, qual, rg, second, out_qual, N, L, R, minscore, nq, w.fold_cyc, w.fold_din, status};
+        ApplyGenericArgs a = {seq, qual, rg, second, out_qual, N, L, R, minscore, nq, ndin1, dm, dr, dqq, dp, dd_, status};
         apply_generic_kernel<<<sms * 8, 256, 0, st>>>(a);
         KBBQ_LAUNCHED();
         return KBBQ_OK;
@@ -532,7 +557,7 @@
     if (tail) {
         const int64_t n0 = N - tail;
         ApplyGenericArgs ga = {seq + n0 * L, qual + n0 * L, rg ? rg + n0 : nullptr, second ? second + n0 : nullptr,
-                               out_qual + n0 * L, tail, L, R, minscore, nq, w.fold_cyc, w.fold_din, status};
+                               out_qual + n0 * L, tail, L, R, minscore, nq, ndin1, dm, dr, dqq, dp, dd_, status};
         apply_generic_kernel<<<1, 256, 0, st>>>(ga);
         KBBQ_LAUNCHED();
         N = n0;
@@ -540,7 +565,7 @@
     if (segmode) {
         seg_prepare_kernel<<<1, 256, 0, st>>>(seg_rows, 2 * R, g.G, (unsigned long long)N, w.seg, w.uni, status);
         KBBQ_LAUNCHED();
-    } else {
+    } else if (R > 1) {
         rc = run_prepare(rg, second, N, g.G, R, w, status, sms, sl.ngs, g.gbytes, sl.slot, st);
         if (rc) return rc;
     }
@@ -548,7 +573,9 @@
     a.nsub = segmode ? 2 * R : R; a.segmode = segmode ? 1 : 0;
     a.seq = seq; a.qual = qual; a.out = out_qual; a.total_bytes = N * L; a.g = g; a.t = tc; a.R = R; a.nq = nq;
     a.sl = sl;
-    a.entries = w.entries; a.seg = w.seg; a.uni = w.uni; a.fold_cyc = w.fold_cyc; a.fold_din = w.fold_din; a.status = status;
+    a.entries = w.entries; a.seg = (R == 1 && !segmode) ? nullptr : w.seg; a.uni = w.uni; a.status = status;
+    a.E1 = (uint32_t)((N + g.G - 1) / g.G); a.rg = rg; a.second = second; a.nrows = N;
+    a.ndin1 = ndin1; a.meanq = dm; a.rgdq = dr; a.qdq = dqq; a.posdq = dp; a.dindq = dd_;
     return launch_apply_smem(a, sms, a.sl.total, st);
 }
 
diff --git a/kbbq-py_b200/csrc/model.cuh b/kbbq-py_b200/csrc/model.cuh
--- a/kbbq-py_b200/csrc/model.cuh
+++ b/kbbq-py_b200/csrc/model.cuh
@@ -34,55 +34,6 @@
 }
 __device__ __forceinline__ bool dd_le(dd a, double bh, double bl) {
     return a.hi < bh || (a.hi == bh && a.lo <= bl);
-}
-
-__global__ void marginals_q_kernel(const long long *pos_errs, const long long *pos_total, int L2,
-                                   long long *q_errs, long long *q_total) {
-    const int q = blockIdx.x, rg = blockIdx.y;
-    const size_t base = ((size_t)rg * NQ + q) * L2;
-    long long e = 0, t = 0;
-    for (int c = threadIdx.x; c < L2; c += blockDim.x) { e += pos_errs[base + c]; t += pos_total[base + c]; }
-    __shared__ long long se[32], st[32];
-    for (int o = 16; o; o >>= 1) { e += __shfl_down_sync(0xFFFFFFFFu, e, o); t += __shfl_down_sync(0xFFFFFFFFu, t, o); }
-    if ((threadIdx.x & 31) == 0) { se[threadIdx.x >> 5] = e; st[threadIdx.x >> 5] = t; }
-    __syncthreads();
-    if (threadIdx.x == 0) {
-        e = 0; t = 0;
-        for (int w = 0; w < (blockDim.x + 31) / 32; ++w) { e += se[w]; t += st[w]; }
-        q_errs[rg * NQ + q] = e;
-        q_total[rg * NQ + q] = t;
-    }
-}
-
-__global__ void marginals_rg_kernel(const long long *q_errs, const long long *q_total, int R,
-                                    long long *rg_errs, long long *rg_total, long long *meanq) {
-    const int rg = blockIdx.x;
-    __shared__ long long s_e[NQ], s_t[NQ];
-    if (threadIdx.x < NQ) {
-        s_e[threadIdx.x] = q_errs[rg * NQ + threadIdx.x];
-        s_t[threadIdx.x] = q_total[rg * NQ + threadIdx.x];
-    }
-    __syncthreads();
-    if (threadIdx.x != 0) return;
-    long long e = 0, t = 0;
-    dd acc = {0.0, 0.0};
-    for (int q = 0; q < NQ; ++q) {
-        const long long tq = s_t[q];
-        e += s_e[q];
-        t += tq;
-        if (tq) acc = dd_add(acc, two_prod((double)tq, c_p[q]));
-    }
-    rg_errs[rg] = e;
-    rg_total[rg] = t;
-    long long mq = 0;
-    if (t > 0) {
-        if (acc.hi == 0.0) mq = NQ - 1;
-        else {
-            const dd p = dd_div_d(acc, (double)t);
-            for (int m = 1; m < NQ; ++m) mq += dd_le(p, c_bound_hi[m], c_bound_lo[m]) ? 1 : 0;
-        }
-    }
-    meanq[rg] = mq;
 }
 
 __device__ __forceinline__ dd round_to_x87(dd s) {
@@ -97,108 +48,216 @@
     return {h, __dadd_rn(__dsub_rn(s.hi, h), lo_r)};
 }
 
+constexpr int CAND_LANES = 16;
+constexpr int CAND_PER_LANE = (NQ + CAND_LANES - 1) / CAND_LANES;
+constexpr int MODEL_THREADS = 512;
+
+struct Cands { double lnp[CAND_PER_LANE], ln1mp[CAND_PER_LANE]; };
+__device__ __forceinline__ Cands load_cands() {
+    Cands k;
+    const int s = threadIdx.x & (CAND_LANES - 1);
+#pragma unroll
+    for (int j = 0; j < CAND_PER_LANE; ++j) {
+        const int c = s + CAND_LANES * j;
+        k.lnp[j] = c < NQ ? c_lnp[c] : 0.0;
+        k.ln1mp[j] = c < NQ ? c_ln1mp[c] : 0.0;
+    }
+    return k;
+}
+__device__ __forceinline__ void load_prior_table(double *s_prior) {
+    for (int i = threadIdx.x; i < NQ; i += blockDim.x) s_prior[i] = c_prior[i];
+}
+
 template <typename PRIOR>
-__device__ __forceinline__ int posterior_q_cell(PRIOR prior, long long errs, long long tot) {
+__device__ __forceinline__ int posterior_q_cell(PRIOR prior, long long errs, long long tot, const Cands &cd,
+                                                const double *s_prior) {
+    const int s = threadIdx.x & (CAND_LANES - 1);
     const double k = (double)(errs + 1), mm = (double)((tot + 2) - (errs + 1));
-    int best = 0;
+    int best = s;
     double bh = 0.0, bl = 0.0;
-    bool have = false;
-    for (int c = 0; c < NQ; ++c) {
+#pragma unroll
+    for (int j = 0; j < CAND_PER_LANE; ++j) {
+        const int c = s + CAND_LANES * j;
+        if (c >= NQ) break;
         int d = (int)((PRIOR)c - prior);
         d = d < 0 ? -d : d;
-        const double pr = d < NQ ? c_prior[d] : -KBBQ_INF;
-        const double a = __dmul_rn(k, c_lnp[c]);
-        const double b = (mm == 0.0) ? 0.0 : __dmul_rn(mm, c_ln1mp[c]);
+        const double pr = d < NQ ? s_prior[d] : -KBBQ_INF;
+        const double a = __dmul_rn(k, cd.lnp[j]);
+        const double b = (mm == 0.0) ? 0.0 : __dmul_rn(mm, cd.ln1mp[j]);
         const double ll = __dadd_rn(a, b);
         double h, l;
         if (isinf(pr) || isinf(ll)) { h = -KBBQ_INF; l = 0.0; }
-        else { dd s = round_to_x87(two_sum(pr, ll)); h = s.hi; l = s.lo; }
-        if (!have || h > bh || (h == bh && l > bl)) { best = c; bh = h; bl = l; have = true; }
+        else { dd x = round_to_x87(two_sum(pr, ll)); h = x.hi; l = x.lo; }
+        if (j == 0 || h > bh || (h == bh && l > bl)) { best = c; bh = h; bl = l; }
+    }
+#pragma unroll
+    for (int o = CAND_LANES / 2; o; o >>= 1) {
+        const double oh = __shfl_xor_sync(0xFFFFFFFFu, bh, o), ol = __shfl_xor_sync(0xFFFFFFFFu, bl, o);
+        const int oc = __shfl_xor_sync(0xFFFFFFFFu, best, o);
+        if (oh > bh || (oh == bh && (ol > bl || (ol == bl && oc < best)))) { bh = oh; bl = ol; best = oc; }
     }
     return best;
 }
-__device__ __forceinline__ int delta_q_cell(int prior, long long errs, long long tot) {
-    return posterior_q_cell<int>(prior, errs, tot) - prior;
-}
-
-__global__ void delta_q_kernel(const long long *prior, const long long *errs, const long long *tot,
-                               long long n, long long *out) {
-    long long i = (long long)blockIdx.x * blockDim.x + threadIdx.x;
-    if (i < n) out[i] = delta_q_cell((int)prior[i], errs[i], tot[i]);
-}
-
-__global__ void posterior_q_real_kernel(const double *prior, const long long *errs, const long long *tot,
-                                        long long n, long long *out) {
-    long long i = (long long)blockIdx.x * blockDim.x + threadIdx.x;
-    if (i < n) out[i] = posterior_q_cell<double>(prior[i], errs[i], tot[i]);
-}
-
-struct DeltaArgs {
-    const long long *meanq, *rg_errs, *rg_total, *q_errs, *q_total, *pos_errs, *pos_total, *din_errs, *din_total;
+
+template <typename IN, typename PRIOR, bool DELTA>
+__global__ void __launch_bounds__(MODEL_THREADS) posterior_cells_kernel(const IN *prior, const long long *errs,
+                                                                        const long long *tot, long long n, long long *out) {
+    __shared__ double s_prior[NQ];
+    load_prior_table(s_prior);
+    __syncthreads();
+    const Cands cd = load_cands();
+    const int half = (threadIdx.x >> 4) & 1;
+    const long long wpb = blockDim.x >> 5, stride = 2 * (long long)gridDim.x * wpb;
+    for (long long i0 = 2 * ((long long)blockIdx.x * wpb + (threadIdx.x >> 5)); i0 < n; i0 += stride) {
+        const long long i = i0 + half;
+        const bool v = i < n;
+        const PRIOR p = v ? (PRIOR)prior[i] : (PRIOR)0;
+        const int r = posterior_q_cell<PRIOR>(p, v ? errs[i] : 0, v ? tot[i] : 0, cd, s_prior);
+        if (v && (threadIdx.x & (CAND_LANES - 1)) == 0) out[i] = DELTA ? (long long)(r - (int)p) : (long long)r;
+    }
+}
+
+struct ModelArgs {
+    const long long *pos_errs, *pos_total, *din_errs, *din_total;
+    long long *q_errs, *q_total, *rg_errs, *rg_total, *meanq;
     int R, nq, ncyc, ndin;
+    int nx;
+    int deltas;
     long long *rgdq, *qdq, *posdq, *dindq;
 };
 
-__global__ void delta_levels12_kernel(DeltaArgs a) {
-    const int rg = blockIdx.x;
-    __shared__ int s_prior1;
-    if (threadIdx.x == 0) {
-        const int mq = (int)a.meanq[rg];
-        const int d = delta_q_cell(mq, a.rg_errs[rg], a.rg_total[rg]);
-        a.rgdq[rg] = d;
-        s_prior1 = mq + d;
-    }
-    __syncthreads();
-    for (int q = threadIdx.x; q < a.nq; q += blockDim.x)
-        a.qdq[rg * a.nq + q] = delta_q_cell(s_prior1, a.q_errs[rg * a.nq + q], a.q_total[rg * a.nq + q]);
-}
-
-__global__ void delta_level3_kernel(DeltaArgs a) {
-    const long long ncell_pos = (long long)a.R * a.nq * a.ncyc;
-    const long long ncell_din = (long long)a.R * a.nq * (a.ndin + 1);
-    long long i = (long long)blockIdx.x * blockDim.x + threadIdx.x;
-    if (i < ncell_pos) {
-        const long long gq = i / a.ncyc;
-        const int rg = (int)(gq / a.nq);
-        const int prior2 = (int)(a.meanq[rg] + a.rgdq[rg] + a.qdq[gq]);
-        a.posdq[i] = delta_q_cell(prior2, a.pos_errs[i], a.pos_total[i]);
-    } else if (i < ncell_pos + ncell_din) {
-        i -= ncell_pos;
-        const long long gq = i / (a.ndin + 1);
-        const int d = (int)(i - gq * (a.ndin + 1));
-        if (d == a.ndin) { a.dindq[i] = 0; return; }
-        const int rg = (int)(gq / a.nq);
-        const int prior2 = (int)(a.meanq[rg] + a.rgdq[rg] + a.qdq[gq]);
-        a.dindq[i] = delta_q_cell(prior2, a.din_errs[gq * a.ndin + d], a.din_total[gq * a.ndin + d]);
-    }
-}
-
-__global__ void fold_kernel(const long long *meanq, const long long *rgdq, const long long *qdq,
-                            const long long *posdq, const long long *dindq, int R, int nq, int L2,
-                            int ndin1, short *fold_cyc, short *fold_din) {
-    const long long ncyc = (long long)R * NQ * L2, ndin = (long long)R * NQ * 16;
-    long long i = (long long)blockIdx.x * blockDim.x + threadIdx.x;
-    if (i < ncyc) {
-        const long long gq = i / L2;
-        const int c2 = (int)(i - gq * L2);
-        const int rg = (int)(gq / NQ), q = (int)(gq - (long long)rg * NQ);
-        long long v = 0;
-        if (q < nq)
-            v = meanq[rg] + rgdq[rg] + qdq[rg * nq + q] + posdq[((size_t)rg * nq + q) * L2 + c2] +
-                dindq[((size_t)rg * nq + q) * ndin1 + ndin1 - 1];
-        fold_cyc[i] = (short)v;
-    } else if (i < ncyc + ndin) {
-        i -= ncyc;
-        const long long gq = i >> 4;
-        const int n = (int)(i & 15);
-        const int rg = (int)(gq / NQ), q = (int)(gq - (long long)rg * NQ);
-        long long v = 0;
-        if (q < nq) {
-            const size_t row = ((size_t)rg * nq + q) * ndin1;
-            v = dindq[row + nat_to_ref(n >> 2) * 4 + nat_to_ref(n & 3)] - dindq[row + ndin1 - 1];
-        }
-        fold_din[i] = (short)v;
-    }
-}
-
-}
+template <bool FROM_POS>
+__global__ void __launch_bounds__(MODEL_THREADS) model_kernel(const ModelArgs a) {
+    extern __shared__ int s_prior2[];
+    __shared__ double s_prior[NQ], s_ph[NQ], s_pl[NQ];
+    __shared__ long long s_qe[NQ], s_qt[NQ];
+    __shared__ long long s_rg[4];
+    const int rg = blockIdx.x / a.nx, x = blockIdx.x - rg * a.nx;
+    const int tid = threadIdx.x, lane = tid & 31, warp = tid >> 5, half = lane >> 4, nwarps = blockDim.x >> 5;
+    const bool lead = (lane & (CAND_LANES - 1)) == 0;
+    const int nq = a.nq;
+    load_prior_table(s_prior);
+    const long long P = (long long)nq * a.ncyc, ncell = P + (long long)nq * (a.ndin + 1);
+    const long long j0 = ncell * x / a.nx, j1 = ncell * (x + 1) / a.nx;
+    const size_t rq = (size_t)rg * nq;
+    struct Cell { long long e, t, *o; int q; bool v, pad; };
+    auto fetch = [&](long long c0) {
+        Cell c = {0, 0, nullptr, 0, false, false};
+        const long long j = c0 + half;
+        if (j >= j1) return c;
+        if (j < P) {
+            c.q = (int)(j / a.ncyc);
+            const size_t i = (rq + c.q) * a.ncyc + (size_t)(j - (long long)c.q * a.ncyc);
+            c.e = a.pos_errs[i]; c.t = a.pos_total[i]; c.o = a.posdq + i; c.v = true;
+        } else {
+            const long long k = j - P;
+            c.q = (int)(k / (a.ndin + 1));
+            const int d = (int)(k - (long long)c.q * (a.ndin + 1));
+            c.o = a.dindq + (rq + c.q) * (a.ndin + 1) + d;
+            if (d == a.ndin) c.pad = true;
+            else { c.e = a.din_errs[(rq + c.q) * a.ndin + d]; c.t = a.din_total[(rq + c.q) * a.ndin + d]; c.v = true; }
+        }
+        return c;
+    };
+    Cell cur = {0, 0, nullptr, 0, false, false};
+    if (a.deltas) cur = fetch(j0 + 2 * warp);
+
+    if (FROM_POS) {
+        const int L2 = a.ncyc;
+        for (int q = warp; q < NQ; q += nwarps) {
+            const size_t base = ((size_t)rg * NQ + q) * L2;
+            long long e = 0, t = 0;
+            for (int c0 = lane; c0 < L2; c0 += 8 * 32) {
+                long long ve[8], vt[8];
+#pragma unroll
+                for (int u = 0; u < 8; ++u) {
+                    const int c = c0 + 32 * u;
+                    ve[u] = c < L2 ? a.pos_errs[base + c] : 0;
+                    vt[u] = c < L2 ? a.pos_total[base + c] : 0;
+                }
+#pragma unroll
+                for (int u = 0; u < 8; ++u) { e += ve[u]; t += vt[u]; }
+            }
+#pragma unroll
+            for (int o = 16; o; o >>= 1) { e += __shfl_xor_sync(0xFFFFFFFFu, e, o); t += __shfl_xor_sync(0xFFFFFFFFu, t, o); }
+            if (lane == 0) { s_qe[q] = e; s_qt[q] = t; }
+        }
+        __syncthreads();
+        if (tid < NQ) {
+            const dd p = two_prod((double)s_qt[tid], c_p[tid]);
+            s_ph[tid] = p.hi;
+            s_pl[tid] = p.lo;
+            if (x == 0) { a.q_errs[rg * NQ + tid] = s_qe[tid]; a.q_total[rg * NQ + tid] = s_qt[tid]; }
+        }
+        __syncthreads();
+        if (tid == 0) {
+            long long e = 0, t = 0;
+            dd acc = {0.0, 0.0};
+            for (int q = 0; q < NQ; ++q) {
+                e += s_qe[q];
+                t += s_qt[q];
+                if (s_qt[q]) acc = dd_add(acc, dd{s_ph[q], s_pl[q]});
+            }
+            long long mq = 0;
+            if (t > 0) {
+                if (acc.hi == 0.0) mq = NQ - 1;
+                else {
+                    const dd p = dd_div_d(acc, (double)t);
+                    for (int m = 1; m < NQ; ++m) mq += dd_le(p, c_bound_hi[m], c_bound_lo[m]) ? 1 : 0;
+                }
+            }
+            s_rg[0] = e; s_rg[1] = t; s_rg[2] = mq;
+            if (x == 0) { a.rg_errs[rg] = e; a.rg_total[rg] = t; a.meanq[rg] = mq; }
+        }
+        if (!a.deltas) return;
+    } else if (tid == 0) {
+        s_rg[0] = a.rg_errs[rg]; s_rg[1] = a.rg_total[rg]; s_rg[2] = a.meanq[rg];
+    }
+    __syncthreads();
+    const Cands cd = load_cands();
+
+    if (warp == 0) {
+        const int mq = (int)s_rg[2];
+        const int d = posterior_q_cell<int>(mq, s_rg[0], s_rg[1], cd, s_prior) - mq;
+        if (lane == 0) {
+            s_rg[3] = d;
+            if (x == 0) a.rgdq[rg] = d;
+        }
+    }
+    __syncthreads();
+
+    int qa0 = 0, qa1 = 0, qb0 = 0, qb1 = 0;
+    if (x == 0) qa1 = nq;
+    else {
+        if (j0 < P) { qa0 = (int)(j0 / a.ncyc); qa1 = (int)((min(j1, P) - 1) / a.ncyc) + 1; }
+        if (j1 > P) { qb0 = (int)((max(j0, P) - P) / (a.ndin + 1)); qb1 = (int)((j1 - 1 - P) / (a.ndin + 1)) + 1; }
+    }
+    {
+        const int na = qa1 - qa0, n2 = na + qb1 - qb0;
+        const int prior1 = (int)s_rg[2] + (int)s_rg[3];
+        const long long *qe = FROM_POS ? s_qe : a.q_errs + (size_t)rg * nq;
+        const long long *qt = FROM_POS ? s_qt : a.q_total + (size_t)rg * nq;
+        for (int t0 = 2 * warp; t0 < n2; t0 += 2 * nwarps) {
+            const int t = t0 + half;
+            const bool v = t < n2;
+            const int q = t < na ? qa0 + t : qb0 + t - na;
+            const int qd = posterior_q_cell<int>(prior1, v ? qe[q] : 0, v ? qt[q] : 0, cd, s_prior) - prior1;
+            if (v && lead) {
+                s_prior2[q] = (int)(s_rg[2] + s_rg[3] + (long long)qd);
+                if (x == 0) a.qdq[(size_t)rg * nq + q] = qd;
+            }
+        }
+    }
+    __syncthreads();
+
+    for (long long c0 = j0 + 2 * warp; c0 < j1; c0 += 2 * nwarps) {
+        const Cell nxt = fetch(c0 + 2 * nwarps);
+        if (cur.pad && lead) *cur.o = 0;
+        const int p2 = cur.v ? s_prior2[cur.q] : 0;
+        const int r = posterior_q_cell<int>(p2, cur.e, cur.t, cd, s_prior);
+        if (cur.v && lead) *cur.o = r - p2;
+        cur = nxt;
+    }
+}
+
+}
diff --git a/kbbq-py_b200/csrc/prepare.cuh b/kbbq-py_b200/csrc/prepare.cuh
--- a/kbbq-py_b200/csrc/prepare.cuh
+++ b/kbbq-py_b200/csrc/prepare.cuh
@@ -16,7 +16,6 @@
     unsigned int *seg;
     unsigned int *cursor;
     entry_t *entries;
-    unsigned int *uni;
     int *status;
     int grid;
     int ng;
@@ -59,87 +58,101 @@
     }
 }
 
-__device__ __forceinline__ void identity_rows(const PrepArgs &a, long long grp, unsigned int &exist, unsigned int &sec,
-                                              bool report) {
-    unsigned int rgv[MAX_G];
-    load_rows(a, grp, rgv, sec, exist);
-    if (a.rg) {
-        unsigned int ok = 0;
-#pragma unroll
-        for (int k = 0; k < MAX_G; ++k)
-            if ((exist >> k) & 1) {
-                if (rgv[k] == 0) ok |= 1u << k;
-                else if (report) atomicOr(a.status, KBBQ_FLAG_RG_RANGE);
-            }
-        exist = ok;
-    }
-}
-
-__global__ void prep_uniform_kernel(PrepArgs a) {
-    const long long t0 = (long long)blockIdx.x * blockDim.x + threadIdx.x;
-    const long long stride = (long long)gridDim.x * blockDim.x;
-    if (t0 == 0) {
-        a.seg[0] = 0;
-        a.seg[1] = (unsigned int)a.ngroups;
-    }
+
+__device__ __forceinline__ void identity_rows(const uint16_t *rg, const uint8_t *second, long long N, int G, long long grp,
+                                              unsigned int &exist, unsigned int &sec) {
+    exist = 0;
+    sec = 0;
+#pragma unroll
+    for (int k = 0; k < MAX_G; ++k) {
+        const long long r = grp * G + k;
+        if (k < G && r < N) {
+            if (!rg || rg[r] == 0) exist |= 1u << k;
+            if (second && second[r]) sec |= 1u << k;
+        }
+    }
+}
+
+__device__ __noinline__ entry_t identity_record(const uint16_t *rg, const uint8_t *second, long long N, int G,
+                                                   uint32_t gbytes, uint32_t first, uint32_t grp) {
+    unsigned int exist, sec;
+    identity_rows(rg, second, N, G, grp, exist, sec);
+    const uint32_t mis0 = (uint32_t)(((unsigned long long)first * gbytes) & 15ull);
+    return make_entry(mis0 + (grp - first) * gbytes, grp, exist, sec);
+}
+
+__device__ __forceinline__ bool consumers_any(bool v, int nthreads) {
+    uint32_t r;
+    asm volatile("{\n .reg .pred p, q;\n setp.ne.u32 p, %1, 0;\n bar.red.or.pred q, 1, %2, p;\n selp.u32 %0, 1, 0, q;\n}"
+                 : "=r"(r)
+                 : "r"((uint32_t)v), "r"(nthreads)
+                 : "memory");
+    return r != 0;
+}
+
+__device__ __noinline__ bool slice_uniform(const uint16_t *rg, const uint8_t *second, long long N, int G, uint32_t lo,
+                                              uint32_t hi, int nthreads, int *status, uint32_t &flo, uint32_t &fhi) {
+    const int tid = threadIdx.x;
     unsigned int exist0, sec0;
-    identity_rows(a, 0, exist0, sec0, false);
-    bool differs = exist0 != (1u << a.G) - 1u;
-    for (int k = 2; k < a.G; ++k) differs |= ((sec0 >> k) & 1u) != ((sec0 >> (k & 1)) & 1u);
-    const bool wide = (a.G & (a.G - 1)) == 0 && a.G <= 16 && (!a.second || ((uintptr_t)a.second & 15u) == 0) &&
-                      (!a.rg || ((uintptr_t)a.rg & 15u) == 0);
-    long long done_groups = 0;
+    identity_rows(rg, second, N, G, 0, exist0, sec0);
+    const entry_t p0 = make_entry(0u, 0, exist0, sec0);
+    flo = p0.z;
+    fhi = p0.w;
+    bool differs = exist0 != (1u << G) - 1u;
+    for (int k = 2; k < G; ++k) differs |= ((sec0 >> k) & 1u) != ((sec0 >> (k & 1)) & 1u);
+    const long long r0 = (long long)lo * G, r1 = min((long long)hi * G, N);
+    differs |= (long long)hi * G > N;
+    auto row_differs = [&](long long r) {
+        bool d = (second && second[r] ? 1u : 0u) != ((sec0 >> ((int)(r % G) & 1)) & 1u);
+        if (rg && rg[r]) { d = true; atomicOr(status, KBBQ_FLAG_RG_RANGE); }
+        return d;
+    };
+    const bool wide = (G % 2 == 0 || G == 1) && (!second || ((uintptr_t)second & 15u) == 0) &&
+                      (!rg || ((uintptr_t)rg & 15u) == 0);
+    long long a0 = r1, a1 = r1;
     if (wide) {
-        const long long chunks = a.N / 16;
-        uint4 pat;
-        {
-            unsigned int v[4];
-            for (int j = 0; j < 4; ++j) {
-                v[j] = 0;
-                for (int k = 0; k < 4; ++k) v[j] |= ((sec0 >> ((4 * j + k) % a.G)) & 1u) << (8 * k);
-            }
-            pat = make_uint4(v[0], v[1], v[2], v[3]);
-        }
-        for (long long c = t0; c < chunks; c += stride) {
-            if (a.second) {
-                const uint4 s = reinterpret_cast<const uint4 *>(a.second)[c];
-                auto norm = [](unsigned int x) { return ((x | ((x | 0x80808080u) - 0x01010101u)) >> 7) & 0x01010101u; };
-                differs |= norm(s.x) != pat.x || norm(s.y) != pat.y || norm(s.z) != pat.z || norm(s.w) != pat.w;
-            } else {
-                differs |= sec0 != 0;
-            }
-            if (a.rg) {
-                const uint4 r0 = reinterpret_cast<const uint4 *>(a.rg)[2 * c], r1 = reinterpret_cast<const uint4 *>(a.rg)[2 * c + 1];
-                if (r0.x | r0.y | r0.z | r0.w | r1.x | r1.y | r1.z | r1.w) { differs = true; atomicOr(a.status, KBBQ_FLAG_RG_RANGE); }
-            }
-        }
-        done_groups = chunks * 16 / a.G;
-    }
-    for (long long grp = done_groups + t0; grp < a.ngroups; grp += stride) {
-        unsigned int exist, sec;
-        identity_rows(a, grp, exist, sec, true);
-        differs |= exist != exist0 || sec != sec0;
-    }
-    if (differs) a.uni[0] = 1u;
-    if (t0 == 0) {
-        const entry_t p0 = make_entry(0u, 0, exist0, sec0);
-        a.uni[1] = p0.z;
-        a.uni[2] = p0.w;
-    }
-}
-
-__global__ void prep_identity_kernel(PrepArgs a) {
-    if (a.uni[0] == 0u) return;
-    const unsigned long long E = (unsigned long long)a.ngroups;
-    for (long long grp = (long long)blockIdx.x * blockDim.x + threadIdx.x; grp < a.ngroups;
-         grp += (long long)gridDim.x * blockDim.x) {
-        unsigned int exist, sec;
-        identity_rows(a, grp, exist, sec, false);
-        const unsigned long long lo = slice_lo(E, slice_of(E, (unsigned long long)grp, a.grid), a.grid);
-        const unsigned int j = (unsigned int)(((unsigned long long)grp - lo) % (unsigned int)a.ng);
-        const unsigned int mis0 = (unsigned int)((((unsigned long long)grp - j) * a.gbytes) & 15ull);
-        a.entries[grp] = make_entry(mis0 + j * a.gbytes, grp, exist, sec);
-    }
+        a0 = min((r0 + 15) / 16 * 16, r1);
+        a1 = max(a0, r1 / 16 * 16);
+    }
+    for (long long r = r0 + tid; r < a0; r += nthreads) differs |= row_differs(r);
+    for (long long r = a1 + tid; r < r1; r += nthreads) differs |= row_differs(r);
+    if (a1 > a0) {
+        const unsigned int e = (sec0 & 1u) * 0x01010101u, o = (G == 1 ? sec0 & 1u : (sec0 >> 1) & 1u) * 0x01010101u;
+        const unsigned int pat = (e & 0x00FF00FFu) | (o & 0xFF00FF00u);
+        auto norm = [](unsigned int x) { return ((x | ((x | 0x80808080u) - 0x01010101u)) >> 7) & 0x01010101u; };
+        constexpr int U = 8;
+        const long long c0 = a0 / 16, c1 = a1 / 16;
+        if (second) {
+            for (long long c = c0 + tid; c < c1; c += U * (long long)nthreads) {
+                uint4 v[U];
+#pragma unroll
+                for (int u = 0; u < U; ++u) {
+                    const long long cu = c + u * (long long)nthreads;
+                    v[u] = cu < c1 ? reinterpret_cast<const uint4 *>(second)[cu] : make_uint4(pat, pat, pat, pat);
+                }
+#pragma unroll
+                for (int u = 0; u < U; ++u)
+                    differs |= (norm(v[u].x) != pat) | (norm(v[u].y) != pat) | (norm(v[u].z) != pat) | (norm(v[u].w) != pat);
+            }
+        } else {
+            differs |= pat != 0u;
+        }
+        if (rg) {
+            for (long long c = 2 * c0 + tid; c < 2 * c1; c += (U / 2) * (long long)nthreads) {
+                uint4 v[U / 2];
+#pragma unroll
+                for (int u = 0; u < U / 2; ++u) {
+                    const long long cu = c + u * (long long)nthreads;
+                    v[u] = cu < 2 * c1 ? reinterpret_cast<const uint4 *>(rg)[cu] : make_uint4(0u, 0u, 0u, 0u);
+                }
+                unsigned int any = 0;
+#pragma unroll
+                for (int u = 0; u < U / 2; ++u) any |= v[u].x | v[u].y | v[u].z | v[u].w;
+                if (any) { differs = true; atomicOr(status, KBBQ_FLAG_RG_RANGE); }
+            }
+        }
+    }
+    return !consumers_any(differs, nthreads);
 }
 
 template <int MODE>
@@ -235,8 +248,6 @@
     unsigned int *cursor;
     unsigned int *uni;
     entry_t *entries;
-    short *fold_cyc;
-    short *fold_din;
     size_t bytes;
 };
 
@@ -251,8 +262,6 @@
     w.cursor = (unsigned int *)(p + off);   off = align_up(off + sizeof(unsigned int) * (size_t)R, 256);
     w.uni = (unsigned int *)(p + off);      off = align_up(off + sizeof(unsigned int) * 4, 256);
     w.entries = (entry_t *)(p + off);       off = align_up(off + sizeof(entry_t) * max_entries, 256);
-    w.fold_cyc = (short *)(p + off);        off = align_up(off + sizeof(short) * (size_t)R * NQ * 2 * L, 256);
-    w.fold_din = (short *)(p + off);        off = align_up(off + sizeof(short) * (size_t)R * NQ * 16, 256);
     w.bytes = off;
     return w;
 }
@@ -263,22 +272,13 @@
     PrepArgs a;
     a.rg = rg; a.second = second; a.N = N; a.G = G;
     a.ngroups = (N + G - 1) / G; a.R = R;
-    a.seg = w.seg; a.cursor = w.cursor; a.entries = w.entries; a.uni = w.uni; a.status = status;
+    a.seg = w.seg; a.cursor = w.cursor; a.entries = w.entries; a.status = status;
     a.grid = grid; a.ng = ng; a.gbytes = gbytes; a.slot = slot;
-    KBBQ_CUDA(cudaMemsetAsync(w.uni, (R == 1 && a.ngroups > 0) ? 0 : 0xFF, sizeof(unsigned int) * 4, st));
     if (a.ngroups == 0) {
         KBBQ_CUDA(cudaMemsetAsync(w.seg, 0, sizeof(unsigned int) * ((size_t)R + 1), st));
         return KBBQ_OK;
     }
     const unsigned int blocks = (unsigned int)((a.ngroups + PREP_THREADS - 1) / PREP_THREADS);
-    if (R == 1) {
-        const unsigned int few = std::min<unsigned int>(blocks, (unsigned int)std::max(grid, 1) * 8u);
-        prep_uniform_kernel<<<few, PREP_THREADS, 0, st>>>(a);
-        KBBQ_LAUNCHED();
-        prep_identity_kernel<<<few, PREP_THREADS, 0, st>>>(a);
-        KBBQ_LAUNCHED();
-        return KBBQ_OK;
-    }
     const size_t smem = R <= PREP_SMEM_RG ? sizeof(unsigned int) * (size_t)R : 0;
     KBBQ_CUDA(cudaMemsetAsync(w.cursor, 0, sizeof(unsigned int) * (size_t)R, st));
     prep_bucket_kernel<0><<<blocks, PREP_THREADS, smem, st>>>(a);
diff --git a/kbbq-py_b200/csrc/stage.cuh b/kbbq-py_b200/csrc/stage.cuh
--- a/kbbq-py_b200/csrc/stage.cuh
+++ b/kbbq-py_b200/csrc/stage.cuh
@@ -76,7 +76,7 @@
     int ng;
     long long total_bytes;
     int pw, nprod;
-    bool uniform;
+    uint32_t E1;
 };
 
 __device__ __forceinline__ void mbar_expect_tx(uint32_t bar, uint32_t bytes) {
@@ -94,7 +94,7 @@
     if (p.contig) {
         if (lane != 0 || p.pw != 0) return;
         for (int sub = 0; sub < p.nsub; ++sub) {
-            uint32_t s_lo = p.seg[sub], s_hi = p.seg[sub + 1];
+            uint32_t s_lo = p.seg ? p.seg[sub] : 0u, s_hi = p.seg ? p.seg[sub + 1] : p.E1;
             if (s_hi <= p.lo) continue;
             if (s_lo >= p.hi) break;
             if (s_lo < p.lo) s_lo = p.lo;
diff --git a/kbbq-py_b200/kbbq/_native.py b/kbbq-py_b200/kbbq/_native.py
--- a/kbbq-py_b200/kbbq/_native.py
+++ b/kbbq-py_b200/kbbq/_native.py
@@ -23,6 +23,7 @@
     "kbbq_workspace_bytes": (_i, [_i64, _i, _i, C.POINTER(_sz)]),
     "kbbq_build": (_i, [_vp] * 5 + [_i64, _i, _i, _i] + [_vp] * 4 + [_vp, _sz, _vp, _i, _vp]),
     "kbbq_marginals": (_i, [_vp, _vp, _i, _i] + [_vp] * 5 + [_vp]),
+    "kbbq_model": (_i, [_vp] * 4 + [_i, _i] + [_vp] * 9 + [_vp]),
     "kbbq_delta_q": (_i, [_vp, _vp, _vp, _i64, _vp, _vp]),
     "kbbq_get_delta_qs": (_i, [_vp] * 9 + [_i, _i, _i, _i] + [_vp] * 4 + [_vp]),
     "kbbq_apply": (_i, [_vp] * 4 + [_i64, _i, _i, _i] + [_vp] * 5 + [_i, _i, _vp, _vp, _sz, _vp, _i, _vp]),
diff --git a/kbbq-py_b200/kbbq/device.py b/kbbq-py_b200/kbbq/device.py
--- a/kbbq-py_b200/kbbq/device.py
+++ b/kbbq-py_b200/kbbq/device.py
@@ -139,15 +139,10 @@
 
     @_on_device
     def model(self):
-        L, R = self.L, self.R
-        _native.check(self.lib.kbbq_marginals(_p(self.pos_errs), _p(self.pos_total), L, R, _p(self.q_errs),
-                                              _p(self.q_total), _p(self.rg_errs), _p(self.rg_total),
-                                              _p(self.meanq), self._stream()))
-        _native.check(self.lib.kbbq_get_delta_qs(_p(self.meanq), _p(self.rg_errs), _p(self.rg_total),
-                                                 _p(self.q_errs), _p(self.q_total), _p(self.pos_errs),
-                                                 _p(self.pos_total), _p(self.din_errs), _p(self.din_total),
-                                                 R, NQ, 2 * L, 16, _p(self.rgdq), _p(self.qdq), _p(self.posdq),
-                                                 _p(self.dindq), self._stream()))
+        _native.check(self.lib.kbbq_model(_p(self.pos_errs), _p(self.pos_total), _p(self.din_errs), _p(self.din_total),
+                                          self.L, self.R, _p(self.q_errs), _p(self.q_total), _p(self.rg_errs),
+                                          _p(self.rg_total), _p(self.meanq), _p(self.rgdq), _p(self.qdq),
+                                          _p(self.posdq), _p(self.dindq), self._stream()))
 
     @_on_device
     def apply(self, seq, qual, out, rg=None, second=None, path=0):
```

After: 887.0 billion (median of 6 runs). 1.02x the previous value.
